# tomer196/GaUDI

Hardware: AMD Instinct MI355X
Metric: guided molecules/sec (1000-step) (higher is better)
Workload: dtype f32

## Files before the change

### gaudi_amd/_lib.py

```python
from __future__ import annotations

import ctypes as C
import os

import numpy as np

_PKG = os.path.dirname(os.path.abspath(__file__))
LIB_PATH = os.environ.get("GAUDI_LIB", os.path.join(_PKG, "libgaudi_hip.so"))


class GaudiError(RuntimeError):
    pass


class EdmConfig(C.Structure):
    _fields_ = [("in_node_nf", C.c_int32), ("hidden_nf", C.c_int32), ("n_layers", C.c_int32),
                ("inv_sublayers", C.c_int32), ("attention", C.c_int32), ("tanh", C.c_int32),
                ("coords_range", C.c_float), ("norm_constant", C.c_float), ("normalization_factor", C.c_float),
                ("diffusion_steps", C.c_int32), ("noise_power", C.c_float), ("noise_precision", C.c_float),
                ("norm_values", C.c_float * 3), ("sin_embedding", C.c_int32)]


class PredConfig(C.Structure):
    _fields_ = [("in_nf", C.c_int32), ("out_nf", C.c_int32), ("hidden_nf", C.c_int32), ("n_layers", C.c_int32),
# ... 18 lines not shown


class AtomTables(C.Structure):
    _fields_ = [("n_types", C.c_int32), ("ring_size", C.c_int32 * 16), ("ring_elem", (C.c_int32 * 6) * 16),
                ("templ", ((C.c_double * 2) * 6) * 16), ("no_orientation", C.c_int32 * 16), ("extra_angle", C.c_double * 16),
                ("n_template_h", C.c_int32 * 16), ("template_h_parent", (C.c_int32 * 2) * 16), ("h_elem", C.c_int32),
                ("c_elem", C.c_int32), ("h_bond", C.c_double)]


ATOMS_MAX_ATOMS = 384
ATOMS_MAX_BONDS = 384
ATOMS_PLACE_H, ATOMS_FINGERPRINT = 1, 2

FP = C.POINTER(C.c_float)
IP = C.POINTER(C.c_int32)
DP = C.POINTER(C.c_double)


class TargetSpec(C.Structure):
    _fields_ = [("K", C.c_int32), ("w", FP), ("q", FP), ("c", FP), ("side", IP), ("scale", FP),
                ("w_per_mol", C.c_int32), ("q_per_mol", C.c_int32), ("c_per_mol", C.c_int32), ("side_per_mol", C.c_int32),
                ("scale_per_mol", C.c_int32), ("t_lo", C.c_int32), ("t_hi", C.c_int32)]


TARGET_CB = C.CFUNCTYPE(None, C.c_void_p, C.c_int, C.c_int, FP, C.c_float, FP)
TARGET_CBZ = C.CFUNCTYPE(None, C.c_void_p, C.c_int, C.c_int, C.c_int, C.c_int, FP, FP, C.c_float, FP, FP)

EXPORTS = {
    "gaudi_create": (C.c_int, [C.c_int, C.POINTER(C.c_void_p)]),
    "gaudi_destroy": (None, [C.c_void_p]),
    "gaudi_last_error": (C.c_char_p, [C.c_void_p]),
    "gaudi_load_edm": (C.c_int, [C.c_void_p, C.POINTER(EdmConfig), C.c_int, C.POINTER(C.c_char_p), C.POINTER(FP),
                                 C.POINTER(C.c_int64)]),
    "gaudi_load_predictor": (C.c_int, [C.c_void_p, C.POINTER(PredConfig), C.c_int, C.POINTER(C.c_char_p),
                                       C.POINTER(FP), C.POINTER(C.c_int64)]),
    "gaudi_get_gamma": (C.c_int, [C.c_void_p, FP]),
    "gaudi_get_step_coefficients": (C.c_int, [C.c_void_p, FP]),
    "gaudi_phi": (C.c_int, [C.c_void_p, C.c_int, C.c_int, FP, FP, FP, FP, FP]),
    "gaudi_predictor_fwd": (C.c_int, [C.c_void_p, C.c_int, C.c_int, FP, FP, FP, FP, FP]),
    "gaudi_predictor_grad": (C.c_int, [C.c_void_p, C.c_int, C.c_int, FP, FP, FP, FP, FP, FP, FP]),
    "gaudi_step": (C.c_int, [C.c_void_p, C.c_int, C.c_int, C.c_int, FP, FP, FP, FP, FP, C.c_float, FP]),
    "gaudi_decode": (C.c_int, [C.c_void_p, C.c_int, C.c_int, FP, FP, FP, FP, FP, FP]),
    "gaudi_sample": (C.c_int, [C.c_void_p, C.c_int, C.c_int, FP, FP, C.c_uint64, C.c_int64, FP, C.c_float, FP,
                               C.c_float, FP, FP, FP, C.POINTER(Diag)]),
    "gaudi_sample_cb": (C.c_int, [C.c_void_p, C.c_int, C.c_int, FP, FP, C.c_uint64, C.c_int64, FP, C.c_float, TARGET_CB,
                                  C.c_void_p, C.c_float, FP, FP, FP, C.POINTER(Diag)]),
    "gaudi_sample_cbz": (C.c_int, [C.c_void_p, C.c_int, C.c_int, FP, FP, C.c_uint64, C.c_int64, FP, C.c_float, TARGET_CBZ,
                                   C.c_void_p, C.c_float, FP, FP, FP, C.POINTER(Diag)]),
    "gaudi_sample_chain": (C.c_int, [C.c_void_p, C.c_int, C.c_int, FP, FP, C.c_uint64, C.c_int64, FP, C.c_float, C.c_int, FP]),
    "gaudi_predict_noised": (C.c_int, [C.c_void_p, C.c_int, C.c_int, FP, FP, IP, FP, FP, C.c_uint64, C.c_int64, FP, FP, FP]),
    "gaudi_check_stability": (C.c_int, [C.c_void_p, C.POINTER(RingTables), C.c_int, C.c_int, FP, IP, IP,
                                        C.POINTER(C.c_uint8), FP, FP, C.POINTER(StabilityAux)]),
    "gaudi_stability_profile_get": (C.c_int, [C.c_void_p, C.POINTER(C.c_int32), C.POINTER(C.c_double)]),
    "gaudi_rings_to_atoms": (C.c_int, [C.c_void_p, C.POINTER(RingTables), C.POINTER(AtomTables), C.c_int, C.c_int, FP, IP, IP,
                                       C.c_int, C.c_int, C.c_int, IP, IP, DP, DP, IP, IP, IP, C.POINTER(C.c_uint64)]),
    "gaudi_atoms_profile_get": (C.c_int, [C.c_void_p, C.POINTER(C.c_int32), C.POINTER(C.c_double)]),
    "gaudi_philox_normal": (C.c_int, [C.c_void_p, C.c_uint64, C.c_int64, C.c_int, C.c_int, C.c_int, C.c_int, FP]),
    "gaudi_host_schedule": (C.c_int, [C.c_int, C.c_float, C.c_float, FP, FP]),
    "gaudi_host_eigh3": (C.c_int, [C.c_int, DP, DP]),
    "gaudi_host_graph_meta": (C.c_int, [C.c_int, C.c_int, FP, FP, C.POINTER(C.c_int32), C.POINTER(C.c_int32),
                                        C.POINTER(C.c_int32), C.POINTER(C.c_uint32), C.POINTER(C.c_uint32), FP, C.c_int32,
                                        C.POINTER(C.c_int32)]),
    "gaudi_host_pack_matrix": (C.c_int, [C.c_int, C.c_int, C.c_int, C.c_int, C.c_int, FP, FP]),
    "gaudi_host_pack_matrix_split": (C.c_int, [C.c_int, C.c_int, C.c_int, C.c_int, C.c_int, C.c_int, C.c_float, FP, FP]),
    "gaudi_host_pack_matrix_f16": (C.c_int, [C.c_int, C.c_int, C.c_int, C.c_int, C.c_int, C.c_float, FP, FP]),
    "gaudi_host_weight_scale": (C.c_int, [C.c_int, C.POINTER(FP), IP, IP, IP, FP]),
    "gaudi_host_node_operand_offset": (C.c_int, [C.c_int, C.c_int, C.c_int, C.c_int, C.c_int, IP]),
    "gaudi_profile_reset": (C.c_int, [C.c_void_p, C.c_int]),
    "gaudi_profile_get": (C.c_int, [C.c_void_p, C.POINTER(C.c_int32), C.POINTER(C.c_double), C.POINTER(C.c_int64)]),
    "gaudi_set_steps_per_launch": (C.c_int, [C.c_void_p, C.c_int]),
    "gaudi_set_readout_nodes": (C.c_int, [C.c_void_p, C.c_int]),
    "gaudi_set_fix_noise": (C.c_int, [C.c_void_p, C.c_int, C.c_int64]),
    "gaudi_host_graph_meta8": (C.c_int, [C.c_int, C.c_int, FP, FP, C.POINTER(C.c_int32), C.POINTER(C.c_int32),
                                         C.POINTER(C.c_int32), C.POINTER(C.c_uint32), C.POINTER(C.c_uint32), FP,
                                         C.POINTER(C.c_uint16), C.POINTER(C.c_uint16), C.c_int32, C.POINTER(C.c_int32)]),
    "gaudi_kernel_variant": (C.c_int, [C.c_void_p, C.POINTER(C.c_int32), C.POINTER(C.c_int32)]),
    "gaudi_edge_math": (C.c_int, [C.c_void_p, C.POINTER(C.c_int32), C.POINTER(C.c_int32)]),
    "gaudi_node_buffers": (C.c_int, [C.c_void_p, C.POINTER(C.c_int32)]),
    "gaudi_last_workgroups": (C.c_int, [C.c_void_p, C.POINTER(C.c_int32), C.POINTER(C.c_int32)]),
    "gaudi_host_pack_plan_wide": (C.c_int, [C.c_int, C.c_int, C.c_int, C.c_int, FP, FP, C.POINTER(C.c_int32), C.POINTER(C.c_int32),
                                           C.POINTER(C.c_int32), C.POINTER(C.c_int32)]),
    "gaudi_set_plan_hint": (C.c_int, [C.c_void_p, C.c_int32, C.c_int32]),
    "gaudi_last_warning": (C.c_char_p, [C.c_void_p]),
    "gaudi_abi_version": (C.c_int, []),
    "gaudi_last_family_split": (C.c_int, [C.c_void_p, C.POINTER(C.c_int32)]),
    "gaudi_profile_clock": (C.c_int, [C.c_void_p, C.POINTER(C.c_double)]),
    "gaudi_last_keep_h": (C.c_int, [C.c_void_p, C.POINTER(C.c_int32)]),
    "gaudi_host_pack_plan": (C.c_int, [C.c_int, C.c_int, FP, FP, C.POINTER(C.c_int32), C.POINTER(C.c_int32), C.POINTER(C.c_int32),
                                      C.POINTER(C.c_int32)]),
    "gaudi_edm_nll": (C.c_int, [C.c_void_p, C.c_int, C.c_int, FP, FP, IP, FP, FP, C.c_uint64, C.c_int64, FP, FP, FP]),
    "gaudi_host_nll_terms": (C.c_int, [C.c_int, C.c_float, C.c_float, C.c_float, C.c_float, C.c_int, C.c_int, C.c_int, FP, FP, FP,
                                       IP, FP]),
    "gaudi_predictor_loss_grad": (C.c_int, [C.c_void_p, C.c_int, C.c_int, FP, FP, IP, FP, FP, FP, C.c_uint64, C.c_int64, FP, FP,
                                            FP, FP, IP]),
    "gaudi_predictor_grad_size": (C.c_int, [C.c_void_p, C.POINTER(C.c_int64)]),
    "gaudi_host_pred_train_layout": (C.c_int, [C.c_void_p, C.c_int, C.POINTER(C.c_char_p), C.POINTER(FP), C.POINTER(C.c_int64),
                                               IP, IP, FP]),
    "gaudi_edm_loss_grad": (C.c_int, [C.c_void_p, C.c_int, C.c_int, FP, FP, IP, FP, FP, C.c_uint64, C.c_int64, FP, C.c_int, FP,
                                      FP, FP, FP, IP]),
    "gaudi_edm_grad_size": (C.c_int, [C.c_void_p, C.POINTER(C.c_int64)]),
    "gaudi_edm_set_train_weights": (C.c_int, [C.c_void_p, C.c_int, C.POINTER(C.c_char_p), C.POINTER(FP), C.POINTER(C.c_int64)]),
    "gaudi_host_edm_train_layout": (C.c_int, [C.c_void_p, C.c_int, C.POINTER(C.c_char_p), C.POINTER(FP), C.POINTER(C.c_int64),
                                              IP, IP, FP]),
    "gaudi_host_edm_seed_coef": (C.c_int, [C.c_int, C.c_int, C.c_int, C.c_int, C.c_int, IP, FP, FP, FP]),
    "gaudi_sample_grid": (C.c_int, [C.c_void_p, C.c_int, C.c_int, FP, FP, C.c_uint64, C.c_int64, FP, C.c_float, FP, C.c_float,
                                    C.c_int, IP, FP, FP, FP, FP, FP, FP, C.POINTER(Diag)]),
    "gaudi_step_pair": (C.c_int, [C.c_void_p, C.c_int, C.c_int, C.c_int, C.c_int, FP, FP, FP, FP, FP, C.c_float, FP]),
    "gaudi_sample_cb_grid": (C.c_int, [C.c_void_p, C.c_int, C.c_int, FP, FP, C.c_uint64, C.c_int64, FP, C.c_float, TARGET_CB,
                                       TARGET_CBZ, C.c_void_p, C.c_float, C.c_int, IP, FP, FP, FP, FP, FP, FP, C.POINTER(Diag)]),
    "gaudi_host_grid_coefficients": (C.c_int, [C.c_int, C.c_float, C.c_float, C.c_int, IP, FP, IP]),
    "gaudi_sample_target": (C.c_int, [C.c_void_p, C.c_int, C.c_int, FP, FP, C.c_uint64, C.c_int64, FP, C.c_float,
                                      C.POINTER(TargetSpec), C.c_int, IP, FP, FP, FP, FP, FP, FP, FP, C.POINTER(Diag)]),
    "gaudi_step_target": (C.c_int, [C.c_void_p, C.c_int, C.c_int, C.c_int, C.c_int, FP, FP, FP, FP, C.POINTER(TargetSpec), FP, FP]),
    "gaudi_host_target_seed": (C.c_int, [C.POINTER(TargetSpec), C.c_int, C.c_int, FP, FP]),
}

ABI_VERSION = 7
_ROUND6_EXPORTS = ("gaudi_last_warning", "gaudi_abi_version", "gaudi_last_family_split", "gaudi_profile_clock", "gaudi_last_keep_h")
_NLL_EXPORTS = ("gaudi_edm_nll", "gaudi_predictor_loss_grad", "gaudi_predictor_grad_size", "gaudi_edm_loss_grad",
                "gaudi_edm_grad_size", "gaudi_edm_set_train_weights")
_GRID_EXPORTS = ("gaudi_sample_grid", "gaudi_step_pair", "gaudi_sample_cb_grid")
_TARGET_EXPORTS = ("gaudi_sample_target", "gaudi_step_target")
_ATOMS_EXPORTS = ("gaudi_rings_to_atoms", "gaudi_atoms_profile_get")

_lib = None


def load_library() -> C.CDLL:
    global _lib
    if _lib is not None:
        return _lib
    if not os.path.exists(LIB_PATH):
        raise GaudiError(f"{LIB_PATH} not found: build it with `python -m gaudi_amd.build` "
                         "(there is no CPU fallback for the sampler)")
    lib = C.CDLL(LIB_PATH)
    lenient = "GAUDI_LIB" in os.environ
    abi = None
    if hasattr(lib, "gaudi_abi_version"):
        lib.gaudi_abi_version.restype, lib.gaudi_abi_version.argtypes = C.c_int, []
        abi = int(lib.gaudi_abi_version())
    if abi != ABI_VERSION and not lenient:
        raise GaudiError(f"{LIB_PATH} exports ABI version {abi}, this package expects {ABI_VERSION}: rebuild it "
                         "(`python -m gaudi_amd.build --force`)")
    for name, (res, args) in EXPORTS.items():
        if lenient and not hasattr(lib, name) and (name.startswith("gaudi_host_") or name in _ROUND6_EXPORTS + _NLL_EXPORTS + _GRID_EXPORTS + _TARGET_EXPORTS + _ATOMS_EXPORTS):
            continue
        if lenient and abi != ABI_VERSION and name.startswith("gaudi_host_"):
            continue
        fn = getattr(lib, name)
        fn.restype = res
        fn.argtypes = args
    _lib = lib
    return lib


def fptr(a: np.ndarray | None):
    if a is None:
        return None
    assert a.dtype == np.float32 and a.flags["C_CONTIGUOUS"]
    return a.ctypes.data_as(FP)


def f32(a) -> np.ndarray:
    return np.ascontiguousarray(np.asarray(a, dtype=np.float32))


def grid_coefficients(T: int, noise_power: float, noise_precision: float, grid):
    lib = load_library()
    g = np.ascontiguousarray(np.asarray(grid).reshape(-1), dtype=np.int32)
    coef = np.zeros((max(len(g) - 1, 0), 4), np.float32)
    land = np.zeros(max(len(g) - 1, 0), np.int32)
    rc = lib.gaudi_host_grid_coefficients(int(T), float(noise_power), float(noise_precision), len(g), g.ctypes.data_as(IP),
                                          coef.ctypes.data_as(FP), land.ctypes.data_as(IP))
    if rc != 0:
        raise GaudiError(f"gaudi_host_grid_coefficients failed ({rc}): the grid must be strictly descending integers "
                         f"T >= g[0] > ... > g[n] = 0 with at least two entries")
    return coef, land
```

### gaudi_amd/csrc/gaudi_hip.hip

```cpp
#include <hip/hip_runtime.h>

#include <algorithm>
#include <climits>
#include <queue>
#include <cmath>
#include <cstdio>
#include <cstdlib>
#include <chrono>
#include <cstring>
#include <map>
#include <mutex>
#include <string>
#include <vector>

#include "../../include/gaudi_hip.h"
#include "kernel_table.h"

using namespace gaudi;

struct DevBuf {
  void* p = nullptr;
  size_t cap = 0;
  hipError_t reserve(size_t bytes) {
    if (bytes <= cap) return hipSuccess;
    if (p) (void)hipFree(p);
    p = nullptr;
    cap = 0;
    hipError_t e = hipMalloc(&p, bytes);
    if (e == hipSuccess) cap = bytes;
    return e;
  }
  void release() {
    if (p) (void)hipFree(p);
    p = nullptr;
    cap = 0;
  }
  template <class T>
  T* as() const { return (T*)p; }
};

struct PinBuf {
  void* p = nullptr;
  size_t cap = 0;
  hipError_t reserve(size_t bytes) {
    if (bytes <= cap) return hipSuccess;
    if (p) (void)hipHostFree(p);
    p = nullptr;
    cap = 0;
    hipError_t e = hipHostMalloc(&p, bytes, hipHostMallocDefault);
    if (e == hipSuccess) cap = bytes;
    return e;
  }
  void release() {
    if (p) (void)hipHostFree(p);
    p = nullptr;
    cap = 0;
  }
  template <class T>
  T* as() const { return (T*)p; }
};

enum NodeBuf : int {
  kResident = 0,
  kAllGlobal = 1,
  kPqLds = 2,
  kPredFifthGlobal = 3,
};
struct LaunchPlan {
  int waves = 4;
  int ring = 0;
  bool mr = false;
  NodeBuf nodes = kResident;
  bool two = false;
  bool fr = false;
  int ef = 2;
  int groups = 0;
  int nslots = 0;
  int hk = 0;
  int pubx = 0, pub_ch = 0;
};

struct gaudi_handle {
  int device = 0;
  hipStream_t stream = nullptr;
  std::string err;
  std::string warn;
  bool has_edm = false, has_pred = false;
  gaudi_edm_config ecfg{};
  gaudi_pred_config pcfg{};
  int HPE = 0, HPP = 0;
  DevBuf edm_w, pred_w, coef_d, edm_w4, pred_w4;
  DevBuf edm_ws, pred_ws;
  size_t edm_w_bytes = 0, pred_w_bytes = 0, edm_ws_bytes = 0, pred_ws_bytes = 0;
  float edm_hinv = 0.f, pred_hinv = 0.f;
  std::vector<float> gamma, coef;
  DevBuf d_mask, d_order, d_edges, d_emask, d_npairs, d_seg, d_zin, d_zout, d_t, d_x, d_h, d_noise, d_nan, d_dpred,
      d_pred, d_tw, d_stash, d_chain, d_sx, d_stype, d_sn, d_sflags, d_sdist, d_sadj, d_saux, d_stab, d_as, d_ncols, d_soff,
      d_sidx, d_gnode, d_rowmap, d_compmol, d_ncomp, d_clock, d_gcoef, d_gidx, d_zt;
  DevBuf d_atoms[9];
  DevBuf d_vtpar, d_vttrace, d_vtdev;
  struct VtCall {
    const gaudi_target_spec* spec = nullptr;
    int K = 0, Btot = 0, b0 = 0;
    float* trace = nullptr;
  }* vt = nullptr;
  PinBuf p_pred, p_dpred;
  PinBuf p_z, p_dz;
  DevBuf d_dz;
  hipEvent_t cb_event = nullptr;
  int steps_per_launch = 25;
  int variant = 8;
  LaunchPlan plan;
  bool split = true;
  bool no_fr = false;
  bool wide_full = true;
  bool gn8_pq = true;
  bool gn8 = true;
  bool force_gn8 = false;
  bool pack = true;
  int pairs_cap = -1;
  int pairs = 1;
  int num_cus = 256;
  bool pred_rounds = true;
  bool pack_now = false;
  bool force_mr = false;
  bool force_gn = false;
  bool fix_noise = false;
  long long fix_key = 0;
  int readout_n = 0;
  struct PredTrainState* pt = nullptr;
  struct EdmTrainState* et = nullptr;
  bool edm_stale = false;
  int plan_min_slots = 0, plan_force_waves = 0;
  int call_min_slots = 0, call_force_waves = 0;
  bool call_cut = false;
  int call_narrow = 0;
  const int32_t* call_molmap = nullptr;
  bool keep_h = true;
  bool gn8_pack = true;
  bool family_split = false;
  int last_split_resident = 0;
  bool prof = false;
  struct EventLog {
    std::vector<std::pair<hipEvent_t, hipEvent_t>> pending, spare;
    double ms = 0.0;
    long long n = 0;
    static constexpr size_t kWindow = 32;
    hipError_t fold(size_t keep) {
      while (pending.size() > keep) {
        float t = 0.f;
        hipError_t e = hipEventSynchronize(pending.front().second);
        if (e == hipSuccess) e = hipEventElapsedTime(&t, pending.front().first, pending.front().second);
        if (e != hipSuccess) return e;
        ms += t;
        ++n;
        spare.push_back(pending.front());
        pending.erase(pending.begin());
      }
      return hipSuccess;
    }
    hipError_t begin(hipStream_t st, std::pair<hipEvent_t, hipEvent_t>& ev) {
      hipError_t e = fold(kWindow - 1);
      if (e != hipSuccess) return e;
      if (!spare.empty()) {
        ev = spare.back();
        spare.pop_back();
      } else {
        if ((e = hipEventCreate(&ev.first)) != hipSuccess) return e;
        if ((e = hipEventCreate(&ev.second)) != hipSuccess) return e;
      }
      return hipEventRecord(ev.first, st);
    }
    hipError_t end(hipStream_t st, const std::pair<hipEvent_t, hipEvent_t>& ev) {
      pending.push_back(ev);
      return hipEventRecord(ev.second, st);
    }
    void reset(bool destroy) {
      for (auto& p : pending) spare.push_back(p);
      pending.clear();
      if (destroy) {
        for (auto& p : spare) {
          (void)hipEventDestroy(p.first);
          (void)hipEventDestroy(p.second);
        }
        spare.clear();
      }
      ms = 0.0;
      n = 0;
    }
  } prof_log, stab_log, atoms_log;
  long long prof_steps = 0;
#ifdef GAUDI_STAMPS
  DevBuf d_stamps;
  unsigned long long stamp_acc[32] = {0};
#endif
};

// ... 407 lines not shown
      }
      if (want_align && !sl.empty()) {
        const int prev_i = sl.back().i;
        while (sl.size() % 16) sl.push_back({prev_i, prev_i, 0.f, false});
      }
      want_align = false;
      const int o = (int)sl.size() % 16;
      if ((o + L + 15) / 16 > 2) {
        const int prev_i = sl.empty() ? i : sl.back().i;
        while (sl.size() % 16) sl.push_back({prev_i, prev_i, 0.f, false});
      }
      runs[b][i] = {(int)sl.size(), L};
      sl.insert(sl.end(), run.begin(), run.end());
      total[b] += L;
    }
    if (!sl.empty()) {
      const int prev_i = sl.back().i;
      while (sl.size() % 16) sl.push_back({prev_i, prev_i, 0.f, false});
    }
    M.ncols[b] = last + 1;
    M.ntiles[b] = (int)sl.size() / 16;
    max_tiles = std::max(max_tiles, M.ntiles[b]);
  }
  M.S = std::max(16 * max_tiles, (min_slots + 15) / 16 * 16);
  if (M.S > 0xffff) {
    err = "too many edge slots";
    return GAUDI_E_CAPACITY;
  }
  const int S = M.S;
  M.edges.assign((size_t)B * S, 0);
  M.emask.assign((size_t)B * S, 0.f);
  M.seg.assign((size_t)B * N, 0);
  M.soff.assign((size_t)B * (N + 1), 0);
  M.sidx.assign((size_t)B * S, 0);
  for (int b = 0; b < B; ++b) {
    const std::vector<Slot>& sl = slots[b];
    const int ns = (int)sl.size();
    for (int t0 = 0; t0 < ns; t0 += 16) {
      int c = 0;
      while (c < 16) {
        int e = c;
        while (e + 1 < 16 && sl[t0 + e + 1].i == sl[t0 + c].i) ++e;
        const int i = sl[t0 + c].i;
        const int part = runs[b][i].second > 0 && runs[b][i].first < t0 ? 1 : 0;
        for (int k = c; k <= e; ++k) {
          const Slot& q = sl[t0 + k];
          M.edges[(size_t)b * S + t0 + k] = (uint32_t)q.i | ((uint32_t)q.j << 8) | ((uint32_t)c << 16) |
                                            ((uint32_t)(k == e) << 20) | ((uint32_t)part << 21);
          M.emask[(size_t)b * S + t0 + k] = q.m;
        }
        c = e + 1;
      }
    }
    for (int i = 0; i < N; ++i)
      M.seg[(size_t)b * N + i] = ((uint32_t)runs[b][i].first << 16) | (uint32_t)runs[b][i].second;
    uint16_t* off = &M.soff[(size_t)b * (N + 1)];
    uint16_t* idx = &M.sidx[(size_t)b * S];
    int n_out = 0;
    for (int j = 0; j < N; ++j) {
      off[j] = (uint16_t)n_out;
      for (int k = 0; k < ns; ++k)
        if (sl[k].live && sl[k].j == j) idx[n_out++] = (uint16_t)k;
    }
    off[N] = (uint16_t)n_out;
  }
  M.order.resize(B);
  for (int b = 0; b < B; ++b) M.order[b] = b;
  std::stable_sort(M.order.begin(), M.order.end(), [&](int a, int c) {
    return M.ntiles[a] != M.ntiles[c] ? M.ntiles[a] > M.ntiles[c] : total[a] > total[c];
  });
  return GAUDI_OK;
}

KernelTable* gaudi::g_kernel_tables;

static kernel_fn find_kernel(const KernelKey& k) {
  for (const KernelTable* t = g_kernel_tables; t; t = t->next)
    for (int i = 0; i < t->n; ++i)
      if (t->entries[i].key == k) return t->entries[i].fn;
  return nullptr;
}
static std::string key_name(const KernelKey& k) {
  char buf[160];
  snprintf(buf, sizeof buf, "waves=%d SP=%d MR=%d GN=%d FR=%d PG=%d EF=%d HPE=%d HPP=%d VT=%d", k.waves, k.sp, (int)k.mr, k.gn, (int)k.fr,
           (int)k.pg, k.ef, k.hpe, k.hpp, (int)k.vt);
  return buf;
}
static std::string duplicate_kernel_key() {
  std::vector<KernelKey> seen;
  for (const KernelTable* t = g_kernel_tables; t; t = t->next)
    for (int i = 0; i < t->n; ++i) {
      if (std::find(seen.begin(), seen.end(), t->entries[i].key) != seen.end()) return key_name(t->entries[i].key);
      seen.push_back(t->entries[i].key);
    }
  return "";
}
static int gn_of(NodeBuf nodes) { return nodes == kAllGlobal ? 1 : nodes == kPqLds ? 2 : 0; }
static KernelKey key4(int hpe, int hpp, bool gn = false, int ef = 2) {
  KernelKey k{};
  k.waves = 4;
  k.gn = gn ? 1 : 0;
  k.ef = ef;
  k.hpe = hpe;
  k.hpp = hpp;
  return k;
}
static KernelKey key8(int hpe, int hpp, int ring, bool mr, NodeBuf nodes = kResident) {
  KernelKey k{};
  k.waves = 8;
  k.sp = ring;
  k.mr = mr;
  k.gn = gn_of(nodes);
  k.pg = nodes == kPredFifthGlobal;
  k.ef = 2;
  k.hpe = hpe;
  k.hpp = hpp;
  return k;
}
static bool have_kernel8(int hpe, int hpp, int ring, bool mr, NodeBuf nodes = kResident) {
  return find_kernel(key8(hpe, hpp, ring, mr, nodes)) != nullptr;
}
static NodeBuf launch_nodes(const LaunchPlan& p, int hpe, int hpp) {
  return p.nodes == kPredFifthGlobal && !(hpe && hpp) ? kResident : p.nodes;
}
static kernel_fn plan_kernel(const LaunchPlan& p, int hpe, int hpp, bool vt) {
  if (p.waves != 8) {
    KernelKey k = key4(hpe, hpp, p.nodes == kAllGlobal, hpe ? p.ef : 2);
    k.vt = vt && hpp;
    return find_kernel(k);
  }
  const NodeBuf nodes = launch_nodes(p, hpe, hpp);
  const bool mr = p.mr && hpp;
  KernelKey k = nodes == kResident ? key8(hpe, hpp, p.ring, mr) : key8(hpe, hpp, 1, true, nodes);
  k.vt = vt && hpp;
  if (p.fr && nodes == kResident && !mr) {
    k.fr = true;
    if (kernel_fn f = find_kernel(k)) return f;
    k.fr = false;
  }
  return find_kernel(k);
}

static int round_hidden(int H) {
  static const int sizes[] = {32, 48, 64, 128, 192, 208, 256};
  for (int s : sizes)
    if (s >= H) return s;
  return 0;
}

static int dense_ew4(int N) { return std::max(32, ((N + kWaves - 1) / kWaves * (N - 1) + 31) / 32 * 32); }

static size_t lds_bytes(int hpe, int hpp, int N, int D, int EW, bool gn = false, int ef = 2) {
  size_t net = 0;
  if (hpe)
    net = std::max(net, (size_t)((gn ? 0 : 4 * N * (hpe + 4)) + kWaves * 16 * (hpe + 4) + 8 * N + kWaves * EW * 9 + (6 + ef) * hpe +
                                 (ef > 2 ? kWaves * EW * ef : 0)));
  if (hpp) net = std::max(net, (size_t)((gn ? 0 : 5 * N * (hpp + 4)) + kWaves * 16 * (hpp + 4) + 12 * N + kWaves * EW * 10 + 32 + 10 * hpp));
  return sizeof(float) * (common_floats(N, D, EW) + net);
}
static size_t gnode_floats(int hpe, int hpp, int N) {
  return std::max((size_t)(hpe ? 4 * N * (hpe + 4) : 0), (size_t)(hpp ? 5 * N * (hpp + 4) : 0));
}

static size_t lds_floats8_base(int hpe, int hpp, int N, int D, int S, int split, NodeBuf nodes = kResident) {
  size_t net = 0;
  const int pbuf = nodes == kPredFifthGlobal ? 4 : 5;
  const int gn = gn_of(nodes);
  if (hpe) net = std::max(net, (size_t)((gn ? w8::gn_lds_buffers(gn) : 5) * N * (hpe + 4) + w8::edge_ring_floats(hpe, split) + 8 * N + 2 * align4(N) + 96 + S * 9 + 8 * hpe));
  if (hpp) net = std::max(net, (size_t)(w8::edge_ring_floats(hpp, split) + (gn ? w8::gn_lds_buffers(gn) : pbuf) * N * (hpp + 4) + 12 * N + 2 * align4(N) + 96 + S * 10 + 32 + 10 * hpp));
  return common_floats8(N, D, S) + net;
}
static size_t gnode_floats8(int hpe, int hpp, int N) {
  return std::max((size_t)(hpe ? 5 * N * (hpe + 4) : 0), (size_t)(hpp ? 5 * N * (hpp + 4) : 0));
}
static bool gn8_stage_fits(int hpe, int hpp, int N) {
  for (int hp : {hpe, hpp})
    if (hp && 2 * (size_t)w8::stage_stride(N * (hp + 4)) > w8::edge_ring_floats(hp, 1)) return false;
  return true;
}
static bool node_f16_fits(int hp, int N, int split, NodeBuf nodes) {
  const bool gn = gn_of(nodes) != 0;
  if (!hp || !split || !GAUDI_NODE_F16) return true;
  if (N > (gn ? 48 : 32)) return false;
  const int nct = N <= 16 ? 1 : N <= 32 ? 2 : 3;
  const int ring = w8::edge_ring_floats(hp, split);
  return w8::nh_split_floats(hp, nct) <= (w8::node_ring_idle(hp, split, gn) ? ring : ring / 2);
}
static bool plan_pub8(int hpe, int hpp, int N, int D, int S, int split, int& pubx, int& pub_ch, NodeBuf nodes = kResident) {
  pubx = 0;
  pub_ch = 0;
  const int gn = gn_of(nodes);
  if (!node_f16_fits(hpe, N, split, nodes) || !node_f16_fits(hpp, N, split, nodes)) return false;
  const long long cap = 160 * 1024 / 4 - 64;
  const long long base = (long long)lds_floats8_base(hpe, hpp, N, D, S, split, nodes);
  if (base > cap) return false;
  if (!hpp) return true;
  const int T = hpp / 16;
  const long long own = (gn ? 0LL : 2LL * N * (hpp + 4)) + (split ? w8::edge_ring_floats(hpp, split) : 0);
  pub_ch = w8::pub_chunk_tiles(S, own + (cap - base), T);
  if (pub_ch < 1) return false;
  const int nch = (T + pub_ch - 1) / pub_ch;
  pub_ch = (T + nch - 1) / nch;
  pubx = (int)std::max(0LL, (long long)S * (16 * pub_ch + 4) - own);
  return true;
}
static size_t lds_bytes8(int hpe, int hpp, int N, int D, int S, int pubx, int split, NodeBuf nodes = kResident) {
  return sizeof(float) * (lds_floats8_base(hpe, hpp, N, D, S, split, nodes) + (hpp ? pubx : 0));
}

static int launch(gaudi_handle* h, const KParams& P, int hpe, int hpp, long long steps) {
  const LaunchPlan& plan = h->plan;
  const bool v8 = plan.waves == 8;
  const bool se = hpe && plan.ef > 2;
  const kernel_fn fn = plan_kernel(plan, hpe, hpp, P.vt != nullptr);
  if (!fn)
    return fail(h, GAUDI_E_INVALID,
                "no kernel instantiated for padded hidden sizes (" + std::to_string(hpe) + "," + std::to_string(hpp) + ")" +
                    (v8 ? " in the 8-wave family" : se ? " among the sin_embedding kernels" : ""));
  size_t lds = v8 ? lds_bytes8(hpe, hpp, P.N, 3 + P.F, P.EW, P.pubx, plan.ring, launch_nodes(plan, hpe, hpp))
                  : lds_bytes(hpe, hpp, P.N, 3 + P.F, P.EW, plan.nodes == kAllGlobal, se ? 24 : 2);
  if (v8 && P.hk_off) lds = sizeof(float) * ((size_t)P.hk_off + (size_t)plan.hk);
  if (lds > 160 * 1024)
    return fail(h, GAUDI_E_CAPACITY, "molecule needs " + std::to_string(lds) + " B of LDS (>160 KiB): N too large");
  {
    static std::mutex attr_mu;
    static std::map<std::pair<int, const void*>, int> granted_by_fn;
    std::lock_guard<std::mutex> lock(attr_mu);
    int& granted = granted_by_fn[{h->device, (const void*)fn}];
    if ((int)lds > granted) {
      HIPCHECK(h, hipFuncSetAttribute((const void*)fn, hipFuncAttributeMaxDynamicSharedMemorySize, (int)lds));
      granted = (int)lds;
    }
  }
  std::pair<hipEvent_t, hipEvent_t> ev{nullptr, nullptr};
  if (h->prof) HIPCHECK(h, h->prof_log.begin(h->stream, ev));
#ifdef GAUDI_STAMPS
  KParams PS = P;
  HIPCHECK(h, h->d_stamps.reserve(sizeof(unsigned long long) * 32));
  HIPCHECK(h, hipMemsetAsync(h->d_stamps.p, 0, sizeof(unsigned long long) * 32, h->stream));
  PS.stamps = h->d_stamps.as<unsigned long long>();
  hipLaunchKernelGGL(fn, dim3(P.B), dim3(v8 ? w8::kThreads : kThreads), lds, h->stream, PS);
  {
    unsigned long long tmp[32];
    HIPCHECK(h, hipMemcpyAsync(tmp, h->d_stamps.p, sizeof(tmp), hipMemcpyDeviceToHost, h->stream));
    HIPCHECK(h, hipStreamSynchronize(h->stream));
    for (int i = 0; i < 32; ++i) h->stamp_acc[i] += tmp[i];
    if (getenv("GAUDI_PRINT_STAMPS")) {
      static const char* nm[] = {"node_gemm", "edge_gemm", "edge_epilogue", "barrier", "misc", "bwd_node", "bwd_stash_reload",
                                 "bwd_colsum_tail", "pub_wait", "stash", "pub_write", "colsum_loop", "colsum_barrier", "b_dcp",
                                 "b_gemm_de", "b_dv", "b_gemm_dt1", "b_du", "stage_vectors", "geo", "edm_embed_head", "noise_update",
                                 "bwd_reload_loads", "bwd_vec_commit", "pred_readout", "bwd_prologue", "x2", "x3"};
      unsigned long long tot = 0;
      for (int i = 0; i < ST_N; ++i) tot += h->stamp_acc[i];
      fprintf(stderr, "[stamps] cumulative shares (block 0, wave 0):");
      for (int i = 0; i < ST_N; ++i) fprintf(stderr, " %s=%.1f%%", nm[i], 100.0 * h->stamp_acc[i] / (tot ? tot : 1));
      fprintf(stderr, " total=%llu ticks\n", tot);
      if (tmp[31])
        fprintf(stderr, "[stamps] shader clock during this launch: %.0f MHz (%llu cycles / %llu ticks of 100 MHz)\n",
                100.0 * (double)tmp[30] / (double)tmp[31], tmp[30], tmp[31]);
    }
  }
#else
  if (h->prof) {
    KParams PC = P;
    HIPCHECK(h, h->d_clock.reserve(sizeof(unsigned long long) * 4));
    PC.clock_out = h->d_clock.as<unsigned long long>();
    hipLaunchKernelGGL(fn, dim3(P.B), dim3(v8 ? w8::kThreads : kThreads), lds, h->stream, PC);
  } else {
    hipLaunchKernelGGL(fn, dim3(P.B), dim3(v8 ? w8::kThreads : kThreads), lds, h->stream, P);
  }
#endif
  HIPCHECK(h, hipGetLastError());
  if (h->prof) {
    HIPCHECK(h, h->prof_log.end(h->stream, ev));
    h->prof_steps += steps;
  }
  return GAUDI_OK;
}

struct Pack {
  int G = 0;
  int NG = 0;
  std::vector<float> umask, uemask;
  std::vector<uint8_t> align;
  std::vector<int32_t> rowmap;
  std::vector<int32_t> compmol;
  std::vector<int32_t> ncomp;
};
static std::vector<std::vector<int>> used_nodes(int B, int N, const float* node_mask, const float* edge_mask) {
  std::vector<std::vector<int>> used(B);
  for (int b = 0; b < B; ++b) {
    std::vector<char> keep(N, 0);
    for (int i = 0; i < N; ++i) {
      const bool li = node_mask[(size_t)b * N + i] != 0.f;
      if (li) keep[i] = 1;
      for (int j = 0; j < N; ++j) {
        const bool lj = node_mask[(size_t)b * N + j] != 0.f;
        if (edge_mask[((size_t)b * N + i) * N + j] != 0.f && (li || lj)) keep[i] = keep[j] = 1;
      }
    }
    for (int i = 0; i < N; ++i)
      if (keep[i]) used[b].push_back(i);
  }
  return used;
}
static void pack_groups(int B, int N, const float* node_mask, const float* edge_mask, const Meta8& M, Pack& pk, int NG = 0,
                        int TG = w8::kWaves, bool narrow = false, int maxcomp = kMaxComp, const int32_t* molmap = nullptr,
                        int max_multi = INT_MAX) {
  if (NG < N && !narrow) NG = N;
  const std::vector<std::vector<int>> used = used_nodes(B, N, node_mask, edge_mask);
  struct Group {
    std::vector<int> mols;
    int nodes = 0, tiles = 0;
  };
  std::vector<Group> groups;
  int multi = 0;
  for (int b : M.order) {
    const int nn = (int)used[b].size(), nt = M.ntiles[b];
    Group* fit = nullptr;
    for (Group& g : groups)
      if ((int)g.mols.size() < maxcomp && g.nodes + nn <= NG && g.tiles + nt <= TG && (g.mols.size() > 1 || multi < max_multi)) {
        fit = &g;
        if (g.mols.size() == 1) ++multi;
        break;
      }
    if (!fit) {
      groups.emplace_back();
      fit = &groups.back();
    }
    fit->mols.push_back(b);
    fit->nodes += nn;
    fit->tiles += nt;
  }
  const int G = (int)groups.size();
  pk.G = G;
  pk.NG = NG;
  pk.umask.assign((size_t)G * NG, 0.f);
  pk.uemask.assign((size_t)G * NG * NG, 0.f);
  pk.align.assign((size_t)G * NG, 0);
  pk.rowmap.assign((size_t)G * NG, -1);
  pk.compmol.assign((size_t)G * kMaxComp, 0);
  pk.ncomp.assign(G, 0);
  std::vector<int> slot_of(N);
  for (int g = 0; g < G; ++g) {
    int base = 0;
    for (size_t k = 0; k < groups[g].mols.size(); ++k) {
      const int b = groups[g].mols[k];
      pk.compmol[(size_t)g * kMaxComp + k] = molmap ? molmap[b] : b;
      std::fill(slot_of.begin(), slot_of.end(), -1);
      for (size_t r = 0; r < used[b].size(); ++r) slot_of[used[b][r]] = base + (int)r;
      if (!used[b].empty()) pk.align[(size_t)g * NG + base] = 1;
      for (int i : used[b]) {
        const int si = slot_of[i];
        pk.umask[(size_t)g * NG + si] = node_mask[(size_t)b * N + i];
        pk.rowmap[(size_t)g * NG + si] = (b * N + i) | ((int32_t)k << 28);
// ... 84 lines not shown
    }
  }
  if (!gn8 && !narrow_taken && h->pack_now && h->pack && B > 1 && (int64_t)B * N < (1 << 28)) {
    struct Cand {
      int NG, TG;
    };
    std::vector<Cand> cands;
    bool want_wide = h->pairs == 2;
    int max_multi = INT_MAX;
    if (h->pairs == 1 && B > h->num_cus) {
      const int cus = std::max(1, h->num_cus);
      const double solo = (double)((B + cus - 1) / cus);
      auto makespan = [&](int p) {
        const double kPair = 1.81, kAlone = 1.07;
        std::priority_queue<double, std::vector<double>, std::greater<double>> free_at;
        for (int c = 0; c < cus; ++c) free_at.push(0.0);
        double end = 0.0;
        auto run = [&](int n, double cost) {
          for (int k = 0; k < n; ++k) {
            const double t = free_at.top() + cost;
            free_at.pop();
            free_at.push(t);
            end = std::max(end, t);
          }
        };
        run(p, kPair);
        run(B - 2 * p, kAlone);
        return end;
      };
      double best = solo * 0.995;
      int best_p = -1;
      for (int p = cus; p <= B / 2 + cus - 1; p += cus) {
        const int pp = std::min(p, B / 2);
        const double m = makespan(pp);
        if (m < best) { best = m; best_p = pp; }
      }
      if (h->pairs_cap >= 0) best_p = std::min(h->pairs_cap, B / 2);
      if (best_p >= 0) {
        pack_groups(B, N, node_mask, edge_mask, M, pk, N, w8::kWaves);
        want_wide = (long long)pk.G * 10 >= (long long)B * 9;
        max_multi = best_p;
      }
    }
    if (want_wide && h->pairs_cap >= 0) max_multi = h->pairs_cap;
    if (want_wide)
      for (int ng = std::min(2 * N, 32); ng > N; --ng) {
        const long long cap = 160 * 1024 / 4 - 64;
        if ((long long)lds_floats8_base(hpe, hpp, ng, Dz, 16 * (w8::kWaves + 1), h->split ? 2 : 0) > cap) continue;
        cands.push_back({ng, 2 * w8::kWaves});
      }
    cands.push_back({N, w8::kWaves});
    for (const Cand& cd : cands) {
      const bool wide = cd.NG > N;
      pack_groups(B, N, node_mask, edge_mask, M, pk, cd.NG, cd.TG, false, kMaxComp, nullptr, wide ? max_multi : INT_MAX);
      if (pk.G >= B && !(wide && h->pairs_cap == 0)) continue;
      Meta8 M2;
      rc = build_meta8(pk.G, cd.NG, pk.umask.data(), pk.uemask.data(), M2, err, wide ? 0 : M.S, pk.align.data());
      if (rc != GAUDI_OK) continue;
      const bool mr2 = hpp && M2.S > 16 * w8::kWaves;
      if (!wide && M2.S > std::max(M.S, 16 * w8::kWaves)) continue;
      if (mr2 && !mr && !h->pred_rounds) continue;
      RingPlan p2 = plan_for(cd.NG, M2.S, mr2);
      if (p2.mode < 0 || (p2.mode != 0) != (mode_u != 0)) continue;
      RingPlan full{1, 0, 0};
      if (wide && p2.mode == 2 && mr2 && h->wide_full && hpe && hpp && have_kernel8(hpe, hpp, 1, true, kPredFifthGlobal) &&
          plan_pub8(hpe, hpp, cd.NG, Dz, M2.S, 1, full.pubx, full.pub_ch, kPredFifthGlobal)) {
        p2 = full;
        pg_run = true;
      }
      M = std::move(M2);
      B = pk.G;
      nm_used = pk.umask.data();
      n_slots = cd.NG;
      acc = p2;
      mr_run = mr2;
      use_pack = true;
      break;
    }
  }
  const bool packed = use_pack;
  const NodeBuf nodes = pg_run ? kPredFifthGlobal : gn8;
  P.pubx = acc.pubx;
  P.pub_ch = acc.pub_ch;
  if (getenv("GAUDI_DEBUG_PLAN"))
    fprintf(stderr, "[plan] molecules=%d workgroups=%d N=%d node slots=%d S=%d split=%d mr=%d nodes=%d pub_ch=%d pubx=%d lds=%zu\n", B0, B, N,
            n_slots, M.S, acc.mode, (int)mr_run, (int)nodes, acc.pub_ch, acc.pubx, lds_bytes8(hpe, hpp, n_slots, Dz, M.S, acc.pubx, acc.mode, nodes));
  auto up = [&](DevBuf& d, const void* src, size_t bytes) -> hipError_t {
    hipError_t e = d.reserve(bytes);
    if (e != hipSuccess) return e;
    return hipMemcpyAsync(d.p, src, bytes, hipMemcpyHostToDevice, h->stream);
  };
  HIPCHECK(h, up(h->d_ncols, M.ncols.data(), sizeof(int) * B));
  HIPCHECK(h, up(h->d_mask, nm_used, sizeof(float) * B * n_slots));
  if (packed) {
    HIPCHECK(h, up(h->d_rowmap, pk.rowmap.data(), sizeof(int32_t) * pk.rowmap.size()));
    HIPCHECK(h, up(h->d_compmol, pk.compmol.data(), sizeof(int32_t) * pk.compmol.size()));
    HIPCHECK(h, up(h->d_ncomp, pk.ncomp.data(), sizeof(int32_t) * pk.ncomp.size()));
  }
  HIPCHECK(h, up(h->d_order, M.order.data(), sizeof(int) * B));
  HIPCHECK(h, up(h->d_edges, M.edges.data(), sizeof(uint32_t) * M.edges.size()));
  HIPCHECK(h, up(h->d_emask, M.emask.data(), sizeof(float) * M.emask.size()));
  HIPCHECK(h, up(h->d_npairs, M.ntiles.data(), sizeof(int) * B));
  HIPCHECK(h, up(h->d_seg, M.seg.data(), sizeof(uint32_t) * M.seg.size()));
  HIPCHECK(h, up(h->d_soff, M.soff.data(), sizeof(uint16_t) * M.soff.size()));
  HIPCHECK(h, up(h->d_sidx, M.sidx.data(), sizeof(uint16_t) * M.sidx.size()));
  HIPCHECK(h, hipStreamSynchronize(h->stream));
  P.B = B;
  P.N = n_slots;
  P.NR = N;
  P.EW = M.S;
  P.node_mask = h->d_mask.as<float>();
  P.order = h->d_order.as<int>();
  P.edges = h->d_edges.as<uint32_t>();
  P.emask = h->d_emask.as<float>();
  P.npairs = h->d_npairs.as<int>();
  P.seginfo = h->d_seg.as<uint32_t>();
  P.ncols = h->d_ncols.as<int>();
  P.soff = h->d_soff.as<uint16_t>();
  P.sidx = h->d_sidx.as<uint16_t>();
  P.rowmap = packed ? h->d_rowmap.as<int32_t>() : nullptr;
  P.compmol = packed ? h->d_compmol.as<int32_t>() : nullptr;
  P.ncomp = packed ? h->d_ncomp.as<int32_t>() : nullptr;
  P.hk_off = 0;
  int hk = 0;
  if (h->keep_h && GAUDI_NODE_F16 && acc.mode >= 1 && nodes == kResident) {
    const size_t floats = lds_bytes8(hpe, hpp, n_slots, Dz, M.S, acc.pubx, acc.mode) / sizeof(float);
    const size_t at = (floats + 3) & ~(size_t)3;
    const size_t need = (size_t)w8::nh_keep_floats(std::max(hpe, hpp), n_slots);
    if ((at + need) * sizeof(float) + 1024 <= 160 * 1024) {
      P.hk_off = (int)at;
      hk = (int)need;
    }
  }
  if (pg_run) {
    const size_t stride = ((size_t)n_slots * (hpp + 4) + 63) / 64 * 64;
    HIPCHECK(h, h->d_gnode.reserve(sizeof(float) * (stride * (size_t)B + 256)));
    P.gnode = h->d_gnode.as<float>();
    P.gnode_stride = (long long)stride;
  }
  if (gn8) {
    const size_t stride = (gnode_floats8(hpe, hpp, N) + 63) / 64 * 64;
    HIPCHECK(h, h->d_gnode.reserve(sizeof(float) * (stride * (size_t)B + 256)));
    P.gnode = h->d_gnode.as<float>();
    P.gnode_stride = (long long)stride;
  }
  plan.waves = 8;
  plan.ring = acc.mode;
  plan.mr = mr_run;
  plan.nodes = nodes;
  plan.fr = !h->no_fr && gn8 == kResident && acc.mode == 1 && n_slots > 16;
  plan.groups = B;
  plan.nslots = n_slots;
  plan.hk = hk;
  plan.pubx = acc.pubx;
  plan.pub_ch = acc.pub_ch;
  return GAUDI_OK;
}

static int stage_graph(gaudi_handle* h, int B, int N, const float* node_mask, const float* edge_mask, KParams& P, int hpe,
                       int hpp) {
  if (B <= 0 || N <= 0) return fail(h, GAUDI_E_INVALID, "B and N must be positive");
  if ((int64_t)B * N >= (1 << 28)) return fail(h, GAUDI_E_CAPACITY, "B * N must stay below 2^28 per call: cut the request into several calls");
  LaunchPlan plan;
  const bool se = hpe && h->ecfg.sin_embedding;
  if (h->variant == 8 && !h->force_gn && !se) {
    const int rc8 = stage_graph8(h, B, N, node_mask, edge_mask, P, hpe, hpp, plan);
    if (rc8 == GAUDI_OK) h->plan = plan;
    if (rc8 <= 0) return rc8;
    P.pubx = P.pub_ch = 0;
  }
  plan.groups = B;
  plan.nslots = N;
  if (hpp && 4 * N * 3 > 4 * 16 * (hpp + 4))
    return fail(h, GAUDI_E_CAPACITY, "N too large for the 4-wave predictor kernels at this hidden size");
  Meta M;
  std::string err;
  int rc = build_meta(B, N, node_mask, edge_mask, M, err);
  if (rc) return fail(h, rc, err);
  HIPCHECK(h, h->d_mask.reserve(sizeof(float) * B * N));
  HIPCHECK(h, h->d_order.reserve(sizeof(int) * B));
  HIPCHECK(h, h->d_edges.reserve(sizeof(uint32_t) * M.edges.size()));
  HIPCHECK(h, h->d_emask.reserve(sizeof(float) * M.emask.size()));
  HIPCHECK(h, h->d_npairs.reserve(sizeof(int) * M.npairs.size()));
  HIPCHECK(h, h->d_seg.reserve(sizeof(uint32_t) * M.seg.size()));
  HIPCHECK(h, h->d_ncols.reserve(sizeof(int) * B));
  HIPCHECK(h, hipMemcpyAsync(h->d_ncols.p, M.ncols.data(), sizeof(int) * B, hipMemcpyHostToDevice, h->stream));
  HIPCHECK(h, hipMemcpyAsync(h->d_mask.p, node_mask, sizeof(float) * B * N, hipMemcpyHostToDevice, h->stream));
  HIPCHECK(h, hipMemcpyAsync(h->d_order.p, M.order.data(), sizeof(int) * B, hipMemcpyHostToDevice, h->stream));
  HIPCHECK(h, hipMemcpyAsync(h->d_edges.p, M.edges.data(), sizeof(uint32_t) * M.edges.size(), hipMemcpyHostToDevice, h->stream));
  HIPCHECK(h, hipMemcpyAsync(h->d_emask.p, M.emask.data(), sizeof(float) * M.emask.size(), hipMemcpyHostToDevice, h->stream));
  HIPCHECK(h, hipMemcpyAsync(h->d_npairs.p, M.npairs.data(), sizeof(int) * M.npairs.size(), hipMemcpyHostToDevice, h->stream));
  HIPCHECK(h, hipMemcpyAsync(h->d_seg.p, M.seg.data(), sizeof(uint32_t) * M.seg.size(), hipMemcpyHostToDevice, h->stream));
  HIPCHECK(h, hipStreamSynchronize(h->stream));
  P.B = B;
  P.N = N;
  P.NR = N;
  P.EW = M.EW;
  P.node_mask = h->d_mask.as<float>();
  P.order = h->d_order.as<int>();
  P.edges = h->d_edges.as<uint32_t>();
  P.emask = h->d_emask.as<float>();
  P.npairs = h->d_npairs.as<int>();
  P.seginfo = h->d_seg.as<uint32_t>();
  P.ncols = h->d_ncols.as<int>();
  const int Dz = 3 + (hpe ? h->ecfg.in_node_nf : h->pcfg.in_nf);
  const bool part_of_batch = h->plan_min_slots || h->plan_force_waves || h->call_min_slots || h->call_force_waves || h->call_cut;
  const int ef = plan.ef = se ? 24 : 2;
  const bool have_g = (!hpe || find_kernel(key4(hpe, 0, true, ef))) && (!hpp || find_kernel(key4(0, hpp, true)));
  if (h->force_gn || lds_bytes(hpe, hpp, N, Dz, part_of_batch ? std::max(M.EW, dense_ew4(N)) : M.EW, false, ef) > 160 * 1024) {
    if (have_g && lds_bytes(hpe, hpp, N, Dz, M.EW, true, ef) <= 160 * 1024) {
      plan.nodes = kAllGlobal;
      const size_t stride = (gnode_floats(hpe, hpp, N) + 63) / 64 * 64;
      HIPCHECK(h, h->d_gnode.reserve(sizeof(float) * stride * (size_t)B));
      P.gnode = h->d_gnode.as<float>();
      P.gnode_stride = (long long)stride;
    }
  }
  plan.two = plan.nodes == kAllGlobal || (se && hpp && !find_kernel(key4(hpe, hpp, false, ef)));
  h->plan = plan;
  return GAUDI_OK;
}

static void fill_edm(gaudi_handle* h, KParams& P) {
  const gaudi_edm_config& c = h->ecfg;
  P.F = c.in_node_nf;
  P.T = c.diffusion_steps;
  P.edm.w = (h->variant == 8 && h->plan.waves == 4) ? h->edm_w4.as<float>() : h->edm_w.as<float>();
  P.edm.w_bytes = (unsigned)h->edm_w_bytes;
  P.edm.F = c.in_node_nf;
  P.edm.L = c.n_layers;
  P.edm.S = c.inv_sublayers;
  P.edm.attention = c.attention;
  P.edm.use_tanh = c.tanh;
  P.edm.coords_range = c.coords_range;
  P.edm.norm_constant = c.norm_constant;
  P.edm.normf = c.normalization_factor > 0.f ? c.normalization_factor : (float)P.NR;
  P.edm.ktail = h->plan.waves == 8 && has_ktail(c.hidden_nf, h->HPE);
  P.edm.ws = h->edm_ws.as<float>();
  P.edm.ws_bytes = (unsigned)h->edm_ws_bytes;
  P.edm.hinv = h->edm_hinv;
  P.coef = h->coef_d.as<float>();
  const float g0 = h->gamma[0];
  P.alpha0 = sqrtf(sigmoid_host(-g0));
  P.sigma0 = sqrtf(sigmoid_host(g0));
  P.sigma_x = expf(0.5f * g0);
  P.nv0 = c.norm_values[0];
  P.nv1 = c.norm_values[1];
}

extern "C" {

int gaudi_create(int device, gaudi_handle** out) {
  if (!out) return GAUDI_E_INVALID;
  *out = nullptr;
  static const std::string dup = duplicate_kernel_key();
  if (!dup.empty()) {
    fprintf(stderr, "libgaudi_hip: two translation units register the kernel %s\n", dup.c_str());
    return GAUDI_E_INVALID;
  }
  int n = 0;
  if (hipGetDeviceCount(&n) != hipSuccess || device < 0 || device >= n) return GAUDI_E_HIP;
  gaudi_handle* h = new gaudi_handle();
  h->device = device;
  if (const char* v = getenv("GAUDI_WAVES")) h->variant = atoi(v) == 4 ? 4 : 8;
  if (const char* v = getenv("GAUDI_EDGE_MATH")) h->split = std::string(v) != "fp32";
  if (const char* v = getenv("GAUDI_FORCE_GN")) h->force_gn = atoi(v) != 0;
  if (const char* v = getenv("GAUDI_GN8")) h->gn8 = atoi(v) != 0;
  if (const char* v = getenv("GAUDI_FORCE_GN8")) h->force_gn8 = atoi(v) != 0;
  if (const char* v = getenv("GAUDI_FORCE_MR")) h->force_mr = atoi(v) != 0;
  if (const char* v = getenv("GAUDI_PACK")) h->pack = atoi(v) != 0;
  if (const char* v = getenv("GAUDI_GN8_PACK")) h->gn8_pack = atoi(v) != 0;
  if (const char* v = getenv("GAUDI_GN8_PQ")) h->gn8_pq = atoi(v) != 0;
  if (const char* v = getenv("GAUDI_WIDE_FULL")) h->wide_full = atoi(v) != 0;
  if (const char* v = getenv("GAUDI_KEEP_H")) h->keep_h = atoi(v) != 0;
  if (const char* v = getenv("GAUDI_FAMILY_SPLIT")) h->family_split = atoi(v) != 0;
  if (const char* v = getenv("GAUDI_PAIRS")) h->pairs = atoi(v);
  if (const char* v = getenv("GAUDI_PAIRS_CAP")) h->pairs_cap = atoi(v);
  {
    int cus = 0;
    if (hipDeviceGetAttribute(&cus, hipDeviceAttributeMultiprocessorCount, device) == hipSuccess && cus > 0) h->num_cus = cus;
  }
  if (const char* v = getenv("GAUDI_PRED_ROUNDS")) h->pred_rounds = atoi(v) != 0;
  h->no_fr = getenv("GAUDI_NO_FR") != nullptr;
  h->plan.waves = h->variant;
  if (hipSetDevice(device) != hipSuccess || hipStreamCreateWithFlags(&h->stream, hipStreamNonBlocking) != hipSuccess) {
    delete h;
    return GAUDI_E_HIP;
  }
  *out = h;
  return GAUDI_OK;
}

void gaudi_destroy(gaudi_handle* h) {
  if (!h) return;
  (void)hipSetDevice(h->device);
  if (h->stream) (void)hipStreamSynchronize(h->stream);
  h->prof_log.reset(true);
  h->stab_log.reset(true);
  h->atoms_log.reset(true);
  DevBuf* bufs[] = {&h->edm_w, &h->pred_w, &h->coef_d, &h->edm_w4, &h->pred_w4, &h->edm_ws, &h->pred_ws, &h->d_mask, &h->d_order, &h->d_edges, &h->d_emask, &h->d_npairs,
                    &h->d_seg, &h->d_zin, &h->d_zout, &h->d_t, &h->d_x, &h->d_h, &h->d_noise, &h->d_nan, &h->d_dpred,
                    &h->d_pred, &h->d_tw, &h->d_stash, &h->d_chain, &h->d_sx, &h->d_stype, &h->d_sn,
                    &h->d_sflags, &h->d_sdist, &h->d_sadj, &h->d_saux, &h->d_stab, &h->d_as, &h->d_ncols, &h->d_soff, &h->d_sidx,
                    &h->d_gnode, &h->d_rowmap, &h->d_compmol, &h->d_ncomp, &h->d_gcoef, &h->d_gidx, &h->d_zt, &h->d_vtpar, &h->d_vttrace, &h->d_vtdev};
  for (DevBuf* b : bufs) b->release();
  for (DevBuf& b : h->d_atoms) b.release();
  pt_release(h);
  et_release(h);
  h->p_pred.release();
  h->p_dpred.release();
  h->p_z.release();
  h->p_dz.release();
  h->d_dz.release();
  if (h->cb_event) (void)hipEventDestroy(h->cb_event);
  if (h->stream) (void)hipStreamDestroy(h->stream);
  delete h;
}

const char* gaudi_last_error(const gaudi_handle* h) { return h ? h->err.c_str() : "null handle"; }
const char* gaudi_last_warning(const gaudi_handle* h) { return h ? h->warn.c_str() : ""; }
int gaudi_abi_version(void) { return GAUDI_ABI_VERSION; }
int gaudi_profile_clock(gaudi_handle* h, double* shader_mhz) {
  if (!h || !shader_mhz) return GAUDI_E_INVALID;
  *shader_mhz = 0.0;
  if (!h->d_clock.p) return GAUDI_OK;
  HIPCHECK(h, hipSetDevice(h->device));
  unsigned long long c[4] = {0, 0, 0, 0};
  HIPCHECK(h, hipStreamSynchronize(h->stream));
  HIPCHECK(h, hipMemcpy(c, h->d_clock.p, sizeof(c), hipMemcpyDeviceToHost));
  if (c[3] > c[1] && c[2] > c[0]) *shader_mhz = 100.0 * (double)(c[2] - c[0]) / (double)(c[3] - c[1]);
  return GAUDI_OK;
}
int gaudi_last_keep_h(const gaudi_handle* h, int32_t* lds_floats) {
  if (!h || !lds_floats) return GAUDI_E_INVALID;
  *lds_floats = h->plan.hk;
  return GAUDI_OK;
}
int gaudi_last_family_split(const gaudi_handle* h, int32_t* resident_molecules) {
  if (!h || !resident_molecules) return GAUDI_E_INVALID;
  *resident_molecules = h->last_split_resident;
  return GAUDI_OK;
}

int gaudi_load_edm(gaudi_handle* h, const gaudi_edm_config* cfg, int n, const char* const* names,
                   const float* const* tensors, const int64_t* numel) {
  if (!h || !cfg) return GAUDI_E_INVALID;
  HIPCHECK(h, hipSetDevice(h->device));
  const int H = cfg->hidden_nf, F = cfg->in_node_nf, F1 = F + 1, L = cfg->n_layers, S = cfg->inv_sublayers;
  if (H <= 0 || H > 256) return fail(h, GAUDI_E_INVALID, "hidden_nf must be in 1..256");
  if (F < 1 || F > 15) return fail(h, GAUDI_E_INVALID, "in_node_nf must be in 1..15");
  if (L < 1 || S < 1 || cfg->diffusion_steps < 1) return fail(h, GAUDI_E_INVALID, "bad n_layers/inv_sublayers/diffusion_steps");
  if (!(cfg->normalization_factor >= 0.f)) return fail(h, GAUDI_E_INVALID, "normalization_factor must be > 0 (or 0: 'mean' aggregation)");
  const int HP = round_hidden(H);
  if (!HP) return fail(h, GAUDI_E_INVALID, "no kernel instantiated for this hidden size");
  Tensors T;
  for (int i = 0; i < n; ++i) T.m[names[i]] = {tensors[i], numel[i]};
  const int EF = cfg->sin_embedding ? 24 : 2;
  EdmLayout lay{HP, F1, L, S, EF};
  const std::string p = "dynamics.egnn.";
  const int PK = HP * HP;
  float hscale = 0.f;
  {
    NodeScale ns;
    for (int l = 0; l < L; ++l) {
      for (int s = 0; s <= S; ++s) {
        const std::string q = p + "e_block_" + std::to_string(l) + (s < S ? ".gcl_" + std::to_string(s) + "." : ".gcl_equiv.");
        ns.see(T.peek(q + (s < S ? "edge_mlp.0.weight" : "coord_mlp.0.weight"), (int64_t)H * (2 * H + EF)), H, 2 * H + EF, 0, 2 * H);
        ns.see(T.peek(q + (s < S ? "edge_mlp.2.weight" : "coord_mlp.2.weight"), (int64_t)H * H), H, H, 0, H, true);
        if (s < S) {
          ns.see(T.peek(q + "node_mlp.0.weight", (int64_t)H * 2 * H), H, 2 * H, 0, 2 * H);
          ns.see(T.peek(q + "node_mlp.2.weight", (int64_t)H * H), H, H, 0, H);
        }
      }
    }
    hscale = ns.scale();
    if (!(hscale > 0.f) && h->variant == 8 && h->split && EF == 2)
      h->warn = std::string("EDM weights: the fp16-pair images cannot carry this weight set (") + ns.why() +
                "): its calls run the fp32-instruction kernels (about 0.55 x the speed, same results at fp32 accuracy)";
  }
  auto pack = [&](bool lane_linear, std::vector<float>& w, std::vector<float>* ws) {
  w.assign((size_t)lay.total(), 0.f);
  if (ws) ws->assign(2 * (size_t)lay.total(), 0.f);
  PackMode pe;
  pe.lane_linear = lane_linear;
  pe.ktail = lane_linear && has_ktail(H, HP);
  pe.wbase = w.data();
  pe.ws = ws;
  pe.hscale = ws ? hscale : 0.f;
  pe.hktail = has_ktail(H, HP);
  const PackMode pn = pe.with_ktail(false);
  {
    const float* ew = T.get(p + "embedding.weight", (int64_t)H * F1);
    const float* eb = T.get(p + "embedding.bias", H);
    const float* ow = T.get(p + "embedding_out.weight", (int64_t)F1 * H);
    const float* ob = T.get(p + "embedding_out.bias", F1);
    if (ew && eb && ow && ob) {
      for (int f = 0; f < H; ++f)
        for (int k = 0; k < F1; ++k) w[lay.emb_w() + f * F1 + k] = ew[f * F1 + k];
      pack_vec(&w[lay.emb_b()], eb, H);
      for (int o = 0; o < F1; ++o)
        for (int k = 0; k < H; ++k) w[lay.out_w() + o * HP + k] = ow[o * H + k];
      pack_vec(&w[lay.out_b()], ob, F1);
    }
// ... 1233 lines not shown
```

### gaudi_amd/csrc/kernel_table.h

```cpp
#pragma once
#include "sampler_kernel.h"

namespace gaudi {

typedef void (*kernel_fn)(const KParams);

struct KernelKey {
  int waves;
  int sp;
  bool mr;
  int gn;
  bool fr, pg;
  int ef;
  int hpe, hpp;
  bool vt;
};
inline bool operator==(const KernelKey& a, const KernelKey& b) {
  return a.waves == b.waves && a.sp == b.sp && a.mr == b.mr && a.gn == b.gn && a.fr == b.fr && a.pg == b.pg && a.ef == b.ef &&
         a.hpe == b.hpe && a.hpp == b.hpp && a.vt == b.vt;
}

struct KernelEntry {
  KernelKey key;
  kernel_fn fn;
};
template <class V, int HPE, int HPP, bool VT = false>
constexpr KernelEntry entry() {
  KernelEntry e{};
  e.key.waves = V::kWaveCount;
  e.key.sp = V::kSplit;
  e.key.mr = V::kMR;
  e.key.gn = V::kGN;
  e.key.fr = V::kFR;
  e.key.pg = V::kPG;
  e.key.ef = V::kEF;
  e.key.hpe = HPE;
  e.key.hpp = HPP;
  e.key.vt = VT;
  e.fn = &sampler_kernel_v<V, HPE, HPP, VT>;
  return e;
}

struct KernelTable {
  const KernelEntry* entries;
  int n;
  KernelTable* next;
  template <int N>
  explicit KernelTable(const KernelEntry (&e)[N]);
};
extern KernelTable* g_kernel_tables;
template <int N>
KernelTable::KernelTable(const KernelEntry (&e)[N]) : entries(e), n(N), next(g_kernel_tables) {
  g_kernel_tables = this;
}

}
```

### gaudi_amd/csrc/sampler_kernel.h

```cpp
#pragma once
#include "edm_device.h"
#include "pred_device.h"
#include "w8_edm.h"
#include "w8_pred.h"

#ifndef GAUDI_STATIC_PRIO
#define GAUDI_STATIC_PRIO 0
#endif

namespace gaudi {

enum Mode { MODE_PHI = 0, MODE_SAMPLE = 1, MODE_PRED_FWD = 2, MODE_PRED_GRAD = 3, MODE_GUIDE = 4, MODE_NLL = 5 };

struct KParams {
  int mode, B, N, F, EW;
  int NR;
  int do_init, do_decode, guided;
  int s_hi, s_lo, T;
  const float* node_mask;
  const int* order;
  const uint32_t* edges;
  const float* emask;
  const int* npairs;
  const uint32_t* seginfo;
  const int* ncols;
  const uint16_t* soff;
  const uint16_t* sidx;
  int pubx, pub_ch;
  const float* z_in;
  float* z_out;
  const float* t_in;
  float* x_out;
  float* h_out;
  const float* noise;
  int draw_base;
  long long draw_stride;
  unsigned long long seed;
  long long sample_offset;
  int fix_noise;
  long long fix_key;
  float std0;
  const float* coef;
  const int* step_idx;
  float alpha0, sigma0, sigma_x, nv0, nv1;
  int* nan_count;
  EdmDev edm;
  PredDev pred;
  const float* dpred_in;
  const float* dz_in;
  const float* target_w;
  float scale;
  float* pred_out;
  float* stash;
  long long stash_stride;
  float readout_div;
  const float* alpha_sigma;
  float* zt_out;
  int split;
  float* chain_out;
  int keep_frames;
  unsigned long long* stamps;
  float* gnode;
  long long gnode_stride;
  const int32_t* rowmap;
  const int32_t* compmol;
  const int32_t* ncomp;
  unsigned long long* clock_out;
  int hk_off;
  const struct VtDev* vt;
};
struct VtDev {
  const float* par;
  float* trace;
  int top;
  int B;
};
__device__ __forceinline__ const float* vt_row(const VtDev* vt, int b, int K) { return vt->par + (size_t)b * target_row_floats(K); }
__device__ __forceinline__ float* vt_trace_row(const VtDev* vt, int b, int K, int srow) {
  float* const t = vt->trace;
  return t != nullptr ? t + ((size_t)(vt->top - srow) * vt->B + b) * (K + 2) : nullptr;
}
constexpr int kMaxComp = 4;

__host__ __device__ inline int common_floats(int N, int D, int EW) {
  return 3 * align16(N * D) + align16(N) + 16 + align16(N) + 16 + 2 * kWaves * EW + align16(N);
}
__host__ __device__ inline int common_floats8(int N, int D, int S) {
  return 3 * align16(N * D) + align16(N) + 16 + align16(N) + 16 + 2 * S + align16(N) + align16((N + 1 + S + 1) / 2);
}
__device__ __forceinline__ int row_of(int w) { return w & 0x0fffffff; }
__device__ __forceinline__ int comp_of(int w) { return (w >> 28) & 7; }

template <bool GN, int EF = 2>
struct V4T {
  static constexpr int kThreads = gaudi::kThreads;
  static constexpr bool kGlobalNodes = GN;
  static constexpr int kWaveCount = 4, kSplit = 0, kGN = GN ? 1 : 0, kEF = EF;
  static constexpr bool kMR = false, kFR = false, kPG = false;
  using Graph = gaudi::MolGraph;
  template <int HP> using EdmSmem = gaudi::NetSmem<HP, GN, EF>;
  __device__ __forceinline__ static void set_rows(Graph&, const int*, int, int) {}
  __host__ __device__ static int graph_floats(int N, int EW) { return 2 * gaudi::kWaves * EW + align16(N); }
  __device__ __forceinline__ static float* load_graph(const KParams& P, int b, float* base, const float* sMask, Graph& mg, int tid, int wave) {
    const int N = P.N, EW = P.EW;
    uint32_t* sEdge = (uint32_t*)base; base += gaudi::kWaves * EW;
    float* sEm = base; base += gaudi::kWaves * EW;
    uint32_t* sSeg = (uint32_t*)base; base += align16(N);
    for (int i = tid; i < N; i += kThreads) sSeg[i] = P.seginfo[b * N + i];
    for (int i = tid; i < gaudi::kWaves * EW; i += kThreads) {
      sEdge[i] = P.edges[(size_t)b * gaudi::kWaves * EW + i];
      sEm[i] = P.emask[(size_t)b * gaudi::kWaves * EW + i];
    }
    mg.N = N; mg.D = 3 + P.F; mg.EW = EW;
    mg.NC = P.ncols[b];
    mg.mask = sMask; mg.edge = sEdge; mg.em = sEm; mg.seg = sSeg;
    mg.npairs = P.npairs[b * gaudi::kWaves + wave];
#pragma unroll
    for (int w = 0; w < gaudi::kWaves; ++w) mg.npairs_all[w] = P.npairs[b * gaudi::kWaves + w];
    return base;
  }
  template <int HP>
  __device__ __forceinline__ static void edm(const EdmDev& W, const Graph& mg, float* net, const float* sZ, float* sEps,
                                             float* sMean, float t_val, int tid STAMP_DECL, float* gnode) {
    gaudi::NetSmem<HP, GN, EF> sm;
    sm.carve(net, mg.N, mg.EW, gnode);
    gaudi::edm_forward<HP>(W, mg, sm, sZ, sEps, sMean, t_val, tid STAMP_ARGS);
  }
  template <int HP>
  __device__ __forceinline__ static void guide(const PredDev& W, const Graph& mg, float* net, float* sZ, float* sGrad, float* sTmp,
                                               float* sMean, float t_val, float sigma, const float* target_w, float scale,
                                               float* pred_out, float readout_div, float* stash, int tid STAMP_DECL, int phase,
                                               const float* dpred_ext, float* gnode, const float* dz_ext, const VtDev* vt,
                                               int b, int srow) {
    float* const tr = vt != nullptr ? vt_trace_row(vt, b, W.K, srow) : nullptr;
    gaudi::guidance_update<HP, GN>(W, mg, net, sZ, sGrad, sTmp, sMean, t_val, sigma, target_w, scale, tr != nullptr ? tr : pred_out,
                                   readout_div, stash, tid STAMP_ARGS, phase, dpred_ext, gnode, dz_ext,
                                   vt != nullptr ? vt_row(vt, b, W.K) : nullptr, tr != nullptr ? tr + W.K : nullptr);
  }
  template <int HP>
  __device__ __forceinline__ static void pred_entry(const PredDev& W, const Graph& mg, float* net, float* sZ, float* sGrad,
                                                    float* sTmp, float* sMean, float t_val, const float* dpred, bool want_grad,
                                                    float* pred_out, float readout_div, float* stash, int tid STAMP_DECL, float* gnode) {
    gaudi::predictor_entry<HP, GN>(W, mg, net, sZ, sGrad, sTmp, sMean, t_val, dpred, want_grad, pred_out, readout_div, stash,
                                   tid STAMP_ARGS, gnode);
  }
};
using V4 = V4T<false>;
using V4G = V4T<true>;
using V4S = V4T<false, 24>;
using V4GS = V4T<true, 24>;

struct Lds8 {
  float *sZ, *sEps, *sNz, *sMask, *sMean, *net;
  int *sRow, *sCmol;
  uint32_t *sEdge, *sSeg;
  float* sEm;
  uint16_t *sOff, *sIdx;
};
__device__ __forceinline__ Lds8 carve_lds8(float* smem, int N, int D, int S) {
  Lds8 L;
  float* base = smem;
  L.sZ = base; base += align16(N * D);
  L.sEps = base; base += align16(N * D);
  L.sNz = base; base += align16(N * D);
  L.sMask = base; base += align16(N);
  L.sMean = base; base += 16;
  L.sRow = (int*)base; base += align16(N);
  L.sCmol = (int*)base; base += 16;
  L.sEdge = (uint32_t*)base; base += S;
  L.sEm = base; base += S;
  L.sSeg = (uint32_t*)base; base += align16(N);
  L.sOff = (uint16_t*)base;
  L.sIdx = L.sOff + (N + 1);
  base += align16((N + 1 + S + 1) / 2);
  L.net = base;
  return L;
}
struct Graph8Args {
  int N, D, S, NC, ntiles, pubx, pub_ch, hk;
};
__device__ __forceinline__ w8::MolGraph graph8(const Lds8& L, const Graph8Args& a) {
  w8::MolGraph mg;
  mg.N = a.N; mg.D = a.D; mg.S = a.S; mg.NC = a.NC;
  mg.ntiles = a.ntiles;
  mg.rounds = (a.ntiles + w8::kWaves - 1) / w8::kWaves;
  mg.pubx = a.pubx; mg.pub_ch = a.pub_ch;
  mg.hk = a.hk;
  mg.mask = L.sMask; mg.edge = L.sEdge; mg.em = L.sEm; mg.seg = L.sSeg; mg.soff = L.sOff; mg.sidx = L.sIdx;
  mg.row = L.sRow;
  mg.ncomp = __builtin_amdgcn_readfirstlane(L.sCmol[4]);
  mg.NR = a.N;
  return mg;
}
__device__ __forceinline__ int uni(int v) { return __builtin_amdgcn_readfirstlane(v); }
__device__ __forceinline__ unsigned uni(unsigned v) { return (unsigned)__builtin_amdgcn_readfirstlane((int)v); }
__device__ __forceinline__ float uni(float v) {
  return __builtin_bit_cast(float, __builtin_amdgcn_readfirstlane(__builtin_bit_cast(int, v)));
}
template <class T>
__device__ __forceinline__ T* uni(T* p) {
  const unsigned long long u = (unsigned long long)p;
  const unsigned lo = (unsigned)__builtin_amdgcn_readfirstlane((int)(unsigned)u);
  const unsigned hi = (unsigned)__builtin_amdgcn_readfirstlane((int)(unsigned)(u >> 32));
  return (T*)(((unsigned long long)hi << 32) | lo);
}
__device__ __forceinline__ Graph8Args uni(const Graph8Args& a) {
  return Graph8Args{uni(a.N), uni(a.D), uni(a.S), uni(a.NC), uni(a.ntiles), uni(a.pubx), uni(a.pub_ch), uni(a.hk)};
}
__device__ __forceinline__ EdmDev uni(const EdmDev& w) {
  return EdmDev{uni(w.w), uni(w.w_bytes), uni(w.F), uni(w.L), uni(w.S), uni(w.attention), uni(w.use_tanh), uni(w.coords_range),
                uni(w.norm_constant), uni(w.normf), uni(w.ktail), uni(w.ws), uni(w.ws_bytes), uni(w.hinv)};
}
__device__ __forceinline__ PredDev uni(const PredDev& w) {
  return PredDev{uni(w.w), uni(w.w_bytes), uni(w.F), uni(w.K), uni(w.L), uni(w.attention), uni(w.use_tanh), uni(w.coords_range_layer), uni(w.ktail), uni(w.ws),
                 uni(w.ws_bytes), uni(w.hinv)};
}
__device__ __forceinline__ float* lds_base() {
  extern __shared__ __attribute__((aligned(16))) float smem[];
  return smem;
}
__device__ __attribute__((noinline)) void vt_seed8(const VtDev* vt_, int b_, int srow_, int K_, int pred_off_) {
  const VtDev* const vt = uni(vt_);
  const int b = uni(b_), K = uni(K_), tid = threadIdx.x;
  float* const pred = lds_base() + uni(pred_off_);
  if (tid < K) {
    float* const tr = vt_trace_row(vt, b, K, uni(srow_));
    if (tr != nullptr) tr[tid] = pred[tid];
    pred[16 + tid] = target_seed(vt_row(vt, b, K), K, tid, pred[tid]);
  }
  __syncthreads();
}
__device__ __attribute__((noinline)) void vt_norm8(const VtDev* vt_, int b_, int srow_, int K_, int ND_, int grad_off_) {
  const VtDev* const vt = uni(vt_);
  const int K = uni(K_), ND = uni(ND_), tid = threadIdx.x;
  float* const tr = vt_trace_row(vt, uni(b_), K, uni(srow_));
  if (tr == nullptr || tid >= 64) return;
  const float* const g = lds_base() + uni(grad_off_);
  float s = 0.f;
  for (int e = tid; e < ND; e += 64) s += g[e] * g[e];
  for (int off = 32; off > 0; off >>= 1) s += __shfl_xor(s, off);
  if (tid == 0) tr[K] = sqrtf(s);
}
__device__ __attribute__((noinline)) void vt_clip8(const VtDev* vt_, int b_, int srow_, int K_, int mean_off_) {
  const VtDev* const vt = uni(vt_);
  const int K = uni(K_);
  float* const tr = vt_trace_row(vt, uni(b_), K, uni(srow_));
  if (tr != nullptr && threadIdx.x == 0) tr[K + 1] = (lds_base() + uni(mean_off_))[3];
}
#ifndef GAUDI_STAMPS
template <int HP, int SP, int GN = 0, bool FL = false>
__device__ __attribute__((noinline)) void edm8_call(EdmDev W_, Graph8Args ga_, float t_val_, float* gnode_ = nullptr) {
  extern __shared__ __attribute__((aligned(16))) float smem[];
  const EdmDev W = uni(W_);
  const Graph8Args ga = uni(ga_);
  const float t_val = uni(t_val_);
  const Lds8 L = carve_lds8(smem, ga.N, ga.D, ga.S);
  const w8::MolGraph mg = graph8(L, ga);
  w8::NetSmem<HP, SP, GN> sm;
  sm.carve(L.net, ga.N, ga.S, GN ? uni(gnode_) : nullptr);
  sm.hk = ga.hk ? smem + ga.hk : nullptr;
  w8::edm_forward<HP, SP, GN, FL>(W, mg, sm, L.sZ, L.sEps, L.sMean, t_val, (int)threadIdx.x);
}
template <int HP, int SP, bool MR, int GN = 0, bool FL = false, bool PG = false>
__device__ __attribute__((noinline)) void pred_fwd8_call(PredDev W_, Graph8Args ga_, float t_val_, float* stash_, float readout_div_,
                                                         float* gnode_ = nullptr) {
  extern __shared__ __attribute__((aligned(16))) float smem[];
  const PredDev W = uni(W_);
  const Graph8Args ga = uni(ga_);
  const Lds8 L = carve_lds8(smem, ga.N, ga.D, ga.S);
  const w8::MolGraph mg = graph8(L, ga);
  w8::PredSmem<HP, SP, GN, PG> sm;
  sm.carve(L.net, ga.N, ga.S, ga.pubx, (GN || PG) ? uni(gnode_) : nullptr);
  sm.hk = ga.hk ? smem + ga.hk : nullptr;
  w8::pred_forward<HP, SP, MR, GN, FL>(W, mg, sm, L.sZ, uni(t_val_), uni(stash_), uni(readout_div_), (int)threadIdx.x);
}
template <int HP, int SP, bool MR, int GN = 0, bool FL = false, bool PG = false>
__device__ __attribute__((noinline)) void pred_bwd8_call(PredDev W_, Graph8Args ga_, float* stash_, float readout_div_, int resume_,
                                                         float* gnode_ = nullptr) {
  extern __shared__ __attribute__((aligned(16))) float smem[];
  const PredDev W = uni(W_);
  const Graph8Args ga = uni(ga_);
  const Lds8 L = carve_lds8(smem, ga.N, ga.D, ga.S);
  const w8::MolGraph mg = graph8(L, ga);
  w8::PredSmem<HP, SP, GN, PG> sm;
  sm.carve(L.net, ga.N, ga.S, ga.pubx, (GN || PG) ? uni(gnode_) : nullptr);
  w8::pred_backward<HP, SP, MR, GN, FL>(W, mg, sm, uni(stash_), L.sEps , uni(readout_div_), ga.pub_ch, (int)threadIdx.x,
                        uni(resume_) ? L.sZ : nullptr);
}
#endif

template <int SP, bool MR = false, int GN = 0, bool FR = false, bool PG = false>
struct V8T {
  static constexpr bool kFL = MR || GN != 0 || FR;
  static constexpr int kThreads = w8::kThreads;
  static constexpr int kSplit = SP;
  static constexpr int kWaveCount = 8, kGN = GN, kEF = 2;
  static constexpr bool kMR = MR, kFR = FR, kPG = PG;
  using Graph = w8::MolGraph;
  __host__ __device__ static int graph_floats(int N, int S) { return 2 * S + align16(N) + align16((N + 1 + S + 1) / 2); }
  __device__ __forceinline__ static float* load_graph(const KParams& P, int b, float* base, const float* sMask, Graph& mg, int tid, int wave) {
    (void)wave;
    const int N = P.N, S = P.EW;
    uint32_t* sEdge = (uint32_t*)base; base += S;
    float* sEm = base; base += S;
    uint32_t* sSeg = (uint32_t*)base; base += align16(N);
    uint16_t* sOff = (uint16_t*)base;
    uint16_t* sIdx = sOff + (N + 1);
    base += align16((N + 1 + S + 1) / 2);
    for (int i = tid; i < N; i += kThreads) sSeg[i] = P.seginfo[b * N + i];
    for (int i = tid; i < N + 1; i += kThreads) sOff[i] = P.soff[(size_t)b * (N + 1) + i];
    for (int i = tid; i < S; i += kThreads) {
      sEdge[i] = P.edges[(size_t)b * S + i];
      sEm[i] = P.emask[(size_t)b * S + i];
      sIdx[i] = P.sidx[(size_t)b * S + i];
    }
    mg.N = N; mg.D = 3 + P.F; mg.S = S;
    mg.NC = P.ncols[b];
    mg.ntiles = P.npairs[b];
    mg.rounds = (mg.ntiles + w8::kWaves - 1) / w8::kWaves;
    mg.pubx = P.pubx;
    mg.pub_ch = P.pub_ch;
    mg.hk = P.hk_off;
    mg.mask = sMask; mg.edge = sEdge; mg.em = sEm; mg.seg = sSeg; mg.soff = sOff; mg.sidx = sIdx;
    return base;
  }
  __device__ __forceinline__ static void set_rows(Graph& mg, const int* row, int ncomp, int NR) { mg.row = row; mg.ncomp = ncomp; mg.NR = NR; }
  __device__ __forceinline__ static Graph8Args gargs(const Graph& mg) {
    return Graph8Args{mg.N, mg.D, mg.S, mg.NC, mg.ntiles, mg.pubx, mg.pub_ch, mg.hk};
  }
  static constexpr bool kGlobalNodes = GN != 0 || PG;
  template <int HP>
  __device__ __forceinline__ static void edm(const EdmDev& W, const Graph& mg, float* net, const float* sZ, float* sEps,
                                             float* sMean, float t_val, int tid STAMP_DECL, float* gnode) {
#ifdef GAUDI_STAMPS
    w8::NetSmem<HP, SP, GN> sm;
    sm.carve(net, mg.N, mg.S, GN ? uni(gnode) : nullptr);
    sm.hk = w8::lds_at(mg.hk);
    w8::edm_forward<HP, SP, GN>(W, mg, sm, sZ, sEps, sMean, t_val, tid STAMP_ARGS);
#else
    (void)net; (void)sZ; (void)sEps; (void)sMean; (void)tid;
    edm8_call<HP, SP, GN, kFL>(W, gargs(mg), t_val, gnode);
#endif
  }
  template <int HP>
  __device__ __forceinline__ static void guide(const PredDev& W, const Graph& mg, float* net, float* sZ, float* sGrad, float* sTmp,
                                               float* sMean, float t_val, float sigma, const float* target_w, float scale,
                                               float* pred_out, float readout_div, float* stash, int tid STAMP_DECL, int phase,
                                               const float* dpred_ext, float* gnode, const float* dz_ext, const VtDev* vt,
                                               int b, int srow) {
#ifdef GAUDI_STAMPS
    (void)vt; (void)b; (void)srow;
    (void)dz_ext;
    w8::guidance_update<HP, SP, MR, GN, PG>(W, mg, net, sZ, sGrad, sTmp, sMean, t_val, sigma, target_w, scale, pred_out, readout_div, stash,
                                            mg.pubx, mg.pub_ch, tid STAMP_ARGS, phase, dpred_ext, (GN || PG) ? uni(gnode) : nullptr);
#else
    (void)sTmp;
    w8::PredSmem<HP, SP, GN, PG> sm;
    sm.carve(net, mg.N, mg.S, mg.pubx, gnode);
    if (phase != 2) pred_fwd8_call<HP, SP, MR, GN, kFL, PG>(W, gargs(mg), t_val, stash, readout_div, gnode);
    if (vt != nullptr) vt_seed8(vt, b, srow, W.K, (int)(sm.pred - lds_base()));
    else w8::guidance_seed(W, sm, target_w, scale, pred_out, tid, phase, dpred_ext);
    if (phase == 1) return;
    pred_bwd8_call<HP, SP, MR, GN, kFL, PG>(W, gargs(mg), stash, readout_div, phase == 2 ? 1 : 0, gnode);
    if (dz_ext != nullptr) {
      for (int e = tid; e < mg.N * mg.D; e += kThreads) sGrad[e] += dz_ext[e];
      __syncthreads();
    }
    if (vt != nullptr) vt_norm8(vt, b, srow, W.K, mg.N * mg.D, (int)(sGrad - lds_base()));
    w8::guidance_apply(mg, sZ, sGrad, sMean, sigma, tid);
    if (vt != nullptr) vt_clip8(vt, b, srow, W.K, (int)(sMean - lds_base()));
#endif
  }
  template <int HP>
  __device__ __forceinline__ static void pred_entry(const PredDev& W, const Graph& mg, float* net, float* sZ, float* sGrad,
                                                    float* sTmp, float* sMean, float t_val, const float* dpred, bool want_grad,
                                                    float* pred_out, float readout_div, float* stash, int tid STAMP_DECL, float* gnode) {
    w8::predictor_entry<HP, SP, MR, GN, PG>(W, mg, net, sZ, sGrad, sTmp, sMean, t_val, dpred, want_grad, pred_out, readout_div, stash, mg.pubx,
                            mg.pub_ch, tid STAMP_ARGS, gnode);
  }
};
// ... 367 lines not shown
```

### gaudi_amd/csrc/w8_edm.h

```cpp
#pragma once
#include "edm_device.h"
#include "w8_common.h"
#include "w8_split.h"
#include "w8_nodes_f16.h"

namespace gaudi {
namespace w8 {

__host__ __device__ constexpr int gn_lds_buffers(int gn) { return gn == 2 ? 2 : 0; }
template <int HP, int SP = 0, int GN = 0>
struct NetSmem {
  static constexpr bool kGlobalNodes = GN != 0;
  float *h, *p, *q;
  float *agg, *agg1;
  float* ring;
  float *x, *x0;
  uint32_t *pmax, *qmax;
  float* hsc;
  f4* geo;
  float* d0;
  float* trans;
  float* vec;
  float* hk = nullptr;
  __host__ __device__ static int floats(int N, int S) {
// ... 11 lines not shown
    } else {
      p = nb; nb += N * LD;
      q = nb; nb += N * LD;
    }
    agg = nb; nb += N * LD;
    agg1 = nb; nb += N * LD;
    x = base; base += 4 * N;
    x0 = base; base += 4 * N;
    pmax = (uint32_t*)base; base += align4(N);
    qmax = (uint32_t*)base; base += align4(N);
    hsc = base; base += 96;
    geo = (f4*)base; base += S * 4;
    d0 = base; base += S;
    trans = base; base += S * 4;
    vec = base;
  }
};

template <class SM>
__device__ __forceinline__ void compute_geo(const SM& sm, const MolGraph& mg, float norm_constant, int tid, bool write_d0) {
  for (int slot = tid; slot < mg.ntiles * 16; slot += kThreads) {
    const uint32_t e = mg.edge[slot];
    const int i = ew_i(e), j = ew_j(e);
    const float dx = sm.x[4 * i + 0] - sm.x[4 * j + 0];
    const float dy = sm.x[4 * i + 1] - sm.x[4 * j + 1];
    const float dz = sm.x[4 * i + 2] - sm.x[4 * j + 2];
    const float r = dx * dx + dy * dy + dz * dz;
    if (write_d0) {
      sm.d0[slot] = r;
    } else {
      const float inv = 1.0f / (sqrtf(r + 1e-8f) + norm_constant);
      sm.geo[slot] = (f4){r, dx * inv, dy * inv, dz * inv};
    }
  }
}

template <class SM>
__device__ __forceinline__ void coord_update(const SM& sm, const MolGraph& mg, float normf, int tid) {
  for (int idx = tid; idx < mg.N * 3; idx += kThreads) {
    const int n = idx / 3, d = idx % 3;
    const uint32_t sg = mg.seg[n];
    const int st = sg >> 16, len = sg & 0xffff;
    float s = 0.f;
    for (int k = 0; k < len; ++k) s += sm.trans[(st + k) * 4 + d];
    sm.x[4 * n + d] = (sm.x[4 * n + d] + s / normf) * mg.mask[n];
  }
}

struct TileCols {
  bool active;
  int slot;
  int i, j;
  bool run_end;
  int part;
  float mk;
  RunMask rm;
};
__device__ __forceinline__ TileCols load_tile(const MolGraph& mg, int round, int wave, int c) {
  TileCols tc;
  const int tile = round * kWaves + wave;
  tc.active = __builtin_amdgcn_readfirstlane(tile < mg.ntiles ? 1 : 0) != 0;
  tc.slot = (tc.active ? tile : 0) * 16 + c;
  const uint32_t e = mg.edge[tc.slot];
  tc.i = ew_i(e);
  tc.j = ew_j(e);
  tc.run_end = ew_run_end(e);
  tc.part = ew_part(e);
  tc.mk = mg.em[tc.slot];
  tc.rm.set(c, ew_run_start(e));
  return tc;
}

template <int HP>
__device__ __forceinline__ void scatter_runs(f4 (&e)[HP / 16], const TileCols& tc, float* agg0, float* agg1, int g) {
  constexpr int T = HP / 16, LD = HP + 4;
  float* dst = (tc.part ? agg1 : agg0) + tc.i * LD + 4 * g;
#pragma unroll
  for (int t = 0; t < T; ++t) {
    const f4 s = seg_scan(e[t], tc.rm);
    if (tc.run_end) *(f4*)(dst + 16 * t) = s;
  }
}

template <int HP, int SP = 0, int GN = 0, bool FL = false>
__device__ __forceinline__ void edm_forward(const EdmDev& W, const MolGraph& mg, const NetSmem<HP, SP, GN>& sm, const float* sZ,
                                            float* sEps, float* sMean , float t_val, int tid STAMP_DECL) {
  constexpr int LD = HP + 4;
  constexpr int T = HP / 16;
  constexpr int PK = HP * HP;
  const int wave = __builtin_amdgcn_readfirstlane(tid >> 6), lane = tid & 63, c = lane & 15, g = lane >> 4;
  const int N = mg.N, D = mg.D, F = W.F, F1 = F + 1;
  EdmLayout lay{HP, F1, W.L, W.S};
  const float* __restrict__ w = W.w;
  const WBuf wb = make_wbuf(W.w, W.w_bytes);
  const WBuf wbe = SP ? make_wbuf(W.ws, W.ws_bytes) : wb;
  const bool tw = W.ktail != 0;

  for (int idx = tid; idx < N * 3; idx += kThreads) {
    const int n = idx / 3, d = idx % 3;
    const float v = sZ[n * D + d] * mg.mask[n];
    sm.x[4 * n + d] = v;
    sm.x0[4 * n + d] = v;
  }
  {
    const float* ew = w + lay.emb_w();
    const float* eb = w + lay.emb_b();
    for (int idx = tid; idx < N * HP; idx += kThreads) {
      const int n = idx / HP, f = idx % HP;
      float acc = 0.f;
      const float m = mg.mask[n];
      for (int k = 0; k < F; ++k) acc += gload(ew + f * F1 + k) * (sZ[n * D + 3 + k] * m);
      acc += gload(ew + f * F1 + F) * t_val;
      sm.h[n * LD + f] = acc + gload(eb + f);
    }
  }
  __syncthreads();
  compute_geo(sm, mg, 0.f, tid, true);
  typename EdgeRing<HP, SP>::type ring;
  er_init<HP>(ring, sm.ring, W.ktail != 0, W.ws, W.hinv);
  static_assert(SP == 0 || NodeMath<SP>::kF16, "the split edge GEMMs take their column scales from the fp16 node GEMMs' row maxima");
  constexpr bool NH = NodeMath<SP>::kF16;
  constexpr bool RI = node_ring_idle(HP, SP, GN);
  constexpr bool STG = GN && !NH;
  float* const xs0 = sm.ring;
  float* const xs1 = sm.ring + stage_stride(N * LD);
  if constexpr (!RI) er_start<HP>(ring, wbe, lay.gcl(0, 0) + 2 * PK, wave, lane);
  typename NodePFSel<HP, NH>::type pf;
  node_prefetch_x<HP, NH, kAheadOne>(pf, wb, wbe, lay.gcl(0, 0), mg.NC, wave, lane, tw);
  auto hctx = [&]() {
    if constexpr (NH) {
      if constexpr (RI) return node_ctx_h<HP>(sm.ring, EdgeRing<HP, SP>::kFloats, mg.NC, W.hinv, tw, sm.hsc);
      else return node_ctx_h<HP>(ring.slot(ring.par ^ 1), EdgeRing<HP, SP>::kFloats / 2, mg.NC, W.hinv, tw, sm.hsc);
    } else {
      return NodeCtxH{1.f, nullptr, nullptr, tw, nullptr};
    }
  };
  const bool keep = NH && sm.hk != nullptr;
  bool h_kept = false;
  constexpr int NV = (7 * HP + 16 + kThreads - 1) / kThreads;
  VecPF<NV> vpf;
  vec_prefetch<NV, kThreads>(vpf, wb, lay.gcl(0, 0) + 6 * PK, 7 * HP + 16, tid);
  STAMP(ST_EDM_IO);

  for (int l = 0; l < W.L; ++l) {
    compute_geo(sm, mg, W.norm_constant, tid, false);
    STAMP(ST_GEO);
    for (int s = 0; s < W.S; ++s) {
      const int G = lay.gcl(l, s);
      const int Wnext_edge = s + 1 < W.S ? lay.gcl(l, s + 1) + 2 * PK : lay.equ(l) + 2 * PK;
      if constexpr (STG) stage_rows(xs0, sm.h, N * LD, wave, lane);
      for (int idx = tid; idx < N * (LD / 4); idx += kThreads) {
        *(f4*)(sm.agg + 4 * idx) = splat(0.f);
        *(f4*)(sm.agg1 + 4 * idx) = splat(0.f);
      }
      if (tid < N) {
        sm.pmax[tid] = 0u;
        sm.qmax[tid] = 0u;
      }
      vec_commit<NV, kThreads>(vpf, sm.vec, 7 * HP + 16, tid);
      if constexpr (STG) stage_wait();
      else __syncthreads();
      STAMP(ST_STAGE);
      const float *cr = sm.vec, *cd = sm.vec + HP, *b1 = sm.vec + 2 * HP, *b2 = sm.vec + 3 * HP, *wa = sm.vec + 4 * HP,
                  *bn1 = sm.vec + 5 * HP, *bn2 = sm.vec + 6 * HP;
      const float ba = sm.vec[7 * HP];
      const float crmax = sm.vec[7 * HP + 1], cdmax = sm.vec[7 * HP + 2];
      {
        const NodeCtxH cx = keep ? node_ctx_keep<HP>(hctx(), sm.hk, mg.NC) : hctx();
        node_gemm_x<HP, EPI_NONE, false, GN, NH, kAheadOne, kAheadAll, FL>(wb, wbe, G, sm.h, xs0, !h_kept, -1, nullptr, nullptr, b1, sm.p, nullptr, nullptr, mg.NC,
                                                      wave, lane, tw, cx, pf, G + PK, nullptr, sm.pmax);
        h_kept = keep;
        node_gemm_x<HP, EPI_NONE, false, GN, NH, kAheadAll, kAheadOne, FL>(wb, wbe, G + PK, sm.h, xs0, false, -1, nullptr, nullptr, nullptr, sm.q, nullptr,
                                                      nullptr, mg.NC, wave, lane, tw, cx, pf,
                                                      G + 3 * PK, nullptr, sm.qmax);
      }
      STAMP(ST_NODE);
      __syncthreads();
      STAMP(ST_BARRIER);
      if constexpr (RI) er_start<HP>(ring, wbe, G + 2 * PK, wave, lane);
      for (int rd = 0; rd < mg.rounds; ++rd) {
        const TileCols tc = load_tile(mg, rd, wave, c);
        const f4 gg = sm.geo[tc.slot];
        f4 acc[T];
        const float d0v = sm.d0[tc.slot];
        const float ub = __builtin_bit_cast(float, sm.pmax[tc.i]) + __builtin_bit_cast(float, sm.qmax[tc.j]) + crmax * gg[0] + cdmax * fabsf(d0v);
        er_gemm_pq<HP>(acc, ring, wbe, G + 2 * PK, rd + 1 < mg.rounds ? G + 2 * PK : (RI ? -1 : Wnext_edge), b2, cr, cd,
                         sm.p + tc.i * LD + 4 * g, sm.q + tc.j * LD + 4 * g, gg[0], d0v, ub, tc.active, wave, lane STAMP_ARGS);
        STAMP(ST_EDGE);
        if (tc.active) {
          float sdot = 0.f;
#pragma unroll
          for (int t = 0; t < T; ++t) {
            const f4 m = silu4v(acc[t]);
            acc[t] = m;
            const f4 wv = *(const f4*)(wa + 16 * t + 4 * g);
            sdot += m[0] * wv[0] + m[1] * wv[1] + m[2] * wv[2] + m[3] * wv[3];
          }
          float a = 1.f;
          if (W.attention) a = sigmoid_f(reduce_groups(sdot) + ba);
          const float sc = a * tc.mk;
#pragma unroll
          for (int t = 0; t < T; ++t) acc[t] = acc[t] * sc;
          scatter_runs<HP>(acc, tc, sm.agg, sm.agg1, g);
        }
        STAMP(ST_EDGE_EPI);
      }
      __syncthreads();
      STAMP(ST_BARRIER);
      if constexpr (STG) stage_rows(xs0, sm.h, N * LD, wave, lane);
      for (int idx = tid; idx < N * (HP / 4); idx += kThreads) {
        const int n = idx / (HP / 4), f = 4 * (idx % (HP / 4));
        if constexpr (STG)
          *(f4*)(xs1 + n * LD + f) = (*(const f4*)(sm.agg + n * LD + f) + *(const f4*)(sm.agg1 + n * LD + f)) / W.normf;
        else
          *(f4*)(sm.agg + n * LD + f) = (*(const f4*)(sm.agg + n * LD + f) + *(const f4*)(sm.agg1 + n * LD + f)) / W.normf;
      }
      if constexpr (STG) stage_wait();
      else __syncthreads();
      STAMP(ST_MISC);
      node_gemm_x<HP, EPI_SILU, true, GN, NH, kAheadOne, kAheadOne, FL>(wb, wbe, G + 3 * PK, sm.h, xs0, !h_kept, G + 4 * PK, sm.agg, xs1, bn1, sm.p, nullptr, nullptr,
                                              mg.NC, wave, lane, tw, keep ? node_ctx_keep<HP>(hctx(), sm.hk, mg.NC) : hctx(), pf, G + 5 * PK);
      STAMP(ST_NODE);
      __syncthreads();
      STAMP(ST_BARRIER);
      vec_prefetch<NV, kThreads>(vpf, wb, s + 1 < W.S ? lay.gcl(l, s + 1) + 6 * PK : lay.equ(l) + 3 * PK,
                                 s + 1 < W.S ? 7 * HP + 16 : 5 * HP + 16, tid);
      if constexpr (STG) {
        stage_rows(xs0, sm.p, N * LD, wave, lane);
        stage_wait();
      }
      node_gemm_x<HP, EPI_RESIDUAL_MASK, false, GN, NH, kAheadOne, kAheadOne, FL>(wb, wbe, G + 5 * PK, sm.p, xs0, true, -1, nullptr, nullptr, bn2, sm.h, sm.h, mg.mask,
                                                       mg.NC, wave, lane, tw, hctx(), pf,
                                                       s + 1 < W.S ? lay.gcl(l, s + 1) : lay.equ(l));
      h_kept = false;
      STAMP(ST_NODE);
      __syncthreads();
      STAMP(ST_BARRIER);
    }
    {
      const int E = lay.equ(l);
      const int Wnext_edge = l + 1 < W.L ? lay.gcl(l + 1, 0) + 2 * PK : -1;
      vec_commit<NV, kThreads>(vpf, sm.vec, 5 * HP + 16, tid);
      if (tid < N) {
        sm.pmax[tid] = 0u;
        sm.qmax[tid] = 0u;
      }
      if constexpr (STG) {
        stage_rows(xs0, sm.h, N * LD, wave, lane);
        stage_wait();
      } else {
        __syncthreads();
      }
      STAMP(ST_STAGE);
      const float *cr = sm.vec, *cd = sm.vec + HP, *b1 = sm.vec + 2 * HP, *b2 = sm.vec + 3 * HP, *w3 = sm.vec + 4 * HP;
      const float crmax = sm.vec[5 * HP], cdmax = sm.vec[5 * HP + 1];
      {
        const NodeCtxH cx = keep ? node_ctx_keep<HP>(hctx(), sm.hk, mg.NC) : hctx();
        node_gemm_x<HP, EPI_NONE, false, GN, NH, kAheadOne, kAheadAll, FL>(wb, wbe, E, sm.h, xs0, !h_kept, -1, nullptr, nullptr, b1, sm.p, nullptr, nullptr, mg.NC,
                                                      wave, lane, tw, cx, pf, E + PK, nullptr, sm.pmax);
        h_kept = keep;
        node_gemm_x<HP, EPI_NONE, false, GN, NH, kAheadAll, kAheadOne, FL>(wb, wbe, E + PK, sm.h, xs0, false, -1, nullptr, nullptr, nullptr, sm.q, nullptr,
                                                      nullptr, mg.NC, wave, lane, tw, cx, pf, l + 1 < W.L ? lay.gcl(l + 1, 0) : -1, nullptr,
                                                      sm.qmax);
      }
      STAMP(ST_NODE);
      __syncthreads();
      STAMP(ST_BARRIER);
      if constexpr (RI) er_start<HP>(ring, wbe, E + 2 * PK, wave, lane);
      for (int rd = 0; rd < mg.rounds; ++rd) {
        const TileCols tc = load_tile(mg, rd, wave, c);
        const f4 gg = sm.geo[tc.slot];
        f4 acc[T];
        const float d0v = sm.d0[tc.slot];
        const float ub = __builtin_bit_cast(float, sm.pmax[tc.i]) + __builtin_bit_cast(float, sm.qmax[tc.j]) + crmax * gg[0] + cdmax * fabsf(d0v);
        er_gemm_pq<HP>(acc, ring, wbe, E + 2 * PK, rd + 1 < mg.rounds ? E + 2 * PK : (RI ? -1 : Wnext_edge), b2, cr, cd,
                         sm.p + tc.i * LD + 4 * g, sm.q + tc.j * LD + 4 * g, gg[0], d0v, ub, tc.active, wave, lane STAMP_ARGS);
        STAMP(ST_EDGE);
        if (tc.active) {
          float sdot = 0.f;
#pragma unroll
          for (int t = 0; t < T; ++t) {
            const f4 m = silu4v(acc[t]);
            const f4 wv = *(const f4*)(w3 + 16 * t + 4 * g);
            sdot += m[0] * wv[0] + m[1] * wv[1] + m[2] * wv[2] + m[3] * wv[3];
          }
          const float phi = reduce_groups(sdot);
          const float tau = (W.use_tanh ? tanhf(phi) * W.coords_range : phi) * tc.mk;
          if (g == 0) *(f4*)(sm.trans + 4 * tc.slot) = (f4){gg[1] * tau, gg[2] * tau, gg[3] * tau, 0.f};
        }
        STAMP(ST_EDGE_EPI);
      }
      if (l + 1 < W.L) vec_prefetch<NV, kThreads>(vpf, wb, lay.gcl(l + 1, 0) + 6 * PK, 7 * HP + 16, tid);
      __syncthreads();
      STAMP(ST_BARRIER);
      coord_update(sm, mg, W.normf, tid);
      __syncthreads();
      STAMP(ST_MISC);
    }
  }

  {
    const float* ow = w + lay.out_w();
    const float* ob = w + lay.out_b();
    int bad = 0;
// ... 52 lines not shown
```

### gaudi_amd/csrc/w8_nodes_f16.h

```cpp
#pragma once
#include "w8_split.h"

namespace gaudi {
namespace w8 {


constexpr float kLoScale = 2048.f;
#ifndef GAUDI_NODE_ABLATE
#define GAUDI_NODE_ABLATE 0
#endif
constexpr int kAblateH = GAUDI_NODE_ABLATE;
#ifndef GAUDI_NODE_STAMPS
#define GAUDI_NODE_STAMPS 0
#endif
#ifndef GAUDI_NODE_PRIO
#define GAUDI_NODE_PRIO 1
#endif
struct NodeStampH {
  unsigned long long sum[8], last;
  __device__ __forceinline__ void start() { last = __builtin_amdgcn_s_memtime(); }
  __device__ __forceinline__ void mark(int i) {
    const unsigned long long t = __builtin_amdgcn_s_memtime();
    sum[i] += t - last;
    last = t;
  }
};
#if GAUDI_NODE_STAMPS
#define NSTAMP(i) do { if (ns != nullptr) ns->mark(i); } while (0)
#else
#define NSTAMP(i) do { } while (0)
#endif

__device__ __forceinline__ f4 mfma_h(const u4 a, const u4 b, const f4 c) {
  return __builtin_amdgcn_mfma_f32_16x16x32_f16(__builtin_bit_cast(h8, a), __builtin_bit_cast(h8, b), c, 0, 0, 0);
}

__host__ __device__ constexpr bool nh_odd(int HP) { return ((HP / 16) & 1) != 0; }
__host__ __device__ constexpr int nh_chunks(int HP) { return HP / 32; }
__host__ __device__ constexpr int nh_chunk_floats(int HP) { return (HP / 16) * 2 * 256; }
__host__ __device__ constexpr int nh_tail_off(int HP) { return nh_chunks(HP) * nh_chunk_floats(HP); }
__host__ __device__ constexpr int nh_tail_steps(bool ktail) { return ktail ? 1 : 4; }
__host__ __device__ constexpr int nh_chunk_stride(int nct) { return nct * 512 + (nct == 1 ? 16 : 0); }
__host__ __device__ constexpr int nh_split_floats(int HP, int nct) {
  return nh_chunks(HP) * nh_chunk_stride(nct) + (nh_odd(HP) ? nct * 256 : 0);
}
constexpr int kScaleFloatsH = 48;

struct SplitBufH {
  float* base;
  int nct;
  float* sc;
  __device__ __forceinline__ float* chunk(int m) const { return base + m * nh_chunk_stride(nct); }
  __device__ __forceinline__ float* tail(int HP) const { return base + nh_chunks(HP) * nh_chunk_stride(nct); }
  __device__ __forceinline__ float* scale(int) const { return sc; }
};

__device__ __forceinline__ uint32_t wave_max_u32(uint32_t v) {
  auto shr = [](uint32_t x, auto sh_tag) {
    constexpr int SH = decltype(sh_tag)::value;
    return (uint32_t)__builtin_amdgcn_update_dpp(0, (int)x, 0x110 + SH, 0xF, 0xF, true);
  };
  v = umax(v, shr(v, std::integral_constant<int, 1>{}));
  v = umax(v, shr(v, std::integral_constant<int, 2>{}));
  v = umax(v, shr(v, std::integral_constant<int, 4>{}));
  v = umax(v, shr(v, std::integral_constant<int, 8>{}));
  const uint32_t a = __builtin_amdgcn_readlane((int)v, 15), b = __builtin_amdgcn_readlane((int)v, 31),
                 c = __builtin_amdgcn_readlane((int)v, 47), d = __builtin_amdgcn_readlane((int)v, 63);
  return umax(umax(a, b), umax(c, d));
}


__host__ __device__ constexpr int nh_bpos(int c, int g) { return (16 * g + (c ^ g)) * 4; }
struct SplitRowH {
  f4 x;
  uint32_t mx;
};
template <int HP>
__device__ __forceinline__ SplitRowH split_row_load(const float* X, int n, int lane) {
  constexpr int LD = HP + 4;
  SplitRowH r;
  r.x = lane < HP / 4 ? *(const f4*)(X + n * LD + 4 * lane) : splat(0.f);
  r.mx = umax(umax(absbits(r.x[0]), absbits(r.x[1])), umax(absbits(r.x[2]), absbits(r.x[3])));
  return r;
}
template <int HP>
__device__ __forceinline__ void split_row_store(const SplitBufH& sb, const f4 x, uint32_t mx, int n, int lane) {
  constexpr int T = HP / 16, nc = nh_chunks(HP);
  const int m = lane >> 3, g = (lane >> 1) & 3, half = lane & 1;
  int k = 141 - (int)(mx >> 23);
  k = k > 126 ? 126 : k;
  const float s = __builtin_bit_cast(float, (uint32_t)(k + 127) << 23), inv = __builtin_bit_cast(float, (uint32_t)(127 - k) << 23);
  const float y0 = x[0] * s, y1 = x[1] * s, y2 = x[2] * s, y3 = x[3] * s;
  const uint32_t h01 = pk_f16(y0, y1), h23 = pk_f16(y2, y3);
  const f2 f01 = unpk_f16(h01), f23 = unpk_f16(h23);
  const uint32_t l01 = pk_f16((y0 - f01[0]) * kLoScale, (y1 - f01[1]) * kLoScale),
                 l23 = pk_f16((y2 - f23[0]) * kLoScale, (y3 - f23[1]) * kLoScale);
  const int ct = n >> 4, c = n & 15;
  if (m < nc) {
    float* d = sb.chunk(m) + ct * 512 + nh_bpos(c, g) + half * 2;
    *(u2*)d = (u2){h01, h23};
    *(u2*)(d + 256) = (u2){l01, l23};
  } else if (nh_odd(HP) && lane < HP / 4) {
    float* d = sb.tail(HP) + ct * 256 + 4 * (lane - 4 * (T - 1)) * 16 + c;
    d[0] = x[0];
    d[16] = x[1];
    d[32] = x[2];
    d[48] = x[3];
  }
  if (lane == 0) sb.scale(HP)[ct * 16 + c] = inv;
}
template <int HP>
__device__ __forceinline__ void split_rows_h(const SplitBufH& sb, const float* X, int N, int wave, int lane) {
  for (int n = wave; n < N; n += 2 * kWaves) {
    const int n2 = n + kWaves < N ? n + kWaves : n;
    SplitRowH a = split_row_load<HP>(X, n, lane), b = split_row_load<HP>(X, n2, lane);
    a.mx = wave_max_u32(a.mx);
    b.mx = wave_max_u32(b.mx);
    split_row_store<HP>(sb, a.x, a.mx, n, lane);
    if (n2 != n) split_row_store<HP>(sb, b.x, b.mx, n2, lane);
  }
}

__device__ __forceinline__ void lds_barrier() {
  asm volatile("s_waitcnt lgkmcnt(0)" ::: "memory");
  __builtin_amdgcn_s_barrier();
  asm volatile("" ::: "memory");
}

#ifndef GAUDI_NODE_DEPTH
#define GAUDI_NODE_DEPTH 3
#endif
#ifndef GAUDI_NODE_LATE
#define GAUDI_NODE_LATE 0
#endif
template <int HP>
struct NodeGeoH {
  static constexpr int T = HP / 16;
  static constexpr int NTW = T > kWaves ? 2 : 1;
  static constexpr int nc = nh_chunks(HP);
  static constexpr int D = nc < GAUDI_NODE_DEPTH ? (nc > 0 ? nc : 1) : GAUDI_NODE_DEPTH;
  static constexpr bool odd = nh_odd(HP);
};
template <int NTW>
struct NodeSetH {
  u4 p[NTW][2];
};
template <int HP>
struct NodePFH {
  NodeSetH<NodeGeoH<HP>::NTW> s[NodeGeoH<HP>::D];
};

constexpr int kOOBBytes = (int)0x80000000u;
template <int HP>
struct TileLanesH {
  int vo[NodeGeoH<HP>::NTW];
  __device__ __forceinline__ TileLanesH(int wave, int lane, bool on = true) {
#pragma unroll
    for (int u = 0; u < NodeGeoH<HP>::NTW; ++u)
      vo[u] = (on && wave + kWaves * u < NodeGeoH<HP>::T) ? lane * 16 + (wave + kWaves * u) * 2048 : kOOBBytes;
  }
};
template <int HP>
__device__ __forceinline__ void nh_load(NodeSetH<NodeGeoH<HP>::NTW>& s, const WBuf& wh, int chunk_off, const TileLanesH<HP>& tl) {
#pragma unroll
  for (int u = 0; u < NodeGeoH<HP>::NTW; ++u) {
    s.p[u][0] = __builtin_bit_cast(u4, __builtin_amdgcn_raw_buffer_load_b128(wh.r, tl.vo[u], chunk_off * 4, GAUDI_NODE_LOAD_AUX));
    s.p[u][1] = __builtin_bit_cast(u4, __builtin_amdgcn_raw_buffer_load_b128(wh.r, tl.vo[u] + 1024, chunk_off * 4, GAUDI_NODE_LOAD_AUX));
  }
}
constexpr int kAheadOne = 1, kAheadAll = 99;
template <int HP, int AHEAD = kAheadAll>
__device__ __forceinline__ void node_prefetch_h(NodePFH<HP>& pf, const WBuf& wh, int W , int wave, int lane) {
  constexpr int nd = AHEAD < NodeGeoH<HP>::D ? AHEAD : NodeGeoH<HP>::D;
  const TileLanesH<HP> tl(wave, lane);
  static_for<nd>([&](auto d_tag) {
    constexpr int d = decltype(d_tag)::value;
    nh_load<HP>(pf.s[d], wh, 2 * W + d * nh_chunk_floats(HP), tl);
  });
}

struct NodeCtxH {
  float winv;
  float* split_a;
  float* split_b;
  bool ktail;
  float* scales;
  float* scales_b = nullptr;
};

template <int HP, int EPI, bool TWO, int MAXNT, int PIN = kAheadOne, int POUT = kAheadOne, bool FL = false>
__device__ __forceinline__ void node_gemm_h(const WBuf& wh, int Wa, const float* sXa, bool do_split_a, int Wb, const float* sXb,
                                            const float* sBias, float* sY, const float* sRes, const float* sMask, int N, int wave,
                                            int lane, const NodeCtxH& cx, NodePFH<HP>& pf, int nextW = -1, float* gPre = nullptr,
                                            uint32_t* sMaxOut = nullptr ,
                                            NodeStampH* ns = nullptr) {
  (void)ns;
  using G = NodeGeoH<HP>;
  constexpr int T = G::T, LD = HP + 4, NTW = G::NTW, nc = G::nc, D = G::D;
  constexpr int kIn = PIN < D ? PIN : D, kOut = POUT < D ? POUT : D;
  constexpr int kLate = nc < D ? 0 : (GAUDI_NODE_LATE < kOut ? GAUDI_NODE_LATE : kOut);
  const int c = lane & 15, g = lane >> 4;
  const int nt = (MAXNT < 2 || N <= 16) ? 1 : (MAXNT < 3 || N <= 32) ? 2 : 3;
  const bool seq = TWO && cx.split_b == cx.split_a;
  const SplitBufH sa{cx.split_a, nt, cx.scales}, sb{cx.split_b, nt, cx.scales_b != nullptr ? cx.scales_b : cx.scales + kScaleFloatsH};
  const int bpos = nh_bpos(c, g);
  const TileLanesH<HP> tl(wave, lane);
  const TileLanesH<HP> tl_next(wave, lane, nextW >= 0);
  const int Wn = nextW >= 0 ? nextW : Wa;
  static_for<D>([&](auto d_tag) {
    constexpr int d = decltype(d_tag)::value;
    if constexpr (d >= kIn) nh_load<HP>(pf.s[d], wh, 2 * Wa + d * nh_chunk_floats(HP), tl);
  });
  float ta[NTW][4], tb[NTW][4];
  if constexpr (G::odd) {
#pragma unroll
    for (int u = 0; u < NTW; ++u) {
      const int t = wave + kWaves * u < T ? wave + kWaves * u : 0;
#pragma unroll
      for (int q = 0; q < 4; ++q) {
        const int ln = ((q == 0 || !cx.ktail) && wave + kWaves * u < T) ? lane : kOOBLane;
        ta[u][q] = __builtin_bit_cast(float, __builtin_amdgcn_raw_buffer_load_b32(wh.r, ln * 4, (2 * Wa + nh_tail_off(HP) + t * 256 + q * 64) * 4, 0));
        if constexpr (TWO)
          tb[u][q] = __builtin_bit_cast(float, __builtin_amdgcn_raw_buffer_load_b32(wh.r, ln * 4, (2 * Wb + nh_tail_off(HP) + t * 256 + q * 64) * 4, 0));
      }
    }
  }
  NSTAMP(0);
  if (!(kAblateH & 1)) {
    const int ls = FL ? fresh(lane) : lane;
    if (do_split_a) split_rows_h<HP>(sa, sXa, N, wave, ls);
    if (TWO && !seq) split_rows_h<HP>(sb, sXb, N, wave, ls);
    NSTAMP(1);
    if (do_split_a || (TWO && !seq)) lds_barrier();
    NSTAMP(2);
  }

  f4 acc0[MAXNT][NTW], acc1[MAXNT][NTW], y[MAXNT][NTW];
#pragma unroll
  for (int j = 0; j < MAXNT; ++j)
#pragma unroll
    for (int u = 0; u < NTW; ++u) {
      const int t = wave + kWaves * u < T ? wave + kWaves * u : 0;
      acc0[j][u] = splat(0.f);
      acc1[j][u] = splat(0.f);
      y[j][u] = sBias != nullptr ? *(const f4*)(sBias + 16 * t + 4 * g) : splat(0.f);
    }
  struct BH {
    u4 h, l;
  };
  auto bld = [&](const SplitBufH& s_, int i, int j) {
    const float* q = s_.chunk(i) + bpos + j * 512;
    return BH{*(const u4*)q, *(const u4*)(q + 256)};
  };
  auto mm = [&](const NodeSetH<NTW>& s, const BH& b, int j) {
    if (kAblateH & 2) {
      asm volatile("" ::"v"(s.p[0][0]), "v"(s.p[0][1]), "v"(s.p[NTW - 1][0]), "v"(s.p[NTW - 1][1]), "v"(b.h), "v"(b.l));
      return;
    }
#pragma unroll
    for (int u = 0; u < NTW; ++u) acc1[j][u] = mfma_h(s.p[u][0], b.l, acc1[j][u]);
#pragma unroll
    for (int u = 0; u < NTW; ++u) acc0[j][u] = mfma_h(s.p[u][0], b.h, acc0[j][u]);
#pragma unroll
    for (int u = 0; u < NTW; ++u) acc1[j][u] = mfma_h(s.p[u][1], b.h, acc1[j][u]);
  };
  auto fold = [&](const SplitBufH& s_, const float (&tw)[NTW][4]) {
    static_for<MAXNT>([&](auto j_tag) {
      constexpr int j = decltype(j_tag)::value;
      if (j < nt) {
        if constexpr (G::odd) {
          const float* xt = s_.tail(HP) + j * 256 + g * 16 + c;
#pragma unroll
          for (int u = 0; u < NTW; ++u) y[j][u] = mfma1(tw[u][0], xt[0], y[j][u]);
          if (!cx.ktail) {
#pragma unroll
            for (int q = 1; q < 4; ++q)
#pragma unroll
              for (int u = 0; u < NTW; ++u) y[j][u] = mfma1(tw[u][q], xt[64 * q], y[j][u]);
          }
        }
        const float sc = s_.scale(HP)[j * 16 + c] * cx.winv;
#pragma unroll
        for (int u = 0; u < NTW; ++u) {
          y[j][u] = y[j][u] + (acc0[j][u] + acc1[j][u] * (1.0f / kLoScale)) * sc;
          acc0[j][u] = splat(0.f);
          acc1[j][u] = splat(0.f);
        }
      }
    });
  };
  auto source = [&](auto src_tag, const SplitBufH& s_) {
    constexpr int src = decltype(src_tag)::value;
    constexpr bool last_src = !TWO || src == 1;
    const int Wcur = src == 0 ? Wa : Wb;
    BH bcur = bld(s_, 0, 0);
    static_for<nc>([&](auto i_tag) {
      constexpr int i = decltype(i_tag)::value;
      constexpr int d = i % D;
      BH bnext = bcur;
      if constexpr (i + 1 < nc) bnext = bld(s_, i + 1, 0);
      __builtin_amdgcn_sched_barrier(0);
      mm(pf.s[d], bcur, 0);
      if constexpr (MAXNT >= 2) {
        if (nt >= 2) {
          mm(pf.s[d], bld(s_, i, 1), 1);
          if constexpr (MAXNT >= 3) {
            if (nt >= 3) mm(pf.s[d], bld(s_, i, 2), 2);
          }
        }
      }
      __builtin_amdgcn_sched_barrier(0);
      if (!(kAblateH & 4)) {
        if constexpr (i + D < nc) nh_load<HP>(pf.s[d], wh, 2 * Wcur + (i + D) * nh_chunk_floats(HP), tl);
        else if constexpr (!last_src) nh_load<HP>(pf.s[d], wh, 2 * Wb + d * nh_chunk_floats(HP), tl);
        else if constexpr (d < kOut - kLate) nh_load<HP>(pf.s[d], wh, 2 * Wn + d * nh_chunk_floats(HP), tl_next);
      }
      __builtin_amdgcn_sched_barrier(0);
      bcur = bnext;
    });
  };
  auto late = [&](auto d_tag) {
    constexpr int d = decltype(d_tag)::value;
    if constexpr (d >= kOut - kLate && d < kOut) {
      __builtin_amdgcn_sched_barrier(0);
      if (!(kAblateH & 4)) nh_load<HP>(pf.s[d], wh, 2 * Wn + d * nh_chunk_floats(HP), tl_next);
      __builtin_amdgcn_sched_barrier(0);
    }
  };
  NSTAMP(3);
#if GAUDI_NODE_PRIO
  if constexpr (!FL)
    if ((GAUDI_NODE_PRIO == 1 && wave >= kWaves / 2) || (GAUDI_NODE_PRIO == 2 && wave < kWaves / 2)) __builtin_amdgcn_s_setprio(1);
#endif
  source(std::integral_constant<int, 0>{}, sa);
  NSTAMP(4);
  if constexpr (!TWO) late(std::integral_constant<int, kOut - kLate>{});
  fold(sa, ta);
  NSTAMP(5);
  if constexpr (TWO) {
    if (seq) {
      lds_barrier();
      split_rows_h<HP>(sb, sXb, N, wave, FL ? fresh(lane) : lane);
      lds_barrier();
    }
    source(std::integral_constant<int, 1>{}, sb);
    late(std::integral_constant<int, kOut - kLate>{});
    fold(sb, tb);
  }
  static_for<D>([&](auto d_tag) {
    if constexpr (decltype(d_tag)::value > kOut - kLate) late(d_tag);
  });
#if GAUDI_NODE_PRIO
  if constexpr (!FL) __builtin_amdgcn_s_setprio(0);
#endif
  const int le = FL ? fresh(lane) : lane, ce = le & 15, ge = le >> 4;
  static_for<MAXNT>([&](auto j_tag) {
    constexpr int j = decltype(j_tag)::value;
    if (j < nt) {
#pragma unroll
      for (int u = 0; u < NTW; ++u) {
        const int t = wave + kWaves * u;
        const int nd = j * 16 + ce;
        f4 yy = y[j][u];
        if (t < T && nd < N) {
          float* dst = sY + nd * LD + 16 * t + 4 * ge;
          const bool pad = G::odd && cx.ktail && t == T - 1 && ge > 0;
          if (pad) yy = splat(0.f);
          if (gPre != nullptr) nstash_store((f4*)(gPre + nd * HP + 16 * t + 4 * ge), yy);
          if (sMaxOut != nullptr) atomicMax(sMaxOut + nd, umax(umax(absbits(yy[0]), absbits(yy[1])), umax(absbits(yy[2]), absbits(yy[3]))));
          if (!pad) {
            if (EPI == EPI_SILU) yy = silu4v(yy);
            if (EPI == EPI_RESIDUAL_MASK) {
              const f4 r = *(const f4*)(sRes + nd * LD + 16 * t + 4 * ge);
              yy = (r + yy) * sMask[nd];
            }
            if (EPI == EPI_MUL_DSILU) {
              const f4 r = *(const f4*)(sRes + nd * LD + 16 * t + 4 * ge);
              yy = yy * dsilu4v(r);
            }
            if (EPI == EPI_ACCUM) yy = *(const f4*)(sRes + nd * LD + 16 * t + 4 * ge) + yy;
          }
          *(f4*)dst = yy;
        }
      }
    }
  });
  NSTAMP(6);
}

#ifndef GAUDI_NODE_F16
#define GAUDI_NODE_F16 1
#endif
template <int SP>
struct NodeMath {
  static constexpr bool kF16 = SP != 0 && GAUDI_NODE_F16 != 0;
};
template <int HP, bool NH>
struct NodePFSel {
  using type = NodePF<HP>;
};
template <int HP>
struct NodePFSel<HP, true> {
  using type = NodePFH<HP>;
};
template <int HP, bool NH, int AHEAD, class PF>
__device__ __forceinline__ void node_prefetch_x(PF& pf, const WBuf& wb, const WBuf& wbe, int W, int N, int wave, int lane, bool tw) {
  if constexpr (NH) node_prefetch_h<HP, AHEAD>(pf, wbe, W, wave, lane);
  else node_prefetch<HP>(pf, wb, W, wave, lane, tw);
}
template <int HP, int EPI, bool TWO, int GN, bool NH, int PIN, int POUT, bool FL = false, class PF>
__device__ __forceinline__ void node_gemm_x(const WBuf& wb, const WBuf& wbe, int Wa, const float* Xa, const float* XaS, bool split_a, int Wb,
                                            const float* Xb, const float* XbS, const float* sBias, float* sY, const float* sRes,
                                            const float* sMask, int N, int wave, int lane, bool tw, const NodeCtxH& cx, PF& pf,
                                            int nextW = -1, float* gPre = nullptr, uint32_t* sMaxOut = nullptr) {
  if constexpr (NH) {
    node_gemm_h<HP, EPI, TWO, GN ? 3 : 2, PIN, POUT, FL>(wbe, Wa, Xa, split_a, Wb, Xb, sBias, sY, sRes, sMask, N, wave, lane, cx, pf, nextW, gPre,
                                                         sMaxOut);
  } else if constexpr (GN != 0) {
    node_gemm_n<HP, EPI, true, 3>(wb, Wa, XaS, Wb, XbS, sBias, sY, sRes, sMask, N, wave, lane, tw, &pf, nextW, gPre);
  } else {
    node_gemm<HP, EPI, true>(wb, Wa, Xa, Wb, Xb, sBias, sY, sRes, sMask, N, wave, lane, tw, &pf, nextW, gPre);
  }
}
__host__ __device__ constexpr bool node_ring_idle(int HP, int SP, bool GN) {
  return GN || (SP != 0 && GAUDI_NODE_F16 != 0 && (SP == 2 || HP < 48));
}
template <int HP>
__device__ __forceinline__ NodeCtxH node_ctx_h(float* region, int cap, int N, float winv, bool ktail, float* scales) {
  const int nct = N <= 16 ? 1 : N <= 32 ? 2 : 3;
  const int need = nh_split_floats(HP, nct);
  return NodeCtxH{winv, region, 2 * need <= cap ? region + need : region, ktail, scales};
}
__host__ __device__ constexpr int nh_keep_floats(int HP, int N) { return nh_split_floats(HP, N <= 16 ? 1 : N <= 32 ? 2 : 3) + kScaleFloatsH; }
template <int HP>
__device__ __forceinline__ NodeCtxH node_ctx_keep(const NodeCtxH& cx, float* keep, int N) {
  const int nct = N <= 16 ? 1 : N <= 32 ? 2 : 3;
  return NodeCtxH{cx.winv, keep + kScaleFloatsH, cx.split_a, cx.ktail, keep, cx.scales};
  (void)nct;
}

}
}
```

### gaudi_amd/csrc/w8_pred.h

```cpp
#pragma once
#include "pred_device.h"
#include "w8_edm.h"

namespace gaudi {
namespace w8 {

template <int HP, int SP = 0, int GN = 0, bool PG = false>
struct PredSmem {
  static_assert(!(PG && GN != 0), "PG is a variant of the resident kernels");
  static_assert(!GN || SP != 0, "global node buffers: split edge GEMMs only (the fp32 form's publish buffer starts in b0 / b1)");
  static constexpr bool kGlobalNodes = GN != 0;
  float *b2, *b3, *b4;
  float *b0, *b1;
  float* ring;
  float* pub;
  float *x, *x0, *dx;
  uint32_t *pmax, *qmax;
  float* hsc;
  f4* geo;
  float *d0, *trans, *dd0;
  float* pred;
  float* vec;
  float* hk = nullptr;
  __host__ __device__ static int floats(int N, int S, int pubx) {
    return EdgeRing<HP, SP>::kFloats + (GN ? gn_lds_buffers(GN) : PG ? 4 : 5) * N * (HP + 4) + pubx + 12 * N + 2 * align4(N) + 96 + S * 10 + 32 + 10 * HP;
  }
  __device__ __forceinline__ float* publish() const { return GN ? ring : b0; }
  __device__ void carve(float* base, int N, int S, int pubx, float* gnode = nullptr) {
    constexpr int LD = HP + 4;
    if (SP == 0) { ring = base; base += EdgeRing<HP, SP>::kFloats; }
    if (GN || PG) gnode = assume_global(gnode);
    float*& nb = GN ? gnode : base;
    if (GN == 2) { b2 = base; base += N * LD; } else { b2 = nb; nb += N * LD; }
    b3 = nb; nb += N * LD;
    if (PG) { b4 = gnode; gnode += N * LD; } else { b4 = nb; nb += N * LD; }
    b0 = nb; nb += N * LD;
    if (GN == 2) { b1 = base; base += N * LD; } else { b1 = nb; nb += N * LD; }
    if (SP != 0) { ring = base; base += EdgeRing<HP, SP>::kFloats; }
    pub = base; base += pubx;
    x = base; base += 4 * N;
    x0 = base; base += 4 * N;
    dx = base; base += 4 * N;
    pmax = (uint32_t*)base; base += align4(N);
    qmax = (uint32_t*)base; base += align4(N);
    hsc = base; base += 96;
    geo = (f4*)base; base += S * 4;
    d0 = base; base += S;
    trans = base; base += S * 4;
    dd0 = base; base += S;
    pred = base; base += 32;
    vec = base;
  }
};

__host__ __device__ inline long long pred_stash_floats8(int N, int HP, int L, int S) {
  return pred_stash_node_floats(N, HP, L) + (long long)L * S * HP * 2 + 2LL * L * S + (S > 16 * kWaves ? (long long)S * HP : 0);
}
__device__ __forceinline__ size_t edge_stash_off8(int l, int tile, int arr, int S, int HP) {
  return (((size_t)l * (S / 16) + tile) * 2 + arr) * (size_t)(16 * HP);
}

__host__ __device__ inline int pub_chunk_tiles(int S, long long avail_floats, int T) {
  int ch = (int)((avail_floats / (S > 0 ? S : 1) - 4) / 16);
  return ch > T ? T : ch;
}

template <int HP, int SP = 0, bool MR = false, int GN = 0, bool FL = false, class SM = PredSmem<HP, SP, GN>>
__device__ __forceinline__ void pred_forward(const PredDev& W, const MolGraph& mg, const SM& sm, const float* sZ,
                                             float t_val, float* stash, float readout_div, int tid STAMP_DECL) {
  constexpr int LD = HP + 4;
  constexpr int T = HP / 16;
  const int wave = __builtin_amdgcn_readfirstlane(tid >> 6), lane = tid & 63, c = lane & 15, g = lane >> 4;
  const int N = mg.N, D = mg.D, F = W.F, F1 = F + 1, K = W.K, S = mg.S;
  PredLayout lay{HP, F1, K, W.L};
  const float* __restrict__ w = W.w;
  const WBuf wb = make_wbuf(W.w, W.w_bytes);
  const WBuf wbe = SP ? make_wbuf(W.ws, W.ws_bytes) : wb;
  const bool tw = W.ktail != 0;
  float *h = sm.b0, *p = sm.b1, *q = sm.b2, *agg = sm.b3, *agg1 = sm.b4;
  float* estash = stash + pred_stash_node_floats(N, HP, W.L);
  float* astash = estash + (size_t)W.L * S * HP * 2;
  float* pstash = astash + (size_t)W.L * S;

  for (int idx = tid; idx < N * 3; idx += kThreads) {
    const int n = idx / 3, d = idx % 3;
    const float v = sZ[n * D + d] * mg.mask[n];
    sm.x[4 * n + d] = v;
    sm.x0[4 * n + d] = v;
  }
  {
    const float* ew = w + lay.emb_w();
    const float* eb = w + lay.emb_b();
    for (int idx = tid; idx < N * HP; idx += kThreads) {
      const int n = idx / HP, f = idx % HP;
      float acc = 0.f;
      const float m = mg.mask[n];
      for (int k = 0; k < F; ++k) acc += gload(ew + f * F1 + k) * (sZ[n * D + 3 + k] * m);
      acc += gload(ew + f * F1 + F) * t_val;
      h[n * LD + f] = acc + gload(eb + f);
    }
  }
  __syncthreads();
  compute_geo(sm, mg, 0.f, tid, true);
  typename EdgeRing<HP, SP>::type ring;
  er_init<HP>(ring, sm.ring, W.ktail != 0, W.ws, W.hinv);
  constexpr bool NH = NodeMath<SP>::kF16;
  constexpr bool RI = node_ring_idle(HP, SP, GN);
  constexpr bool STG = GN && !NH;
  float* const xs0 = sm.ring;
  float* const xs1 = sm.ring + stage_stride(N * LD);
  if constexpr (!RI) er_start<HP>(ring, wbe, lay.layer(0) + 2 * HP * HP, wave, lane);
  typename NodePFSel<HP, NH>::type pf;
  node_prefetch_x<HP, NH, kAheadOne>(pf, wb, wbe, lay.layer(0), mg.NC, wave, lane, tw);
  auto hctx = [&]() {
    if constexpr (NH) {
      if constexpr (RI) return node_ctx_h<HP>(sm.ring, EdgeRing<HP, SP>::kFloats, mg.NC, W.hinv, tw, sm.hsc);
      else return node_ctx_h<HP>(ring.slot(ring.par ^ 1), EdgeRing<HP, SP>::kFloats / 2, mg.NC, W.hinv, tw, sm.hsc);
    } else {
      return NodeCtxH{1.f, nullptr, nullptr, tw, nullptr};
    }
  };
  const bool keep = NH && sm.hk != nullptr;
  constexpr int NV = (PredLayerW::vec_count(HP) + kThreads - 1) / kThreads;
  VecPF<NV> vpf;
  vec_prefetch<NV, kThreads>(vpf, wb, PredLayerW::vec_off(lay.layer(0), HP), PredLayerW::vec_count(HP), tid);

  for (int l = 0; l < W.L; ++l) {
    const bool last = l == W.L - 1;
    const PredLayerW Lw(w, lay.layer(l), HP, sm.vec);
    vec_commit<NV, kThreads>(vpf, sm.vec, PredLayerW::vec_count(HP), tid);
    if constexpr (STG) stage_rows(xs0, h, N * LD, wave, lane);
    for (int idx = tid; idx < N * LD; idx += kThreads) {
      agg[idx] = 0.f;
      agg1[idx] = 0.f;
    }
    if (tid < N) {
      sm.pmax[tid] = 0u;
      sm.qmax[tid] = 0u;
    }
    float* st = stash + (size_t)l * (3 * N * HP + 4 * N);
    for (int idx = tid; idx < N; idx += kThreads) gstore4((f4*)(st + 3 * N * HP) + idx, *(const f4*)(sm.x + 4 * idx));
    compute_geo(sm, mg, 1.0f, tid, false);
    if constexpr (STG) stage_wait();
    else __syncthreads();
    STAMP(ST_STAGE);
    {
      const NodeCtxH cx = keep ? node_ctx_keep<HP>(hctx(), sm.hk, mg.NC) : hctx();
      node_gemm_x<HP, EPI_NONE, false, GN, NH, kAheadOne, kAheadAll, FL>(wb, wbe, Lw.A, h, xs0, true, -1, nullptr, nullptr, Lw.b1, p, nullptr, nullptr, mg.NC, wave,
                                                    lane, tw, cx, pf, Lw.Bm, nullptr, sm.pmax);
      node_gemm_x<HP, EPI_NONE, false, GN, NH, kAheadAll, kAheadOne, FL>(wb, wbe, Lw.Bm, h, xs0, false, -1, nullptr, nullptr, nullptr, q, nullptr, nullptr, mg.NC,
                                                    wave, lane, tw, cx, pf, Lw.Wn1h, nullptr, sm.qmax);
    }
    STAMP(ST_NODE);
    __syncthreads();
    STAMP(ST_BARRIER);
    if constexpr (RI) er_start<HP>(ring, wbe, Lw.W2, wave, lane);
    for (int idx = tid; idx < N * (HP / 4); idx += kThreads) {
      const int n = idx / (HP / 4), f = 4 * (idx % (HP / 4));
      nstash_store((f4*)st + idx, *(const f4*)(p + n * LD + f));
      nstash_store((f4*)(st + N * HP) + idx, *(const f4*)(q + n * LD + f));
    }
    STAMP(ST_STASH);
    int rd = 0;
    {
    pred_fwd_round:
      const bool more = MR && rd + 1 < mg.rounds;
      const TileCols tc = load_tile(mg, MR ? rd : 0, wave, c);
      const f4 gg = sm.geo[tc.slot];
      f4 acc[T];
      const float d0f = sm.d0[tc.slot];
      const float ub = __builtin_bit_cast(float, sm.pmax[tc.i]) + __builtin_bit_cast(float, sm.qmax[tc.j]) + sm.vec[9 * HP + 1] * gg[0] +
                       sm.vec[9 * HP + 2] * fabsf(d0f);
      er_gemm_pq<HP>(acc, ring, wbe, Lw.W2, last ? (more ? Lw.W2 : -1) : Lw.Wc1, Lw.b2, Lw.cr, Lw.cd, p + tc.i * LD + 4 * g,
                       q + tc.j * LD + 4 * g, gg[0], d0f, ub, tc.active, wave, lane STAMP_ARGS);
      STAMP(ST_EDGE);
      const int tile = tc.slot >> 4;
      if (tc.active) {
        {
          f4* sv = (f4*)(estash + edge_stash_off8(l, tile, 0, S, HP)) + lane;
#pragma unroll
          for (int t = 0; t < T; ++t) stash_store(sv + t * 64, acc[t]);
        }
        float sdot = 0.f;
#pragma unroll
        for (int t = 0; t < T; ++t) {
          const f4 m = silu4v(acc[t]);
          acc[t] = m;
          sdot += dot4(m, *(const f4*)(Lw.wa + 16 * t + 4 * g));
        }
        float a = 1.f;
        if (W.attention) a = sigmoid_f(reduce_groups(sdot) + Lw.ba);
        if (g == 0) gstore(astash + (size_t)l * S + tc.slot, a);
        const float sc = a * tc.mk;
#pragma unroll
        for (int t = 0; t < T; ++t) acc[t] = acc[t] * sc;
        scatter_runs<HP>(acc, tc, agg, agg1, g);
      }
      STAMP(ST_EDGE_EPI);
      if (!last) {
        f4 cp[T];
        er_gemm_regs<HP>(cp, acc, ring, wbe, Lw.Wc1, more ? Lw.W2 : (RI ? -1 : lay.layer(l + 1) + 2 * HP * HP), Lw.bc1, nullptr,
                         tc.active, wave, lane);
        STAMP(ST_EDGE);
        if (tc.active) {
          f4* sc = (f4*)(estash + edge_stash_off8(l, tile, 1, S, HP)) + lane;
          float sdot = 0.f;
#pragma unroll
          for (int t = 0; t < T; ++t) {
            const f4 sg = sigmoid4v(cp[t]);
            const f4 ds = sg * (splat(1.0f) + cp[t] * (splat(1.0f) - sg)), sl = cp[t] * sg;
            stash_store(sc + t * 64, ds);
            sdot += dot4(sl, *(const f4*)(Lw.wc2 + 16 * t + 4 * g));
          }
          const float phi = reduce_groups(sdot);
          if (g == 0) gstore(pstash + (size_t)l * S + tc.slot, phi);
          const float tau = (W.use_tanh ? tanhf(phi) * W.coords_range_layer : phi) * tc.mk;
          if (g == 0) *(f4*)(sm.trans + 4 * tc.slot) = (f4){gg[1] * tau, gg[2] * tau, gg[3] * tau, 0.f};
        }
        STAMP(ST_EDGE_EPI);
      }
      if constexpr (MR) {
        if (++rd < mg.rounds) goto pred_fwd_round;
      }
    }
    __syncthreads();
    STAMP(ST_BARRIER);
    if constexpr (STG) stage_rows(xs0, h, N * LD, wave, lane);
    for (int idx = tid; idx < N * (HP / 4); idx += kThreads) {
      const int n = idx / (HP / 4), f = 4 * (idx % (HP / 4));
      if constexpr (STG)
        *(f4*)(xs1 + n * LD + f) = *(const f4*)(agg + n * LD + f) + *(const f4*)(agg1 + n * LD + f);
      else
        *(f4*)(agg + n * LD + f) = *(const f4*)(agg + n * LD + f) + *(const f4*)(agg1 + n * LD + f);
    }
    if constexpr (STG) stage_wait();
    else __syncthreads();
    STAMP(ST_MISC);
    node_gemm_x<HP, EPI_SILU, true, GN, NH, kAheadOne, kAheadOne, FL>(wb, wbe, Lw.Wn1h, h, xs0, !keep, Lw.Wn1a, agg, xs1, Lw.bn1, p, nullptr, nullptr, mg.NC, wave, lane,
                                            tw, keep ? node_ctx_keep<HP>(hctx(), sm.hk, mg.NC) : hctx(), pf, Lw.Wn2, st + 2 * N * HP );
    STAMP(ST_NODE);
    __syncthreads();
    STAMP(ST_BARRIER);
    vec_prefetch<NV, kThreads>(vpf, wb, PredLayerW::vec_off(lay.layer(l + 1 < W.L ? l + 1 : l), HP), PredLayerW::vec_count(HP), tid);
    if constexpr (STG) {
      stage_rows(xs0, p, N * LD, wave, lane);
      stage_wait();
    }
    node_gemm_x<HP, EPI_RESIDUAL_MASK, false, GN, NH, kAheadOne, kAheadOne, FL>(wb, wbe, Lw.Wn2, p, xs0, true, -1, nullptr, nullptr, Lw.bn2, h, h, mg.mask, mg.NC, wave,
                                                     lane, tw, hctx(), pf, l + 1 < W.L ? lay.layer(l + 1) : -1);
    if (!last) coord_update(sm, mg, 1.0f, tid);
    STAMP(ST_NODE);
    __syncthreads();
    STAMP(ST_BARRIER);
  }
  {
    const float* ow = w + lay.out_w();
    const float* ob = w + lay.out_b();
    const float* msk = mg.mask;
    small_dots<kThreads>(
        N * K, HP, tid, [=](int qq, int f) { return gload(ow + (qq % K) * HP + f); },
        [=](int qq, int f) { return h[(qq / K) * LD + f]; },
        [=](int qq, float acc) { p[qq] = (acc + gload(ob + qq % K)) * msk[qq / K]; });
    __syncthreads();
    if (tid < K) {
      float s = 0.f;
      for (int n = 0; n < N; ++n) s += p[n * K + tid];
      sm.pred[tid] = s / readout_div;
    }
    __syncthreads();
  }
  STAMP(ST_X0);
}

template <int HP, int SP = 0, bool MR = false, int GN = 0, bool FL = false, class SM = PredSmem<HP, SP, GN>>
__device__ __forceinline__ void pred_backward(const PredDev& W, const MolGraph& mg, const SM& sm, const float* stash,
                                              float* sGrad, float readout_div, int pub_ch, int tid STAMP_DECL, const float* sZin = nullptr) {
  constexpr int LD = HP + 4;
  constexpr int T = HP / 16;
  const int wave = __builtin_amdgcn_readfirstlane(tid >> 6), lane = tid & 63, c = lane & 15, g = lane >> 4;
  const int N = mg.N, D = mg.D, F = W.F, F1 = F + 1, K = W.K, S = mg.S;
  PredLayout lay{HP, F1, K, W.L};
  const float* __restrict__ w = W.w;
  const WBuf wb = make_wbuf(W.w, W.w_bytes);
  const WBuf wbe = SP ? make_wbuf(W.ws, W.ws_bytes) : wb;
  const bool tw = W.ktail != 0;
  float *B0 = sm.b0, *B1 = sm.b1, *B2 = sm.b2, *dh = sm.b3, *B4 = sm.b4;
  const int tid_ = tid;
  float* pub = sm.publish();
  const int PLD = 16 * pub_ch + 4;
  const float* estash = stash + pred_stash_node_floats(N, HP, W.L);
  const float* astash = estash + (size_t)W.L * S * HP * 2;
  const float* pstash = astash + (size_t)W.L * S;
  const float* dpred = sm.pred + 16;
  const int nslots = mg.ntiles * 16;
  f4* dus = (f4*)const_cast<float*>(pstash + (size_t)W.L * S);

  if (sZin != nullptr) {
    for (int idx = tid; idx < N * 3; idx += kThreads) {
      const int n = idx / 3, d = idx % 3;
      const float v = sZin[n * D + d] * mg.mask[n];
      sm.x[4 * n + d] = v;
      sm.x0[4 * n + d] = v;
    }
    __syncthreads();
    compute_geo(sm, mg, 0.f, tid, true);
    __syncthreads();
  }
  {
    const float* ow = w + lay.out_w();
    for (int idx = tid; idx < N * HP; idx += kThreads) {
      const int n = idx / HP, f = idx % HP;
      float acc = 0.f;
      for (int k = 0; k < K; ++k) acc += (dpred[k] / readout_div) * gload(ow + k * HP + f);
      dh[n * LD + f] = acc * mg.mask[n];
    }
    for (int idx = tid; idx < N * 4; idx += kThreads) sm.dx[idx] = 0.f;
    for (int idx = tid; idx < S; idx += kThreads) sm.dd0[idx] = 0.f;
  }
  __syncthreads();

  typename EdgeRing<HP, SP>::type ring;
  er_init<HP>(ring, sm.ring, W.ktail != 0, W.ws, W.hinv);
  constexpr bool NH = NodeMath<SP>::kF16;
  constexpr bool RI = node_ring_idle(HP, SP, GN);
  constexpr bool STG = GN && !NH;
  float* const xs0 = sm.ring;
  float* const xs1 = sm.ring + stage_stride(N * LD);
  if constexpr (!RI) {
    const int L0 = lay.layer(W.L - 1);
    er_start<HP>(ring, wbe, L0 + 9 * HP * HP , wave, lane);
  }
  typename NodePFSel<HP, NH>::type pf;
  node_prefetch_x<HP, NH, kAheadOne>(pf, wb, wbe, lay.layer(W.L - 1) + 13 * HP * HP , mg.NC, wave, lane, tw);
  auto hctx = [&]() {
    if constexpr (NH) {
      if constexpr (RI) return node_ctx_h<HP>(sm.ring, EdgeRing<HP, SP>::kFloats, mg.NC, W.hinv, tw, sm.hsc);
      else return node_ctx_h<HP>(ring.slot(ring.par ^ 1), EdgeRing<HP, SP>::kFloats / 2, mg.NC, W.hinv, tw, sm.hsc);
    } else {
      return NodeCtxH{1.f, nullptr, nullptr, tw, nullptr};
    }
  };
  constexpr int NV = (PredLayerW::vec_count(HP) + kThreads - 1) / kThreads;
  VecPF<NV> vpf;
  vec_prefetch<NV, kThreads>(vpf, wb, PredLayerW::vec_off(lay.layer(W.L - 1), HP), PredLayerW::vec_count(HP), tid);
  STAMP(ST_X1);
  for (int l = W.L - 1; l >= 0; --l) {
    const bool last = l == W.L - 1;
    const PredLayerW Lw(w, lay.layer(l), HP, sm.vec);
    const float* st = stash + (size_t)l * (3 * N * HP + 4 * N);
    {
      const int tid = fresh(tid_);
      const int n4 = N * (HP / 4);
#ifdef GAUDI_DIAG_HOT_STASH
      const f4* sp = (const f4*)W.w;
      const f4* sq = (const f4*)(W.w + N * HP);
      const f4* sn = (const f4*)(W.w + 2 * N * HP);
#else
// ... 351 lines not shown
```

### gaudi_amd/engine.py

```python
from __future__ import annotations

import ctypes as C

import numpy as np

from . import _lib
from ._lib import TARGET_CB, TARGET_CBZ, Diag, EdmConfig, GaudiError, PredConfig, f32, fptr


def _strip(sd: dict) -> dict:
    out = {}
    for k, v in sd.items():
        if hasattr(v, "detach"):
            v = v.detach().cpu().numpy()
        out[k[7:] if k.startswith("module.") else k] = f32(v)
    return out


def _noise_power(schedule: str) -> float:
    if schedule == "cosine":
        return 0.0
    parts = str(schedule).split("_")
    try:
        power = float(parts[1]) if len(parts) == 2 and parts[0] == "polynomial" else 0.0
# ... 50 lines not shown
        if sc.shape != ((B,) if per else ()):
            raise GaudiError(f"target spec 'scale' must be a number or [B] = {(B,)}, got {sc.shape}")
        sc = np.ascontiguousarray(sc.reshape(-1))
        keep.append(sc)
        cs.scale = sc.ctypes.data_as(_lib.FP)
        cs.scale_per_mol = 1 if per else 0
    win = spec.get("window")
    if win is not None:
        cs.t_lo, cs.t_hi = int(win[0]), int(win[1])
        if cs.t_lo == 0 and cs.t_hi == 0:
            raise GaudiError("the guidance window must lie inside 1..T")
    return cs, keep


def host_target_seed(spec, pred) -> np.ndarray:
    p = f32(pred)
    if p.ndim != 2:
        raise GaudiError(f"pred must be [B,K], got {p.shape}")
    B, K = p.shape
    cs, keep = target_spec(spec, B, K)
    out = np.empty_like(p)
    rc = _lib.load_library().gaudi_host_target_seed(C.byref(cs), B, K, fptr(p), fptr(out))
    del keep
    if rc != 0:
        raise GaudiError(f"gaudi_host_target_seed failed ({rc}): side must be -1 / 0 / +1 and every parameter finite")
    return out


class Engine:
    def __init__(self, device: int = 0):
        self.lib = _lib.load_library()
        self.h = C.c_void_p()
        rc = self.lib.gaudi_create(int(device), C.byref(self.h))
        if rc != 0:
            raise GaudiError(f"gaudi_create(device={device}) failed with code {rc} (no usable HIP device?)")
        self.device = device
        self.edm_args = None
        self.pred_args = None
        self.fix_noise = False
        self.F = None
        self.K = None

    _default = None

    @classmethod
    def default(cls, device: int = 0) -> "Engine":
        if cls._default is None or not cls._default.h:
            cls._default = cls(device)
        return cls._default

    def close(self):
        if getattr(self, "h", None) is not None and self.h:
            self.lib.gaudi_destroy(self.h)
            self.h = C.c_void_p()

    def __del__(self):
        try:
            self.close()
        except Exception:
            pass

    def _warning(self):
        fn = getattr(self.lib, "gaudi_last_warning", None)
        if fn is None or fn.restype is not C.c_char_p:
            return ""
        msg = fn(self.h)
        return msg.decode() if msg else ""

    def _note_fallback(self):
        w = self._warning()
        if w and w != getattr(self, "_fallback_reason", None):
            import warnings
            warnings.warn("gaudi_amd: " + w, RuntimeWarning, stacklevel=3)
        if w:
            self._fallback_reason = w

    def profile_clock_mhz(self) -> float:
        fn = getattr(self.lib, "gaudi_profile_clock", None)
        if fn is None or not fn.argtypes:
            return 0.0
        v = C.c_double(0.0)
        self._check(fn(self.h, C.byref(v)), "gaudi_profile_clock")
        return float(v.value)

    def keep_h(self) -> int:
        fn = getattr(self.lib, "gaudi_last_keep_h", None)
        if fn is None or not fn.argtypes:
            return 0
        n = C.c_int32(0)
        self._check(fn(self.h, C.byref(n)), "gaudi_last_keep_h")
        return int(n.value)

    def family_split(self) -> int:
        fn = getattr(self.lib, "gaudi_last_family_split", None)
        if fn is None or not fn.argtypes:
            return 0
        n = C.c_int32(0)
        self._check(fn(self.h, C.byref(n)), "gaudi_last_family_split")
        return int(n.value)

    def _check(self, rc: int, what: str):
        if rc != 0:
            msg = self.lib.gaudi_last_error(self.h)
            raise GaudiError(f"{what} failed ({rc}): {msg.decode() if msg else ''}")

    def _tensor_args(self, sd: dict):
        names = list(sd.keys())
        arrs = [sd[k] for k in names]
        n = len(names)
        c_names = (C.c_char_p * n)(*[k.encode() for k in names])
        c_ptrs = (_lib.FP * n)(*[fptr(a) for a in arrs])
        c_numel = (C.c_int64 * n)(*[a.size for a in arrs])
        return n, c_names, c_ptrs, c_numel, arrs

    def load_edm(self, args: dict, state_dict: dict):
        agg = args.get("aggregation_method", "sum")
        if agg not in ("sum", "mean"):
            raise GaudiError(f"unknown aggregation_method {agg!r}")
        sd = _strip(state_dict)
        emb = sd.get("dynamics.egnn.embedding.weight")
        if emb is None:
            raise GaudiError("state dict has no dynamics.egnn.embedding.weight (mode='gnn_dynamics' is unsupported)")
        F = emb.shape[1] - 1
        from .checkpoint import normalize_factors
        nv = normalize_factors(args)
        cfg = EdmConfig(F, int(args["nf"]), int(args["n_layers"]), int(args.get("inv_sublayers", 1)),
                        int(bool(args["attention"])), int(bool(args["tanh"])), float(args["coords_range"]),
                        float(args["norm_constant"]), float(args.get("normalization_factor", 1)) if agg == "sum" else 0.0,
                        int(args["diffusion_steps"]), _noise_power(args["diffusion_noise_schedule"]),
                        float(args["diffusion_noise_precision"]), (C.c_float * 3)(*[float(v) for v in nv]),
                        int(bool(args.get("sin_embedding", False))))
        n, c_names, c_ptrs, c_numel, keep = self._tensor_args(sd)
        self._check(self.lib.gaudi_load_edm(self.h, C.byref(cfg), n, c_names, c_ptrs, c_numel), "gaudi_load_edm")
        self._note_fallback()
        self.edm_args, self.F, self.T = dict(args), F, int(args["diffusion_steps"])
        self.edm_names = list(sd.keys())
        self.edm_shapes = [sd[k].shape for k in self.edm_names]
        self._edm_train_sd = None
        sigma_0 = float(np.sqrt(1.0 / (1.0 + np.exp(-np.float64(self.gamma()[0])))))
        max_norm = max(float(nv[1]), float(nv[2]))
        if sigma_0 * 8 > 1.0 / max_norm:
            raise GaudiError(f"Value for normalization value {max_norm} probably too large with sigma_0 {sigma_0:.5f} and "
                             f"1 / norm_value = {1.0 / max_norm} (en_diffusion.py:336-349: the reference raises the same)")

    def load_predictor(self, args: dict, state_dict: dict):
        sd = _strip(state_dict)
        emb = sd["egnn.embedding.weight"]
        F = emb.shape[1] - 1
        K = sd["egnn.embedding_out.weight"].shape[0]
        cfg = PredConfig(F, K, int(args["nf"]), int(args["n_layers"]), int(bool(args["attention"])),
                         int(bool(args["tanh"])), float(args["coords_range"]))
        n, c_names, c_ptrs, c_numel, keep = self._tensor_args(sd)
        self._check(self.lib.gaudi_load_predictor(self.h, C.byref(cfg), n, c_names, c_ptrs, c_numel),
                    "gaudi_load_predictor")
        reason = getattr(self, "_fallback_reason", None)
        if reason and reason.startswith("predictor weights") and self._warning() != reason:
            self._fallback_reason = None
        self._note_fallback()
        self.pred_args, self.K = dict(args), K
        self.pred_names = list(sd.keys())
        self.pred_shapes = [sd[k].shape for k in self.pred_names]

    edm_sync = None

    def _sync_edm(self, sampler: bool = True):
        if self.edm_sync is not None:
# ... 510 lines not shown
```

### include/gaudi_hip.h

```cpp
#ifndef GAUDI_HIP_H
#define GAUDI_HIP_H

#include <stdint.h>

#ifdef __cplusplus
extern "C" {
#endif

#define GAUDI_OK 0
#define GAUDI_E_INVALID (-1)
#define GAUDI_E_HIP (-2)
#define GAUDI_E_STATE (-3)
#define GAUDI_E_MISSING (-4)
#define GAUDI_E_CAPACITY (-5)

typedef struct gaudi_handle gaudi_handle;

typedef struct {
  int32_t in_node_nf;
  int32_t hidden_nf;
  int32_t n_layers;
  int32_t inv_sublayers;
  int32_t attention;
  int32_t tanh;
  float coords_range;
  float norm_constant;
  float normalization_factor;
  int32_t diffusion_steps;
  float noise_power;
  float noise_precision;
  float norm_values[3];
  int32_t sin_embedding;
} gaudi_edm_config;

typedef struct {
  int32_t in_nf;
  int32_t out_nf;
  int32_t hidden_nf;
  int32_t n_layers;
  int32_t attention;
  int32_t tanh;
  float coords_range;
} gaudi_pred_config;

typedef struct {
  float max_masked_leak;
  float max_cog_rel;
  float max_cog_abs;
  int32_t nan_count;
  int32_t reprojected;
} gaudi_diag;

int gaudi_create(int device, gaudi_handle** out);
void gaudi_destroy(gaudi_handle* h);
const char* gaudi_last_error(const gaudi_handle* h);
const char* gaudi_last_warning(const gaudi_handle* h);
#define GAUDI_ABI_VERSION 7
int gaudi_abi_version(void);

int gaudi_load_edm(gaudi_handle* h, const gaudi_edm_config* cfg, int n, const char* const* names,
                   const float* const* tensors, const int64_t* numel);
int gaudi_load_predictor(gaudi_handle* h, const gaudi_pred_config* cfg, int n, const char* const* names,
                         const float* const* tensors, const int64_t* numel);

int gaudi_get_gamma(gaudi_handle* h, float* gamma_out );
int gaudi_get_step_coefficients(gaudi_handle* h, float* coef_out );

int gaudi_phi(gaudi_handle* h, int B, int N, const float* z, const float* t ,
              const float* node_mask, const float* edge_mask, float* eps_out);

int gaudi_predictor_fwd(gaudi_handle* h, int B, int N, const float* z, const float* t ,
                        const float* node_mask, const float* edge_mask, float* pred_out );
int gaudi_predictor_grad(gaudi_handle* h, int B, int N, const float* z, const float* t, const float* node_mask,
                         const float* edge_mask, const float* dpred , float* pred_out ,
                         float* grad_out );

int gaudi_predict_noised(gaudi_handle* h, int B, int N, const float* x, const float* onehot, const int32_t* t_int,
                         const float* node_mask, const float* edge_mask, uint64_t seed, int64_t sample_offset,
                         const float* noise, float* zt_out , float* pred_out );

int gaudi_predictor_loss_grad(gaudi_handle* h, int B, int N, const float* x, const float* onehot, const int32_t* t_int,
                              const float* node_mask, const float* edge_mask, const float* y , uint64_t seed,
                              int64_t sample_offset, const float* noise , float* loss_out ,
                              float* pred_out , float* grad_out, int32_t* has_grad_out);
int gaudi_predictor_grad_size(gaudi_handle* h, int64_t* n_floats);

int gaudi_edm_loss_grad(gaudi_handle* h, int B, int N, const float* x, const float* onehot, const int32_t* t_int,
                        const float* node_mask, const float* edge_mask, uint64_t seed, int64_t sample_offset,
                        const float* noise , int loss_type, const float* weight ,
                        float* loss_out , float* net_out , float* grad_out ,
                        int32_t* has_grad_out);
int gaudi_edm_grad_size(gaudi_handle* h, int64_t* n_floats);
int gaudi_edm_set_train_weights(gaudi_handle* h, int n, const char* const* names, const float* const* tensors,
                                const int64_t* numel);

int gaudi_edm_nll(gaudi_handle* h, int B, int N, const float* x, const float* onehot, const int32_t* t_int, const float* node_mask,
                  const float* edge_mask, uint64_t seed, int64_t sample_offset, const float* noise ,
                  float* nll_out , float* terms_out );

int gaudi_step(gaudi_handle* h, int B, int N, int s_idx, const float* z_t, const float* node_mask,
               const float* edge_mask, const float* eps_raw, const float* target_w ,
               float scale, float* zs_out);

int gaudi_decode(gaudi_handle* h, int B, int N, const float* z0, const float* node_mask, const float* edge_mask,
                 const float* eps_raw, float* x_out , float* onehot_out );

int gaudi_sample(gaudi_handle* h, int B, int N, const float* node_mask, const float* edge_mask, uint64_t seed,
                 int64_t sample_offset, const float* noise, float std, const float* target_w ,
                 float scale, float* x_out , float* onehot_out ,
                 float* z0_out , gaudi_diag* diag );

int gaudi_sample_grid(gaudi_handle* h, int B, int N, const float* node_mask, const float* edge_mask, uint64_t seed,
                      int64_t sample_offset, const float* noise, float std, const float* target_w , float scale,
                      int n_grid, const int32_t* grid, const float* x0 , const float* onehot0 ,
                      float* x_out, float* onehot_out, float* z0_out , float* zt_out ,
                      gaudi_diag* diag );

typedef struct {
  int32_t K;
  const float* w;
  const float* q;
  const float* c;
  const int32_t* side;
  const float* scale;
  int32_t w_per_mol, q_per_mol, c_per_mol, side_per_mol, scale_per_mol;
  int32_t t_lo, t_hi;
} gaudi_target_spec;

int gaudi_sample_target(gaudi_handle* h, int B, int N, const float* node_mask, const float* edge_mask, uint64_t seed,
                        int64_t sample_offset, const float* noise, float std, const gaudi_target_spec* spec, int n_grid,
                        const int32_t* grid , const float* x0 , const float* onehot0 ,
                        float* x_out, float* onehot_out, float* z0_out , float* zt_out ,
                        float* trace_out , gaudi_diag* diag );
int gaudi_step_target(gaudi_handle* h, int B, int N, int s_idx, int t_idx, const float* z_t, const float* node_mask,
                      const float* edge_mask, const float* eps_raw, const gaudi_target_spec* spec, float* zs_out,
                      float* trace_out );
int gaudi_host_target_seed(const gaudi_target_spec* spec, int B, int K, const float* pred, float* out);

int gaudi_step_pair(gaudi_handle* h, int B, int N, int s_idx, int t_idx, const float* z_t, const float* node_mask,
// ... 136 lines not shown
```

Baseline: 216.5.

## Add one-tile node-GEMM kernel variant and fuse aggregate sum into GEMM loads

Adds an N1 kernel variant for small molecules (at most 16 node slots) that compiles the fp16 node GEMM with a single row tile and a compile-time odd-K tail. It also fuses the agg+agg1 sum (and the normalisation divide in the EDM) into the GEMM's row loads, which removes a separate LDS pass and a barrier. New kernel instantiations are added for the 192/208 hidden sizes, plus a last-kernel-key query for diagnostics. The cost is more template variants and code size, and a fallback to the old kernel when no N1 instance exists.

```diff
diff --git a/gaudi_amd/_lib.py b/gaudi_amd/_lib.py
--- a/gaudi_amd/_lib.py
+++ b/gaudi_amd/_lib.py
@@ -124,6 +124,7 @@
                                            C.POINTER(C.c_int32), C.POINTER(C.c_int32)]),
     "gaudi_set_plan_hint": (C.c_int, [C.c_void_p, C.c_int32, C.c_int32]),
     "gaudi_last_warning": (C.c_char_p, [C.c_void_p]),
+    "gaudi_last_kernel_key": (C.c_int, [C.c_void_p, C.c_char_p, C.c_int]),
     "gaudi_abi_version": (C.c_int, []),
     "gaudi_last_family_split": (C.c_int, [C.c_void_p, C.POINTER(C.c_int32)]),
     "gaudi_profile_clock": (C.c_int, [C.c_void_p, C.POINTER(C.c_double)]),
@@ -164,6 +165,7 @@
 _GRID_EXPORTS = ("gaudi_sample_grid", "gaudi_step_pair", "gaudi_sample_cb_grid")
 _TARGET_EXPORTS = ("gaudi_sample_target", "gaudi_step_target")
 _ATOMS_EXPORTS = ("gaudi_rings_to_atoms", "gaudi_atoms_profile_get")
+_KEY_EXPORTS = ("gaudi_last_kernel_key",)
 
 _lib = None
 
@@ -185,7 +187,7 @@
         raise GaudiError(f"{LIB_PATH} exports ABI version {abi}, this package expects {ABI_VERSION}: rebuild it "
                          "(`python -m gaudi_amd.build --force`)")
     for name, (res, args) in EXPORTS.items():
-        if lenient and not hasattr(lib, name) and (name.startswith("gaudi_host_") or name in _ROUND6_EXPORTS + _NLL_EXPORTS + _GRID_EXPORTS + _TARGET_EXPORTS + _ATOMS_EXPORTS):
+        if lenient and not hasattr(lib, name) and (name.startswith("gaudi_host_") or name in _ROUND6_EXPORTS + _NLL_EXPORTS + _GRID_EXPORTS + _TARGET_EXPORTS + _ATOMS_EXPORTS + _KEY_EXPORTS):
             continue
         if lenient and abi != ABI_VERSION and name.startswith("gaudi_host_"):
             continue
diff --git a/gaudi_amd/csrc/gaudi_hip.hip b/gaudi_amd/csrc/gaudi_hip.hip
--- a/gaudi_amd/csrc/gaudi_hip.hip
+++ b/gaudi_amd/csrc/gaudi_hip.hip
@@ -73,6 +73,7 @@
   NodeBuf nodes = kResident;
   bool two = false;
   bool fr = false;
+  bool n1 = false;
   int ef = 2;
   int groups = 0;
   int nslots = 0;
@@ -113,6 +114,8 @@
   LaunchPlan plan;
   bool split = true;
   bool no_fr = false;
+  bool no_n1 = false;
+  std::string last_key;
   bool wide_full = true;
   bool gn8_pq = true;
   bool gn8 = true;
@@ -686,8 +689,8 @@
 }
 static std::string key_name(const KernelKey& k) {
   char buf[160];
-  snprintf(buf, sizeof buf, "waves=%d SP=%d MR=%d GN=%d FR=%d PG=%d EF=%d HPE=%d HPP=%d VT=%d", k.waves, k.sp, (int)k.mr, k.gn, (int)k.fr,
-           (int)k.pg, k.ef, k.hpe, k.hpp, (int)k.vt);
+  snprintf(buf, sizeof buf, "waves=%d SP=%d MR=%d GN=%d FR=%d PG=%d N1=%d EF=%d HPE=%d HPP=%d VT=%d", k.waves, k.sp, (int)k.mr, k.gn,
+           (int)k.fr, (int)k.pg, (int)k.n1, k.ef, k.hpe, k.hpp, (int)k.vt);
   return buf;
 }
 static std::string duplicate_kernel_key() {
@@ -727,20 +730,27 @@
 static NodeBuf launch_nodes(const LaunchPlan& p, int hpe, int hpp) {
   return p.nodes == kPredFifthGlobal && !(hpe && hpp) ? kResident : p.nodes;
 }
-static kernel_fn plan_kernel(const LaunchPlan& p, int hpe, int hpp, bool vt) {
+static kernel_fn plan_kernel(const LaunchPlan& p, int hpe, int hpp, bool vt, KernelKey* key = nullptr) {
+  KernelKey unused;
+  KernelKey& k = key ? *key : unused;
   if (p.waves != 8) {
-    KernelKey k = key4(hpe, hpp, p.nodes == kAllGlobal, hpe ? p.ef : 2);
+    k = key4(hpe, hpp, p.nodes == kAllGlobal, hpe ? p.ef : 2);
     k.vt = vt && hpp;
     return find_kernel(k);
   }
   const NodeBuf nodes = launch_nodes(p, hpe, hpp);
   const bool mr = p.mr && hpp;
-  KernelKey k = nodes == kResident ? key8(hpe, hpp, p.ring, mr) : key8(hpe, hpp, 1, true, nodes);
+  k = nodes == kResident ? key8(hpe, hpp, p.ring, mr) : key8(hpe, hpp, 1, true, nodes);
   k.vt = vt && hpp;
   if (p.fr && nodes == kResident && !mr) {
     k.fr = true;
     if (kernel_fn f = find_kernel(k)) return f;
     k.fr = false;
+  }
+  if (p.n1 && nodes == kResident && !mr) {
+    k.n1 = true;
+    if (kernel_fn f = find_kernel(k)) return f;
+    k.n1 = false;
   }
   return find_kernel(k);
 }
@@ -816,7 +826,8 @@
   const LaunchPlan& plan = h->plan;
   const bool v8 = plan.waves == 8;
   const bool se = hpe && plan.ef > 2;
-  const kernel_fn fn = plan_kernel(plan, hpe, hpp, P.vt != nullptr);
+  KernelKey key{};
+  const kernel_fn fn = plan_kernel(plan, hpe, hpp, P.vt != nullptr, &key);
   if (!fn)
     return fail(h, GAUDI_E_INVALID,
                 "no kernel instantiated for padded hidden sizes (" + std::to_string(hpe) + "," + std::to_string(hpp) + ")" +
@@ -875,6 +886,7 @@
   }
 #endif
   HIPCHECK(h, hipGetLastError());
+  h->last_key = key_name(key);
   if (h->prof) {
     HIPCHECK(h, h->prof_log.end(h->stream, ev));
     h->prof_steps += steps;
@@ -1125,9 +1137,13 @@
   const NodeBuf nodes = pg_run ? kPredFifthGlobal : gn8;
   P.pubx = acc.pubx;
   P.pub_ch = acc.pub_ch;
+  auto one_step_tail = [](int H, int HP) { return !HP || !w8::nh_odd(HP) || has_ktail(H, HP); };
+  const bool n1_run = !h->no_n1 && nodes == kResident && acc.mode == 1 && n_slots <= 16 &&
+                      one_step_tail(h->ecfg.hidden_nf, hpe) && one_step_tail(h->pcfg.hidden_nf, hpp);
   if (getenv("GAUDI_DEBUG_PLAN"))
-    fprintf(stderr, "[plan] molecules=%d workgroups=%d N=%d node slots=%d S=%d split=%d mr=%d nodes=%d pub_ch=%d pubx=%d lds=%zu\n", B0, B, N,
-            n_slots, M.S, acc.mode, (int)mr_run, (int)nodes, acc.pub_ch, acc.pubx, lds_bytes8(hpe, hpp, n_slots, Dz, M.S, acc.pubx, acc.mode, nodes));
+    fprintf(stderr, "[plan] molecules=%d workgroups=%d N=%d node slots=%d S=%d split=%d mr=%d nodes=%d n1=%d pub_ch=%d pubx=%d lds=%zu\n", B0, B,
+            N, n_slots, M.S, acc.mode, (int)mr_run, (int)nodes, (int)n1_run, acc.pub_ch, acc.pubx,
+            lds_bytes8(hpe, hpp, n_slots, Dz, M.S, acc.pubx, acc.mode, nodes));
   auto up = [&](DevBuf& d, const void* src, size_t bytes) -> hipError_t {
     hipError_t e = d.reserve(bytes);
     if (e != hipSuccess) return e;
@@ -1192,6 +1208,7 @@
   plan.mr = mr_run;
   plan.nodes = nodes;
   plan.fr = !h->no_fr && gn8 == kResident && acc.mode == 1 && n_slots > 16;
+  plan.n1 = n1_run;
   plan.groups = B;
   plan.nslots = n_slots;
   plan.hk = hk;
@@ -1325,6 +1342,7 @@
   }
   if (const char* v = getenv("GAUDI_PRED_ROUNDS")) h->pred_rounds = atoi(v) != 0;
   h->no_fr = getenv("GAUDI_NO_FR") != nullptr;
+  h->no_n1 = getenv("GAUDI_NO_N1") != nullptr;
   h->plan.waves = h->variant;
   if (hipSetDevice(device) != hipSuccess || hipStreamCreateWithFlags(&h->stream, hipStreamNonBlocking) != hipSuccess) {
     delete h;
@@ -1362,6 +1380,11 @@
 
 const char* gaudi_last_error(const gaudi_handle* h) { return h ? h->err.c_str() : "null handle"; }
 const char* gaudi_last_warning(const gaudi_handle* h) { return h ? h->warn.c_str() : ""; }
+int gaudi_last_kernel_key(const gaudi_handle* h, char* buf, int n) {
+  if (!h || !buf || n <= 0) return GAUDI_E_INVALID;
+  snprintf(buf, (size_t)n, "%s", h->last_key.c_str());
+  return GAUDI_OK;
+}
 int gaudi_abi_version(void) { return GAUDI_ABI_VERSION; }
 int gaudi_profile_clock(gaudi_handle* h, double* shader_mhz) {
   if (!h || !shader_mhz) return GAUDI_E_INVALID;
diff --git a/gaudi_amd/csrc/kern8s1_edm_192.hip b/gaudi_amd/csrc/kern8s1_edm_192.hip
--- /dev/null
+++ b/gaudi_amd/csrc/kern8s1_edm_192.hip
@@ -0,0 +1,10 @@
+#include "kernel_table.h"
+
+namespace {
+using namespace gaudi;
+using V = V8T<1, false, 0, false, false, true>;
+const KernelEntry kEntries[] = {
+    entry<V, 192, 0>(),
+};
+KernelTable kTable(kEntries);
+}
diff --git a/gaudi_amd/csrc/kern8s1_fused_192_208.hip b/gaudi_amd/csrc/kern8s1_fused_192_208.hip
--- /dev/null
+++ b/gaudi_amd/csrc/kern8s1_fused_192_208.hip
@@ -0,0 +1,10 @@
+#include "kernel_table.h"
+
+namespace {
+using namespace gaudi;
+using V = V8T<1, false, 0, false, false, true>;
+const KernelEntry kEntries[] = {
+    entry<V, 192, 208>(),
+};
+KernelTable kTable(kEntries);
+}
diff --git a/gaudi_amd/csrc/kernel_table.h b/gaudi_amd/csrc/kernel_table.h
--- a/gaudi_amd/csrc/kernel_table.h
+++ b/gaudi_amd/csrc/kernel_table.h
@@ -11,12 +11,13 @@
   bool mr;
   int gn;
   bool fr, pg;
+  bool n1;
   int ef;
   int hpe, hpp;
   bool vt;
 };
 inline bool operator==(const KernelKey& a, const KernelKey& b) {
-  return a.waves == b.waves && a.sp == b.sp && a.mr == b.mr && a.gn == b.gn && a.fr == b.fr && a.pg == b.pg && a.ef == b.ef &&
+  return a.waves == b.waves && a.sp == b.sp && a.mr == b.mr && a.gn == b.gn && a.fr == b.fr && a.pg == b.pg && a.n1 == b.n1 && a.ef == b.ef &&
          a.hpe == b.hpe && a.hpp == b.hpp && a.vt == b.vt;
 }
 
@@ -33,6 +34,7 @@
   e.key.gn = V::kGN;
   e.key.fr = V::kFR;
   e.key.pg = V::kPG;
+  e.key.n1 = V::kN1;
   e.key.ef = V::kEF;
   e.key.hpe = HPE;
   e.key.hpp = HPP;
diff --git a/gaudi_amd/csrc/sampler_kernel.h b/gaudi_amd/csrc/sampler_kernel.h
--- a/gaudi_amd/csrc/sampler_kernel.h
+++ b/gaudi_amd/csrc/sampler_kernel.h
@@ -96,7 +96,7 @@
   static constexpr int kThreads = gaudi::kThreads;
   static constexpr bool kGlobalNodes = GN;
   static constexpr int kWaveCount = 4, kSplit = 0, kGN = GN ? 1 : 0, kEF = EF;
-  static constexpr bool kMR = false, kFR = false, kPG = false;
+  static constexpr bool kMR = false, kFR = false, kPG = false, kN1 = false;
   using Graph = gaudi::MolGraph;
   template <int HP> using EdmSmem = gaudi::NetSmem<HP, GN, EF>;
   __device__ __forceinline__ static void set_rows(Graph&, const int*, int, int) {}
@@ -248,7 +248,7 @@
   if (tr != nullptr && threadIdx.x == 0) tr[K + 1] = (lds_base() + uni(mean_off_))[3];
 }
 #ifndef GAUDI_STAMPS
-template <int HP, int SP, int GN = 0, bool FL = false>
+template <int HP, int SP, int GN = 0, int FL = 0>
 __device__ __attribute__((noinline)) void edm8_call(EdmDev W_, Graph8Args ga_, float t_val_, float* gnode_ = nullptr) {
   extern __shared__ __attribute__((aligned(16))) float smem[];
   const EdmDev W = uni(W_);
@@ -261,7 +261,7 @@
   sm.hk = ga.hk ? smem + ga.hk : nullptr;
   w8::edm_forward<HP, SP, GN, FL>(W, mg, sm, L.sZ, L.sEps, L.sMean, t_val, (int)threadIdx.x);
 }
-template <int HP, int SP, bool MR, int GN = 0, bool FL = false, bool PG = false>
+template <int HP, int SP, bool MR, int GN = 0, int FL = 0, bool PG = false>
 __device__ __attribute__((noinline)) void pred_fwd8_call(PredDev W_, Graph8Args ga_, float t_val_, float* stash_, float readout_div_,
                                                          float* gnode_ = nullptr) {
   extern __shared__ __attribute__((aligned(16))) float smem[];
@@ -274,7 +274,7 @@
   sm.hk = ga.hk ? smem + ga.hk : nullptr;
   w8::pred_forward<HP, SP, MR, GN, FL>(W, mg, sm, L.sZ, uni(t_val_), uni(stash_), uni(readout_div_), (int)threadIdx.x);
 }
-template <int HP, int SP, bool MR, int GN = 0, bool FL = false, bool PG = false>
+template <int HP, int SP, bool MR, int GN = 0, int FL = 0, bool PG = false>
 __device__ __attribute__((noinline)) void pred_bwd8_call(PredDev W_, Graph8Args ga_, float* stash_, float readout_div_, int resume_,
                                                          float* gnode_ = nullptr) {
   extern __shared__ __attribute__((aligned(16))) float smem[];
@@ -289,13 +289,14 @@
 }
 #endif
 
-template <int SP, bool MR = false, int GN = 0, bool FR = false, bool PG = false>
+template <int SP, bool MR = false, int GN = 0, bool FR = false, bool PG = false, bool N1 = false>
 struct V8T {
-  static constexpr bool kFL = MR || GN != 0 || FR;
+  static_assert(!N1 || (!MR && GN == 0 && !FR && !PG), "N1 is a form of the plain resident kernel");
+  static constexpr int kFL = N1 ? w8::kNodeOneTile : (MR || GN != 0 || FR) ? w8::kNodeFresh : w8::kNodePlain;
   static constexpr int kThreads = w8::kThreads;
   static constexpr int kSplit = SP;
   static constexpr int kWaveCount = 8, kGN = GN, kEF = 2;
-  static constexpr bool kMR = MR, kFR = FR, kPG = PG;
+  static constexpr bool kMR = MR, kFR = FR, kPG = PG, kN1 = N1;
   using Graph = w8::MolGraph;
   __host__ __device__ static int graph_floats(int N, int S) { return 2 * S + align16(N) + align16((N + 1 + S + 1) / 2); }
   __device__ __forceinline__ static float* load_graph(const KParams& P, int b, float* base, const float* sMask, Graph& mg, int tid, int wave) {
diff --git a/gaudi_amd/csrc/w8_edm.h b/gaudi_amd/csrc/w8_edm.h
--- a/gaudi_amd/csrc/w8_edm.h
+++ b/gaudi_amd/csrc/w8_edm.h
@@ -117,7 +117,7 @@
   }
 }
 
-template <int HP, int SP = 0, int GN = 0, bool FL = false>
+template <int HP, int SP = 0, int GN = 0, int FL = 0>
 __device__ __forceinline__ void edm_forward(const EdmDev& W, const MolGraph& mg, const NetSmem<HP, SP, GN>& sm, const float* sZ,
                                             float* sEps, float* sMean , float t_val, int tid STAMP_DECL) {
   constexpr int LD = HP + 4;
@@ -242,19 +242,23 @@
       }
       __syncthreads();
       STAMP(ST_BARRIER);
-      if constexpr (STG) stage_rows(xs0, sm.h, N * LD, wave, lane);
-      for (int idx = tid; idx < N * (HP / 4); idx += kThreads) {
-        const int n = idx / (HP / 4), f = 4 * (idx % (HP / 4));
-        if constexpr (STG)
-          *(f4*)(xs1 + n * LD + f) = (*(const f4*)(sm.agg + n * LD + f) + *(const f4*)(sm.agg1 + n * LD + f)) / W.normf;
-        else
-          *(f4*)(sm.agg + n * LD + f) = (*(const f4*)(sm.agg + n * LD + f) + *(const f4*)(sm.agg1 + n * LD + f)) / W.normf;
-      }
-      if constexpr (STG) stage_wait();
-      else __syncthreads();
+      constexpr bool SUM = NH && GN == 0;
+      if constexpr (!SUM) {
+        if constexpr (STG) stage_rows(xs0, sm.h, N * LD, wave, lane);
+        for (int idx = tid; idx < N * (HP / 4); idx += kThreads) {
+          const int n = idx / (HP / 4), f = 4 * (idx % (HP / 4));
+          if constexpr (STG)
+            *(f4*)(xs1 + n * LD + f) = (*(const f4*)(sm.agg + n * LD + f) + *(const f4*)(sm.agg1 + n * LD + f)) / W.normf;
+          else
+            *(f4*)(sm.agg + n * LD + f) = (*(const f4*)(sm.agg + n * LD + f) + *(const f4*)(sm.agg1 + n * LD + f)) / W.normf;
+        }
+        if constexpr (STG) stage_wait();
+        else __syncthreads();
+      }
       STAMP(ST_MISC);
-      node_gemm_x<HP, EPI_SILU, true, GN, NH, kAheadOne, kAheadOne, FL>(wb, wbe, G + 3 * PK, sm.h, xs0, !h_kept, G + 4 * PK, sm.agg, xs1, bn1, sm.p, nullptr, nullptr,
-                                              mg.NC, wave, lane, tw, keep ? node_ctx_keep<HP>(hctx(), sm.hk, mg.NC) : hctx(), pf, G + 5 * PK);
+      node_gemm_x<HP, EPI_SILU, true, GN, NH, kAheadOne, kAheadOne, FL, SUM ? 2 : 0>(
+          wb, wbe, G + 3 * PK, sm.h, xs0, !h_kept, G + 4 * PK, sm.agg, xs1, bn1, sm.p, nullptr, nullptr, mg.NC, wave, lane, tw,
+          keep ? node_ctx_keep<HP>(hctx(), sm.hk, mg.NC) : hctx(), pf, G + 5 * PK, nullptr, nullptr, sm.agg1, W.normf);
       STAMP(ST_NODE);
       __syncthreads();
       STAMP(ST_BARRIER);
diff --git a/gaudi_amd/csrc/w8_nodes_f16.h b/gaudi_amd/csrc/w8_nodes_f16.h
--- a/gaudi_amd/csrc/w8_nodes_f16.h
+++ b/gaudi_amd/csrc/w8_nodes_f16.h
@@ -75,11 +75,29 @@
   f4 x;
   uint32_t mx;
 };
-template <int HP>
-__device__ __forceinline__ SplitRowH split_row_load(const float* X, int n, int lane) {
+struct RowsOne {
+  const float* x;
+  __device__ __forceinline__ f4 load(int off) const { return *(const f4*)(x + off); }
+};
+template <bool DIV>
+struct RowsSum {
+  const float *a, *b;
+  float d;
+  __device__ __forceinline__ f4 load(int off) const {
+    const f4 s = *(const f4*)(a + off) + *(const f4*)(b + off);
+    return DIV ? s / d : s;
+  }
+};
+__device__ __forceinline__ RowsOne rows_of(const float* x) { return RowsOne{x}; }
+__device__ __forceinline__ RowsOne rows_of(const RowsOne& r) { return r; }
+__device__ __forceinline__ RowsOne rows_of(decltype(nullptr)) { return RowsOne{nullptr}; }
+template <bool DIV>
+__device__ __forceinline__ RowsSum<DIV> rows_of(const RowsSum<DIV>& r) { return r; }
+template <int HP, class SRC>
+__device__ __forceinline__ SplitRowH split_row_load(const SRC& X, int n, int lane) {
   constexpr int LD = HP + 4;
   SplitRowH r;
-  r.x = lane < HP / 4 ? *(const f4*)(X + n * LD + 4 * lane) : splat(0.f);
+  r.x = lane < HP / 4 ? X.load(n * LD + 4 * lane) : splat(0.f);
   r.mx = umax(umax(absbits(r.x[0]), absbits(r.x[1])), umax(absbits(r.x[2]), absbits(r.x[3])));
   return r;
 }
@@ -109,8 +127,9 @@
   }
   if (lane == 0) sb.scale(HP)[ct * 16 + c] = inv;
 }
-template <int HP>
-__device__ __forceinline__ void split_rows_h(const SplitBufH& sb, const float* X, int N, int wave, int lane) {
+template <int HP, class SRC>
+__device__ __forceinline__ void split_rows_h(const SplitBufH& sb, const SRC& X_, int N, int wave, int lane) {
+  const auto X = rows_of(X_);
   for (int n = wave; n < N; n += 2 * kWaves) {
     const int n2 = n + kWaves < N ? n + kWaves : n;
     SplitRowH a = split_row_load<HP>(X, n, lane), b = split_row_load<HP>(X, n2, lane);
@@ -133,6 +152,9 @@
 #ifndef GAUDI_NODE_LATE
 #define GAUDI_NODE_LATE 0
 #endif
+#ifndef GAUDI_NODE_TAIL_EARLY
+#define GAUDI_NODE_TAIL_EARLY 0
+#endif
 template <int HP>
 struct NodeGeoH {
   static constexpr int T = HP / 16;
@@ -160,10 +182,10 @@
       vo[u] = (on && wave + kWaves * u < NodeGeoH<HP>::T) ? lane * 16 + (wave + kWaves * u) * 2048 : kOOBBytes;
   }
 };
-template <int HP>
+template <int HP, int NU = NodeGeoH<HP>::NTW>
 __device__ __forceinline__ void nh_load(NodeSetH<NodeGeoH<HP>::NTW>& s, const WBuf& wh, int chunk_off, const TileLanesH<HP>& tl) {
 #pragma unroll
-  for (int u = 0; u < NodeGeoH<HP>::NTW; ++u) {
+  for (int u = 0; u < NU; ++u) {
     s.p[u][0] = __builtin_bit_cast(u4, __builtin_amdgcn_raw_buffer_load_b128(wh.r, tl.vo[u], chunk_off * 4, GAUDI_NODE_LOAD_AUX));
     s.p[u][1] = __builtin_bit_cast(u4, __builtin_amdgcn_raw_buffer_load_b128(wh.r, tl.vo[u] + 1024, chunk_off * 4, GAUDI_NODE_LOAD_AUX));
   }
@@ -179,6 +201,12 @@
   });
 }
 
+constexpr int kNodePlain = 0;
+constexpr int kNodeFresh = 1;
+constexpr int kNodeOneTile = 2;
+constexpr int kTailRuntime = 0;
+constexpr int kTailOne = 1;
+
 struct NodeCtxH {
   float winv;
   float* split_a;
@@ -188,17 +216,21 @@
   float* scales_b = nullptr;
 };
 
-template <int HP, int EPI, bool TWO, int MAXNT, int PIN = kAheadOne, int POUT = kAheadOne, bool FL = false>
-__device__ __forceinline__ void node_gemm_h(const WBuf& wh, int Wa, const float* sXa, bool do_split_a, int Wb, const float* sXb,
+template <int HP, int EPI, bool TWO, int MAXNT, int PIN = kAheadOne, int POUT = kAheadOne, int FL = kNodePlain, int TAIL = kTailRuntime,
+          int NU = 0, class XB = const float*>
+__device__ __forceinline__ void node_gemm_h(const WBuf& wh, int Wa, const float* sXa, bool do_split_a, int Wb, const XB& sXb,
                                             const float* sBias, float* sY, const float* sRes, const float* sMask, int N, int wave,
                                             int lane, const NodeCtxH& cx, NodePFH<HP>& pf, int nextW = -1, float* gPre = nullptr,
                                             uint32_t* sMaxOut = nullptr ,
                                             NodeStampH* ns = nullptr) {
   (void)ns;
   using G = NodeGeoH<HP>;
-  constexpr int T = G::T, LD = HP + 4, NTW = G::NTW, nc = G::nc, D = G::D;
+  constexpr int T = G::T, LD = HP + 4, NTW = NU > 0 ? NU : G::NTW, nc = G::nc, D = G::D;
   constexpr int kIn = PIN < D ? PIN : D, kOut = POUT < D ? POUT : D;
   constexpr int kLate = nc < D ? 0 : (GAUDI_NODE_LATE < kOut ? GAUDI_NODE_LATE : kOut);
+  constexpr int TQ = TAIL == kTailOne ? 1 : 4;
+  const bool ktail = TAIL == kTailOne ? true : cx.ktail;
+  constexpr bool kFresh = FL == kNodeFresh;
   const int c = lane & 15, g = lane >> 4;
   const int nt = (MAXNT < 2 || N <= 16) ? 1 : (MAXNT < 3 || N <= 32) ? 2 : 3;
   const bool seq = TWO && cx.split_b == cx.split_a;
@@ -209,16 +241,16 @@
   const int Wn = nextW >= 0 ? nextW : Wa;
   static_for<D>([&](auto d_tag) {
     constexpr int d = decltype(d_tag)::value;
-    if constexpr (d >= kIn) nh_load<HP>(pf.s[d], wh, 2 * Wa + d * nh_chunk_floats(HP), tl);
+    if constexpr (d >= kIn) nh_load<HP, NTW>(pf.s[d], wh, 2 * Wa + d * nh_chunk_floats(HP), tl);
   });
-  float ta[NTW][4], tb[NTW][4];
+  float ta[NTW][TQ], tb[NTW][TQ];
   if constexpr (G::odd) {
 #pragma unroll
     for (int u = 0; u < NTW; ++u) {
       const int t = wave + kWaves * u < T ? wave + kWaves * u : 0;
 #pragma unroll
-      for (int q = 0; q < 4; ++q) {
-        const int ln = ((q == 0 || !cx.ktail) && wave + kWaves * u < T) ? lane : kOOBLane;
+      for (int q = 0; q < TQ; ++q) {
+        const int ln = ((q == 0 || !ktail) && wave + kWaves * u < T) ? lane : kOOBLane;
         ta[u][q] = __builtin_bit_cast(float, __builtin_amdgcn_raw_buffer_load_b32(wh.r, ln * 4, (2 * Wa + nh_tail_off(HP) + t * 256 + q * 64) * 4, 0));
         if constexpr (TWO)
           tb[u][q] = __builtin_bit_cast(float, __builtin_amdgcn_raw_buffer_load_b32(wh.r, ln * 4, (2 * Wb + nh_tail_off(HP) + t * 256 + q * 64) * 4, 0));
@@ -227,8 +259,8 @@
   }
   NSTAMP(0);
   if (!(kAblateH & 1)) {
-    const int ls = FL ? fresh(lane) : lane;
-    if (do_split_a) split_rows_h<HP>(sa, sXa, N, wave, ls);
+    const int ls = kFresh ? fresh(lane) : lane;
+    if (do_split_a) split_rows_h<HP>(sa, rows_of(sXa), N, wave, ls);
     if (TWO && !seq) split_rows_h<HP>(sb, sXb, N, wave, ls);
     NSTAMP(1);
     if (do_split_a || (TWO && !seq)) lds_barrier();
@@ -252,7 +284,7 @@
     const float* q = s_.chunk(i) + bpos + j * 512;
     return BH{*(const u4*)q, *(const u4*)(q + 256)};
   };
-  auto mm = [&](const NodeSetH<NTW>& s, const BH& b, int j) {
+  auto mm = [&](const NodeSetH<G::NTW>& s, const BH& b, int j) {
     if (kAblateH & 2) {
       asm volatile("" ::"v"(s.p[0][0]), "v"(s.p[0][1]), "v"(s.p[NTW - 1][0]), "v"(s.p[NTW - 1][1]), "v"(b.h), "v"(b.l));
       return;
@@ -264,21 +296,34 @@
 #pragma unroll
     for (int u = 0; u < NTW; ++u) acc1[j][u] = mfma_h(s.p[u][1], b.h, acc1[j][u]);
   };
-  auto fold = [&](const SplitBufH& s_, const float (&tw)[NTW][4]) {
+  auto tail_steps = [&](const SplitBufH& s_, const float (&tw)[NTW][TQ], auto j_tag) {
+    constexpr int j = decltype(j_tag)::value;
+    if constexpr (G::odd) {
+      const float* xt = s_.tail(HP) + j * 256 + g * 16 + c;
+#pragma unroll
+      for (int u = 0; u < NTW; ++u) y[j][u] = mfma1(tw[u][0], xt[0], y[j][u]);
+      if constexpr (TQ > 1) {
+        if (!ktail) {
+#pragma unroll
+          for (int q = 1; q < TQ; ++q)
+#pragma unroll
+            for (int u = 0; u < NTW; ++u) y[j][u] = mfma1(tw[u][q], xt[64 * q], y[j][u]);
+        }
+      }
+    }
+  };
+  constexpr bool kTailEarly = GAUDI_NODE_TAIL_EARLY != 0;
+  auto tail_early = [&](const SplitBufH& s_, const float (&tw)[NTW][TQ]) {
+    if constexpr (kTailEarly && G::odd)
+      static_for<MAXNT>([&](auto j_tag) {
+        if (decltype(j_tag)::value < nt) tail_steps(s_, tw, j_tag);
+      });
+  };
+  auto fold = [&](const SplitBufH& s_, const float (&tw)[NTW][TQ]) {
     static_for<MAXNT>([&](auto j_tag) {
       constexpr int j = decltype(j_tag)::value;
       if (j < nt) {
-        if constexpr (G::odd) {
-          const float* xt = s_.tail(HP) + j * 256 + g * 16 + c;
-#pragma unroll
-          for (int u = 0; u < NTW; ++u) y[j][u] = mfma1(tw[u][0], xt[0], y[j][u]);
-          if (!cx.ktail) {
-#pragma unroll
-            for (int q = 1; q < 4; ++q)
-#pragma unroll
-              for (int u = 0; u < NTW; ++u) y[j][u] = mfma1(tw[u][q], xt[64 * q], y[j][u]);
-          }
-        }
+        if constexpr (!kTailEarly) tail_steps(s_, tw, j_tag);
         const float sc = s_.scale(HP)[j * 16 + c] * cx.winv;
 #pragma unroll
         for (int u = 0; u < NTW; ++u) {
@@ -311,9 +356,9 @@
       }
       __builtin_amdgcn_sched_barrier(0);
       if (!(kAblateH & 4)) {
-        if constexpr (i + D < nc) nh_load<HP>(pf.s[d], wh, 2 * Wcur + (i + D) * nh_chunk_floats(HP), tl);
-        else if constexpr (!last_src) nh_load<HP>(pf.s[d], wh, 2 * Wb + d * nh_chunk_floats(HP), tl);
-        else if constexpr (d < kOut - kLate) nh_load<HP>(pf.s[d], wh, 2 * Wn + d * nh_chunk_floats(HP), tl_next);
+        if constexpr (i + D < nc) nh_load<HP, NTW>(pf.s[d], wh, 2 * Wcur + (i + D) * nh_chunk_floats(HP), tl);
+        else if constexpr (!last_src) nh_load<HP, NTW>(pf.s[d], wh, 2 * Wb + d * nh_chunk_floats(HP), tl);
+        else if constexpr (d < kOut - kLate) nh_load<HP, NTW>(pf.s[d], wh, 2 * Wn + d * nh_chunk_floats(HP), tl_next);
       }
       __builtin_amdgcn_sched_barrier(0);
       bcur = bnext;
@@ -323,15 +368,16 @@
     constexpr int d = decltype(d_tag)::value;
     if constexpr (d >= kOut - kLate && d < kOut) {
       __builtin_amdgcn_sched_barrier(0);
-      if (!(kAblateH & 4)) nh_load<HP>(pf.s[d], wh, 2 * Wn + d * nh_chunk_floats(HP), tl_next);
+      if (!(kAblateH & 4)) nh_load<HP, NTW>(pf.s[d], wh, 2 * Wn + d * nh_chunk_floats(HP), tl_next);
       __builtin_amdgcn_sched_barrier(0);
     }
   };
   NSTAMP(3);
 #if GAUDI_NODE_PRIO
-  if constexpr (!FL)
+  if constexpr (!kFresh)
     if ((GAUDI_NODE_PRIO == 1 && wave >= kWaves / 2) || (GAUDI_NODE_PRIO == 2 && wave < kWaves / 2)) __builtin_amdgcn_s_setprio(1);
 #endif
+  tail_early(sa, ta);
   source(std::integral_constant<int, 0>{}, sa);
   NSTAMP(4);
   if constexpr (!TWO) late(std::integral_constant<int, kOut - kLate>{});
@@ -340,9 +386,10 @@
   if constexpr (TWO) {
     if (seq) {
       lds_barrier();
-      split_rows_h<HP>(sb, sXb, N, wave, FL ? fresh(lane) : lane);
+      split_rows_h<HP>(sb, sXb, N, wave, kFresh ? fresh(lane) : lane);
       lds_barrier();
     }
+    tail_early(sb, tb);
     source(std::integral_constant<int, 1>{}, sb);
     late(std::integral_constant<int, kOut - kLate>{});
     fold(sb, tb);
@@ -351,9 +398,9 @@
     if constexpr (decltype(d_tag)::value > kOut - kLate) late(d_tag);
   });
 #if GAUDI_NODE_PRIO
-  if constexpr (!FL) __builtin_amdgcn_s_setprio(0);
-#endif
-  const int le = FL ? fresh(lane) : lane, ce = le & 15, ge = le >> 4;
+  if constexpr (!kFresh) __builtin_amdgcn_s_setprio(0);
+#endif
+  const int le = kFresh ? fresh(lane) : lane, ce = le & 15, ge = le >> 4;
   static_for<MAXNT>([&](auto j_tag) {
     constexpr int j = decltype(j_tag)::value;
     if (j < nt) {
@@ -364,7 +411,7 @@
         f4 yy = y[j][u];
         if (t < T && nd < N) {
           float* dst = sY + nd * LD + 16 * t + 4 * ge;
-          const bool pad = G::odd && cx.ktail && t == T - 1 && ge > 0;
+          const bool pad = G::odd && ktail && t == T - 1 && ge > 0;
           if (pad) yy = splat(0.f);
           if (gPre != nullptr) nstash_store((f4*)(gPre + nd * HP + 16 * t + 4 * ge), yy);
           if (sMaxOut != nullptr) atomicMax(sMaxOut + nd, umax(umax(absbits(yy[0]), absbits(yy[1])), umax(absbits(yy[2]), absbits(yy[3]))));
@@ -408,14 +455,22 @@
   if constexpr (NH) node_prefetch_h<HP, AHEAD>(pf, wbe, W, wave, lane);
   else node_prefetch<HP>(pf, wb, W, wave, lane, tw);
 }
-template <int HP, int EPI, bool TWO, int GN, bool NH, int PIN, int POUT, bool FL = false, class PF>
+template <int HP, int EPI, bool TWO, int GN, bool NH, int PIN, int POUT, int FL = kNodePlain, int XBS = 0, class PF>
 __device__ __forceinline__ void node_gemm_x(const WBuf& wb, const WBuf& wbe, int Wa, const float* Xa, const float* XaS, bool split_a, int Wb,
                                             const float* Xb, const float* XbS, const float* sBias, float* sY, const float* sRes,
                                             const float* sMask, int N, int wave, int lane, bool tw, const NodeCtxH& cx, PF& pf,
-                                            int nextW = -1, float* gPre = nullptr, uint32_t* sMaxOut = nullptr) {
+                                            int nextW = -1, float* gPre = nullptr, uint32_t* sMaxOut = nullptr,
+                                            const float* Xb1 = nullptr, float xb_div = 1.f) {
+  static_assert(XBS == 0 || (NH && GN == 0 && TWO), "summed second sources: the fp16-pair form of the resident kernels");
   if constexpr (NH) {
-    node_gemm_h<HP, EPI, TWO, GN ? 3 : 2, PIN, POUT, FL>(wbe, Wa, Xa, split_a, Wb, Xb, sBias, sY, sRes, sMask, N, wave, lane, cx, pf, nextW, gPre,
-                                                         sMaxOut);
+    constexpr int MAXNT = GN ? 3 : FL == kNodeOneTile ? 1 : 2;
+    constexpr int TAIL = FL == kNodeOneTile && nh_odd(HP) ? kTailOne : kTailRuntime;
+    if constexpr (XBS == 0)
+      node_gemm_h<HP, EPI, TWO, MAXNT, PIN, POUT, FL, TAIL>(wbe, Wa, Xa, split_a, Wb, Xb, sBias, sY, sRes, sMask, N, wave, lane, cx, pf, nextW,
+                                                            gPre, sMaxOut);
+    else
+      node_gemm_h<HP, EPI, TWO, MAXNT, PIN, POUT, FL, TAIL>(wbe, Wa, Xa, split_a, Wb, RowsSum<XBS == 2>{Xb, Xb1, xb_div}, sBias, sY, sRes, sMask, N,
+                                                            wave, lane, cx, pf, nextW, gPre, sMaxOut);
   } else if constexpr (GN != 0) {
     node_gemm_n<HP, EPI, true, 3>(wb, Wa, XaS, Wb, XbS, sBias, sY, sRes, sMask, N, wave, lane, tw, &pf, nextW, gPre);
   } else {
diff --git a/gaudi_amd/csrc/w8_pred.h b/gaudi_amd/csrc/w8_pred.h
--- a/gaudi_amd/csrc/w8_pred.h
+++ b/gaudi_amd/csrc/w8_pred.h
@@ -65,7 +65,7 @@
   return ch > T ? T : ch;
 }
 
-template <int HP, int SP = 0, bool MR = false, int GN = 0, bool FL = false, class SM = PredSmem<HP, SP, GN>>
+template <int HP, int SP = 0, bool MR = false, int GN = 0, int FL = 0, class SM = PredSmem<HP, SP, GN>>
 __device__ __forceinline__ void pred_forward(const PredDev& W, const MolGraph& mg, const SM& sm, const float* sZ,
                                              float t_val, float* stash, float readout_div, int tid STAMP_DECL) {
   constexpr int LD = HP + 4;
@@ -225,19 +225,23 @@
     }
     __syncthreads();
     STAMP(ST_BARRIER);
-    if constexpr (STG) stage_rows(xs0, h, N * LD, wave, lane);
-    for (int idx = tid; idx < N * (HP / 4); idx += kThreads) {
-      const int n = idx / (HP / 4), f = 4 * (idx % (HP / 4));
-      if constexpr (STG)
-        *(f4*)(xs1 + n * LD + f) = *(const f4*)(agg + n * LD + f) + *(const f4*)(agg1 + n * LD + f);
-      else
-        *(f4*)(agg + n * LD + f) = *(const f4*)(agg + n * LD + f) + *(const f4*)(agg1 + n * LD + f);
-    }
-    if constexpr (STG) stage_wait();
-    else __syncthreads();
+    constexpr bool SUM = NH && GN == 0;
+    if constexpr (!SUM) {
+      if constexpr (STG) stage_rows(xs0, h, N * LD, wave, lane);
+      for (int idx = tid; idx < N * (HP / 4); idx += kThreads) {
+        const int n = idx / (HP / 4), f = 4 * (idx % (HP / 4));
+        if constexpr (STG)
+          *(f4*)(xs1 + n * LD + f) = *(const f4*)(agg + n * LD + f) + *(const f4*)(agg1 + n * LD + f);
+        else
+          *(f4*)(agg + n * LD + f) = *(const f4*)(agg + n * LD + f) + *(const f4*)(agg1 + n * LD + f);
+      }
+      if constexpr (STG) stage_wait();
+      else __syncthreads();
+    }
     STAMP(ST_MISC);
-    node_gemm_x<HP, EPI_SILU, true, GN, NH, kAheadOne, kAheadOne, FL>(wb, wbe, Lw.Wn1h, h, xs0, !keep, Lw.Wn1a, agg, xs1, Lw.bn1, p, nullptr, nullptr, mg.NC, wave, lane,
-                                            tw, keep ? node_ctx_keep<HP>(hctx(), sm.hk, mg.NC) : hctx(), pf, Lw.Wn2, st + 2 * N * HP );
+    node_gemm_x<HP, EPI_SILU, true, GN, NH, kAheadOne, kAheadOne, FL, SUM ? 1 : 0>(
+        wb, wbe, Lw.Wn1h, h, xs0, !keep, Lw.Wn1a, agg, xs1, Lw.bn1, p, nullptr, nullptr, mg.NC, wave, lane, tw,
+        keep ? node_ctx_keep<HP>(hctx(), sm.hk, mg.NC) : hctx(), pf, Lw.Wn2, st + 2 * N * HP , nullptr, agg1);
     STAMP(ST_NODE);
     __syncthreads();
     STAMP(ST_BARRIER);
@@ -272,7 +276,7 @@
   STAMP(ST_X0);
 }
 
-template <int HP, int SP = 0, bool MR = false, int GN = 0, bool FL = false, class SM = PredSmem<HP, SP, GN>>
+template <int HP, int SP = 0, bool MR = false, int GN = 0, int FL = 0, class SM = PredSmem<HP, SP, GN>>
 __device__ __forceinline__ void pred_backward(const PredDev& W, const MolGraph& mg, const SM& sm, const float* stash,
                                               float* sGrad, float readout_div, int pub_ch, int tid STAMP_DECL, const float* sZin = nullptr) {
   constexpr int LD = HP + 4;
diff --git a/gaudi_amd/engine.py b/gaudi_amd/engine.py
--- a/gaudi_amd/engine.py
+++ b/gaudi_amd/engine.py
@@ -156,6 +156,14 @@
         v = C.c_double(0.0)
         self._check(fn(self.h, C.byref(v)), "gaudi_profile_clock")
         return float(v.value)
+
+    def last_kernel_key(self) -> str:
+        fn = getattr(self.lib, "gaudi_last_kernel_key", None)
+        if fn is None or not fn.argtypes:
+            return ""
+        buf = C.create_string_buffer(256)
+        self._check(fn(self.h, buf, len(buf)), "gaudi_last_kernel_key")
+        return buf.value.decode()
 
     def keep_h(self) -> int:
         fn = getattr(self.lib, "gaudi_last_keep_h", None)
diff --git a/include/gaudi_hip.h b/include/gaudi_hip.h
--- a/include/gaudi_hip.h
+++ b/include/gaudi_hip.h
@@ -55,6 +55,7 @@
 void gaudi_destroy(gaudi_handle* h);
 const char* gaudi_last_error(const gaudi_handle* h);
 const char* gaudi_last_warning(const gaudi_handle* h);
+int gaudi_last_kernel_key(const gaudi_handle* h, char* buf, int n);
 #define GAUDI_ABI_VERSION 7
 int gaudi_abi_version(void);
 
```

Result: faster. 222.4 (median of 6 runs) (+2.7%).
